# JulHoltzDevelopers/WavesAndEigenvalues.jl

Measured on AMD Instinct MI355X. Metric: eigenpairs/sec, higher is better.
Workload: dtype f64

## Files before the change

dev/probes/modes_ab.py:

```python
import os, sys
import numpy as np
ROOT = os.path.dirname(os.path.dirname(os.path.dirname(os.path.abspath(__file__))))
sys.path.insert(0, ROOT)
import wae_amd
from wae_amd.helmholtz.family import annulus_family
preset = sys.argv[1] if len(sys.argv) > 1 else "C3"
r = int(sys.argv[2]) if len(sys.argv) > 2 else 64
modes = [int(m) for m in sys.argv[3:]] or [0, 1, 2, 6]
L, pb = annulus_family(preset, tau=2e-4)
fam = L.device()
cz = L.coefficients(2 * np.pi * (500 + 20j))
names = {0: "A X", 1: "residual", 2: "Jacobi sweep", 6: "product + first sweep"}
out = {}
for m in modes:
    os.environ["WAE_BENCH_MODE"] = str(m)
    best = min(fam.bench_spmv(cz, r=r, reps=30) for _ in range(3))
    out[names.get(m, m)] = round(best * 1e3, 1)
print(os.environ.get("WAE_LIB_PATH", "default"), preset, r, out, flush=True)
```

wavesandeigenvalues.jl_amd/csrc/debug.hip:

```cpp
#include <algorithm>
#include <vector>

#include "solver.h"

namespace {
struct StreamGuard {
    hipStream_t s = nullptr;
    ~StreamGuard() { if (s) (void)hipStreamDestroy(s); }
};
int64_t span(int64_t nv, int64_t stride, int64_t blk) { return nv > 0 ? (nv - 1) * stride + blk : 0; }
void fill_xorshift(std::vector<cplx> &hx) {
    uint64_t s = 0x9E3779B97F4A7C15ull;
    for (auto &v : hx) { s ^= s << 13; s ^= s >> 7; s ^= s << 17; v.x = (double)(s & 0xFFFFF) / 524288.0 - 1.0; v.y = (double)((s >> 20) & 0xFFFFF) / 524288.0 - 1.0; }
}
template <class F> double mean_ms(hipStream_t st, int reps, F &&one) {
    for (int i = 0; i < 3; ++i) one();
    hipEvent_t e0, e1;
    HIP_CHECK(hipEventCreate(&e0));
    HIP_CHECK(hipEventCreate(&e1));
    HIP_CHECK(hipEventRecord(e0, st));
    for (int i = 0; i < reps; ++i) one();
    HIP_CHECK(hipEventRecord(e1, st));
    HIP_CHECK(hipEventSynchronize(e1));
    float ms = 0.f;
// ... 242 lines not shown
        HIP_CHECK(hipMemsetAsync(relres.p, 0, (size_t)nb * sizeof(double), st));
        HIP_CHECK(hipMemsetAsync(rescale.p, 0, (size_t)nb * sizeof(cplx), st));
        HIP_CHECK(hipMemsetAsync(cmask.p, 0, (size_t)nch, st));
        s_relres.alloc((size_t)nev * nb); s_int.alloc((size_t)nev * nint); s_cmask.alloc((size_t)nev * nch); s_rescale.alloc((size_t)nev * nb);
        s_sv.alloc((size_t)nev * 2 * nb); s_vsq.alloc((size_t)nev * 2 * nb);
        HIP_CHECK(hipMemsetAsync(s_sv.p, 0, (size_t)nev * 2 * nb * sizeof(double), st));
        HIP_CHECK(hipMemsetAsync(s_vsq.p, 0, (size_t)nev * 2 * nb * sizeof(cplx), st));
        GmresDev S;
        S.nb = nb; S.m = m; S.histcap = histcap;
        S.R = R.p; S.cs = cs.p; S.sn = sn.p; S.g = g.p; S.sv = sv.p; S.vsq = vsq.p;
        S.conv = ints.p; S.steps = S.conv + nb; S.iters = S.steps + nb; S.histlen = S.iters + nb; S.stalled = S.histlen + nb; S.status = S.stalled + nb;
        S.relres = relres.p; S.bnorm = bn.p; S.hist = hist.p; S.rescale = rescale.p; S.cmask = cmask.p;
        S.Hraw = Hraw.p; S.sub = sub.p;
        auto d2d = [&](void *dst, const void *src, size_t bytes) { HIP_CHECK(hipMemcpyAsync(dst, src, bytes, hipMemcpyDeviceToDevice, st)); };
        for (int e = 0, ii = 0; e < nev; ++e) {
            const int64_t kind = ev[4 * e], j = ev[4 * e + 1], off = ev[4 * e + 3];
            const int use_mask = ev[4 * e + 2] ? 1 : 0;
            const double tol = evd[2 * e], lim = evd[2 * e + 1];
            cplx *a = dpool.p + off;
            int row0 = -1, rows = 0;
            if (kind == WAE_GMRES_INIT) {
                launch_gmres_init(S, a, ddone.p + (size_t)ii * nb, use_mask, st);
                ++ii;
                row0 = 0; rows = 1;
            } else if (kind == WAE_GMRES_STEP) {
                d2d(vsq.p + (size_t)(j + 1) * nb, dinv.p + (size_t)e * 2 * nb, (size_t)nb * sizeof(cplx));
                launch_gmres_step(S, a, (int)j, tol, lim, use_mask, a + (j + 2) * N, n, st);
                row0 = (int)j + 1; rows = 1;
            } else if (kind == WAE_GMRES_PAIR) {
                cplx *c1 = a, *c2 = c1 + (j + 1) * N, *gram = c2 + (j + 1) * N, *norms = gram + 3 * N, *W1 = norms + 2 * N, *W2 = W1 + blk,
                     *alpha = W2 + blk, *c2m = alpha + N, *hd2 = c2m + (j + 1) * N;
                launch_gmres_pair_coef(S, (int)j, c1, c2, gram, alpha, c2m, hd2, st);
                d2d(vsq.p + (size_t)(j + 1) * nb, dinv.p + (size_t)e * 2 * nb, (size_t)2 * nb * sizeof(cplx));
                launch_gmres_step(S, c1, (int)j, tol, 1e300, use_mask, W1, n, st, norms);
                launch_gmres_step(S, hd2, (int)j + 1, tol, lim, use_mask, W2, n, st, norms + N);
                row0 = (int)j + 1; rows = 2;
            } else {
                launch_gmres_solve_y(S, (int)j, a, st);
            }
            d2d(s_relres.p + (size_t)e * nb, relres.p, (size_t)nb * sizeof(double));
            d2d(s_int.p + (size_t)e * nint, ints.p, (size_t)nint * sizeof(int));
            d2d(s_cmask.p + (size_t)e * nch, cmask.p, (size_t)nch);
            d2d(s_rescale.p + (size_t)e * nb, rescale.p, (size_t)nb * sizeof(cplx));
            if (rows) {
                d2d(s_sv.p + (size_t)e * 2 * nb, sv.p + (size_t)row0 * nb, (size_t)rows * nb * sizeof(double));
                d2d(s_vsq.p + (size_t)e * 2 * nb, vsq.p + (size_t)row0 * nb, (size_t)rows * nb * sizeof(cplx));
            }
        }
        auto back = [&](void *dst, const void *src, size_t bytes) { HIP_CHECK(hipMemcpyAsync(dst, src, bytes, hipMemcpyDeviceToHost, st)); };
        cplx *oc = (cplx *)cstate;
        back(pool, dpool.p, (size_t)plen * sizeof(cplx));
        back(oc, R.p, nR * sizeof(cplx)); back(oc + nR, sn.p, nrow * sizeof(cplx)); back(oc + nR + nrow, g.p, (nrow + nb) * sizeof(cplx));
        back(oc + nR + 2 * nrow + nb, vsq.p, (nrow + 2 * nb) * sizeof(cplx)); back(oc + nR + 3 * nrow + 3 * nb, Hraw.p, nR * sizeof(cplx));
        back(dstate, cs.p, nrow * sizeof(double)); back(dstate + nrow, sv.p, (nrow + 2 * nb) * sizeof(double));
        back(dstate + 2 * nrow + 2 * nb, sub.p, nrow * sizeof(double)); back(dstate + 3 * nrow + 2 * nb, hist.p, (size_t)histcap * nb * sizeof(double));
        back(snap_relres, s_relres.p, (size_t)nev * nb * sizeof(double)); back(snap_int, s_int.p, (size_t)nev * nint * sizeof(int));
        back(snap_cmask, s_cmask.p, (size_t)nev * nch); back(snap_rescale, s_rescale.p, (size_t)nev * nb * sizeof(cplx));
        back(snap_sv, s_sv.p, (size_t)nev * 2 * nb * sizeof(double)); back(snap_vsq, s_vsq.p, (size_t)nev * 2 * nb * sizeof(cplx));
        HIP_CHECK(hipStreamSynchronize(st));
        return WAE_OK;
    });
}

extern "C" {

int wae_bench_spmv(wae_family *h, const double *coeffs, int32_t r, int32_t reps, double *ms_out) {
    return guarded([&]() {
        WAE_REQUIRE(h && coeffs && r > 0 && reps > 0 && ms_out, "bad argument");
        HIP_CHECK(hipSetDevice(h->device));
        hipStream_t st = h->stream;
        const size_t cnt = (size_t)h->d * r;
        DevBuf<cplx> x, y, pcd;
        x.alloc(cnt); y.alloc(cnt);
        std::vector<cplx> hx(cnt);
        fill_xorshift(hx);
        HIP_CHECK(hipMemcpyAsync(x.p, hx.data(), cnt * sizeof(cplx), hipMemcpyHostToDevice, st));
        std::vector<zc> pc;
        plane_coeffs(h, coeffs, WAE_OP_N, pc);
        std::vector<cplx> tab((size_t)h->nplanes);
        slot_coeffs(h, h->slot_plane[0], pc, tab.data());
        pcd.upload(tab.data(), tab.size(), st);
        const OpDev A = h->ops[0].dev(WAE_OP_N);
        const int bmode = getenv("WAE_BENCH_MODE") ? atoi(getenv("WAE_BENCH_MODE")) : MODE_AX;
        DevBuf<cplx> bb;
        if (bmode != MODE_AX) { bb.alloc(cnt); HIP_CHECK(hipMemcpyAsync(bb.p, hx.data(), cnt * sizeof(cplx), hipMemcpyHostToDevice, st)); }
        auto one = [&]() { launch_spmv(A, pcd.p, 1 << 30, x.p, y.p, bmode != MODE_AX ? bb.p : nullptr, 0.8, r, bmode, st); };
        *ms_out = mean_ms(st, reps, one);
        return WAE_OK;
    });
}

int wae_debug_spmv(wae_family *h, int32_t which, int32_t level, int32_t mode, const double *coeffs, int32_t ncoef, const double *X,
                   const double *B, double *Y, double *B2, int32_t r, int32_t op, double jac_w, const uint8_t *cmask, int32_t flags,
                   int64_t *n_in_q, int64_t *n_out_q) {
    return guarded([&]() {
        WAE_REQUIRE(h && which >= 0 && which <= 2 && level >= 0 && op >= 0 && op <= 2, "bad argument");
        WAE_REQUIRE(level == 0 || h->solver_ready, "levels >= 1 need wae_solver_setup");
        WAE_REQUIRE(which == 0 ? (level == 0 || level < (int)h->ops.size() - 1) : level < (int)h->xfer.size(), "no such level");
        const int64_t n_in = which == 0 ? h->ops[level].n : (which == 1 ? h->xfer[level].nf : h->xfer[level].nc);
        const int64_t n_out = which == 0 ? h->ops[level].n : (which == 1 ? h->xfer[level].nc : h->xfer[level].nf);
        if (n_in_q) *n_in_q = n_in;
        if (n_out_q) *n_out_q = n_out;
        if (!X && !Y) return WAE_OK;
        WAE_REQUIRE(X && Y && r > 0 && r <= 256, "bad argument (1 <= r <= 256)");
        WAE_REQUIRE(which != 0 || (coeffs && (ncoef == 1 || ncoef == r)), "ncoef must be 1 or r");
        WAE_REQUIRE(mode >= MODE_AX && mode <= MODE_AX_J0 && (which == 0 || mode == (which == 1 ? MODE_AX : MODE_ADD)), "bad mode");
        WAE_REQUIRE(B || mode == MODE_AX || mode == MODE_AX_DS || mode == MODE_AX_J0, "this mode reads B");
        WAE_REQUIRE(mode != MODE_AX_J0 || B2, "mode 6 writes B2");
        HIP_CHECK(hipSetDevice(h->device));
        hipStream_t st = h->stream;
        const int *perm = level == 0 && which != 1 ? h->perm() : nullptr;
        const int *perm_in = level == 0 && which != 2 ? h->perm() : nullptr;
        DevBuf<cplx> xc, yc, xi, yi, bi, pcd;
        DevBuf<unsigned char> cm;
        const size_t cin = (size_t)n_in * r, cout = (size_t)n_out * r;
        xc.alloc(std::max(cin, cout)); yc.alloc(cout); xi.alloc(cin); yi.alloc(cout); bi.alloc(cout);
        HIP_CHECK(hipMemcpyAsync(xc.p, X, cin * sizeof(cplx), hipMemcpyHostToDevice, st));
        launch_colmajor_to_inter(xc.p, n_in, r, xi.p, r, st, perm_in);
        auto stage = [&](const double *src, cplx *dst) {
            HIP_CHECK(hipMemcpyAsync(yc.p, src, cout * sizeof(cplx), hipMemcpyHostToDevice, st));
            launch_colmajor_to_inter(yc.p, n_out, r, dst, r, st, perm);
        };
        stage(Y, yi.p);
        if (mode == MODE_AX_J0) stage(B2, bi.p);
        else if (B) stage(B, bi.p);
        if (cmask) cm.upload(cmask, (size_t)(r + 7) / 8, st);
        OpDev A;
        int cps = 1 << 30;
        if (which == 0) {
            std::vector<cplx> tab((size_t)ncoef * h->nplanes);
            std::vector<zc> pc;
            for (int s = 0; s < ncoef; ++s) {
                plane_coeffs(h, coeffs + (size_t)s * 2 * h->T, op, pc);
                slot_coeffs(h, h->slot_plane[level], pc, &tab[(size_t)s * h->nplanes]);
            }
            pcd.upload(tab.data(), tab.size(), st);
            A = h->ops[level].dev(op);
            cps = ncoef == 1 ? (1 << 30) : 1;
        } else {
            A = h->xfer[level].devR();
        }
        if (flags & 1) A.tiles = nullptr;
        const Transfer *xf = which == 0 ? nullptr : &h->xfer[level];
        const bool by_tile = xf && xf->ft.ready && !(flags & 1) && r >= 8;
        if (which == 2) {
            const cplx *src = (const void *)B == (const void *)Y ? yi.p : bi.p;
            if (by_tile) launch_prolong_tiles(xf->ft.dev, xi.p, src, yi.p, r, st, cmask ? cm.p : nullptr);
            else launch_prolong_add(xf->p_ptr.p, xf->p_col.p, xf->p_val.p, xf->nf, xi.p, src, yi.p, r, st, cmask ? cm.p : nullptr);
        } else
        launch_spmv(A, which == 0 ? pcd.p : h->one_dev.p, cps, xi.p, yi.p, (mode == MODE_AX || mode == MODE_AX_DS) ? nullptr : bi.p, jac_w, r, mode, st,
                    cmask ? cm.p : nullptr);
        launch_inter_to_colmajor(yi.p, r, n_out, r, yc.p, st, perm);
        HIP_CHECK(hipMemcpyAsync(Y, yc.p, cout * sizeof(cplx), hipMemcpyDeviceToHost, st));
        if (mode == MODE_AX_J0) {
            HIP_CHECK(hipStreamSynchronize(st));
            launch_inter_to_colmajor(bi.p, r, n_out, r, yc.p, st, perm);
            HIP_CHECK(hipMemcpyAsync(B2, yc.p, cout * sizeof(cplx), hipMemcpyDeviceToHost, st));
        }
        HIP_CHECK(hipStreamSynchronize(st));
        return WAE_OK;
    });
}

int wae_debug_prolong(wae_family *h, int32_t level, const double *X, const double *B, double *Y, double *norms, int32_t r, const uint8_t *cmask,
                      int32_t flags) {
    return guarded([&]() {
        WAE_REQUIRE(h && X && B && Y && norms, "bad argument");
        require_solver(h);
        WAE_REQUIRE(level >= 0 && level < (int)h->xfer.size(), "no such level");
        WAE_REQUIRE(r >= 1 && r <= 256, "bad argument (1 <= r <= 256)");
        WAE_REQUIRE(flags >= 0 && flags < 4, "unknown flag");
        const Transfer *xf = &h->xfer[level];
        const int64_t nc = xf->nc, nf = xf->nf;
        HIP_CHECK(hipSetDevice(h->device));
        hipStream_t st = h->stream;
        const int *perm = level == 0 ? h->perm() : nullptr;
        const size_t cin = (size_t)nc * r, cout = (size_t)nf * r;
        const bool by_tile = xf->ft.ready && !(flags & 1) && r >= 8;
        DevBuf<cplx> xc, yc, xi, yi, bi, part, nrm;
        DevBuf<unsigned char> cm;
        xc.alloc(cin); yc.alloc(cout); xi.alloc(cin); yi.alloc(cout); bi.alloc(cout); nrm.alloc((size_t)r);
        part.alloc((size_t)(by_tile ? xf->ft.dev.ntiles : PROLONG_NORM_BLOCKS) * r);
        HIP_CHECK(hipMemcpyAsync(xc.p, X, cin * sizeof(cplx), hipMemcpyHostToDevice, st));
        launch_colmajor_to_inter(xc.p, nc, r, xi.p, r, st, nullptr);
        HIP_CHECK(hipMemcpyAsync(yc.p, Y, cout * sizeof(cplx), hipMemcpyHostToDevice, st));
        launch_colmajor_to_inter(yc.p, nf, r, yi.p, r, st, perm);
        HIP_CHECK(hipStreamSynchronize(st));
        HIP_CHECK(hipMemcpyAsync(yc.p, B, cout * sizeof(cplx), hipMemcpyHostToDevice, st));
        launch_colmajor_to_inter(yc.p, nf, r, bi.p, r, st, perm);
        if (cmask) cm.upload(cmask, (size_t)(r + 7) / 8, st);
        cplx *const dst = (flags & 2) ? nullptr : yi.p;
        if (by_tile) launch_prolong_tiles(xf->ft.dev, xi.p, bi.p, dst, r, st, cmask ? cm.p : nullptr, part.p, nrm.p);
        else launch_prolong_add(xf->p_ptr.p, xf->p_col.p, xf->p_val.p, nf, xi.p, bi.p, dst, r, st, cmask ? cm.p : nullptr, part.p, nrm.p);
        launch_inter_to_colmajor(yi.p, r, nf, r, yc.p, st, perm);
        HIP_CHECK(hipMemcpyAsync(Y, yc.p, cout * sizeof(cplx), hipMemcpyDeviceToHost, st));
        std::vector<cplx> hn((size_t)r);
        HIP_CHECK(hipMemcpyAsync(hn.data(), nrm.p, (size_t)r * sizeof(cplx), hipMemcpyDeviceToHost, st));
        HIP_CHECK(hipStreamSynchronize(st));
        for (int b = 0; b < r; ++b) norms[b] = hn[(size_t)b].x;
        return WAE_OK;
    });
}

int wae_debug_vcycle(wae_family *h, int32_t level, const double *coeffs, int32_t ncoef, const double *B, double *Y, int32_t r, int32_t op,
                     int32_t flags, const uint8_t *cmask) {
    return guarded([&]() {
        WAE_REQUIRE(h && coeffs && B && Y, "bad argument");
        require_solver(h);
        const int L = (int)h->ops.size() - 1;
        WAE_REQUIRE(level >= 0 && level <= L, "no such level");
        WAE_REQUIRE(r >= 1 && r <= h->NB, "r must be in 1..NB (opts[6] of wae_solver_setup)");
        WAE_REQUIRE(ncoef == 1 || ncoef == r, "ncoef must be 1 or r");
        WAE_REQUIRE(op >= 0 && op <= 2, "bad op");
        WAE_REQUIRE(flags >= 0 && flags < 8, "unknown flag");
        WAE_REQUIRE(!(flags & 4) || level == 0, "flags bit 2 (Y = M^-1 A V) needs level 0");
        HIP_CHECK(hipSetDevice(h->device));
        hipStream_t st = h->stream;
        struct LightRestore { bool &on; bool was; ~LightRestore() { on = was; } } light_restore{h->vc_light, h->vc_light};
        h->vc_light = (flags & 1) != 0;
        const Batch bt = ncoef == 1 ? Batch::one_system(r, op) : Batch::per_column(r, op);
        std::vector<std::vector<zc>> pcs((size_t)bt.nsys);
        for (int s = 0; s < bt.nsys; ++s) plane_coeffs(h, coeffs + (size_t)s * 2 * h->T, op, pcs[(size_t)s]);
        upload_pc(h, pcs);
        dense_setup(h, bt);
        const int64_t n = h->ops[level].n;
        const size_t cnt = (size_t)n * r;
        const int *perm = level == 0 ? h->perm() : nullptr;
        DevBuf<cplx> col, vin, fout;
        DevBuf<unsigned char> cm;
        col.alloc(cnt);
        if (cmask) cm.upload(cmask, (size_t)(r + 7) / 8, st);
        const unsigned char *mk = (cmask && r >= 8) ? cm.p : nullptr;
        cplx *x = h->lx[level].p;
        HIP_CHECK(hipMemcpyAsync(col.p, Y, cnt * sizeof(cplx), hipMemcpyHostToDevice, st));
        launch_colmajor_to_inter(col.p, n, r, x, r, st, perm);
        launch_copy(x, h->lt[level].p, cnt, st);
        if (flags & 2) { fout.alloc(cnt); launch_copy(x, fout.p, cnt, st); }
        cplx *b = level == 0 ? h->W.p : h->lb[level].p;
        HIP_CHECK(hipMemcpyAsync(col.p, B, cnt * sizeof(cplx), hipMemcpyHostToDevice, st));
        bool have_x0 = false;
        if (flags & 4) {
            vin.alloc(cnt);
            launch_colmajor_to_inter(col.p, n, r, vin.p, r, st, perm);
            have_x0 = L > 0;
            launch_spmv(h->ops[0].dev(op), pc_level(h, 0), bt.cps, vin.p, b, have_x0 ? x : nullptr, have_x0 ? pre_weight(h) : 0.0, r,
                        have_x0 ? MODE_AX_J0 : MODE_AX, st, mk);
        } else {
            launch_colmajor_to_inter(col.p, n, r, b, r, st, perm);
        }
        const cplx *res = vcycle(h, bt, level, b, mk, have_x0, (flags & 2) ? fout.p : nullptr);
        launch_inter_to_colmajor(res, r, n, r, col.p, st, perm);
        HIP_CHECK(hipMemcpyAsync(Y, col.p, cnt * sizeof(cplx), hipMemcpyDeviceToHost, st));
        HIP_CHECK(hipStreamSynchronize(st));
        return WAE_OK;
    });
}

int wae_bench_spmv_level(wae_family *h, const double *coeffs, int32_t which, int32_t level, int32_t r, int32_t reps, double *ms_out,
                         int64_t *bytes_out) {
    return guarded([&]() {
        WAE_REQUIRE(h && coeffs && which >= 0 && which <= 2 && level >= 0 && r > 0 && r <= 256 && reps > 0 && ms_out, "bad argument");
        require_solver(h);
        WAE_REQUIRE(which == 0 ? (level == 0 || level < (int)h->ops.size() - 1) : level < (int)h->xfer.size(), "no such level");
        HIP_CHECK(hipSetDevice(h->device));
        hipStream_t st = h->stream;
        const int64_t n_in = which == 0 ? h->ops[level].n : (which == 1 ? h->xfer[level].nf : h->xfer[level].nc);
        const int64_t n_out = which == 0 ? h->ops[level].n : (which == 1 ? h->xfer[level].nc : h->xfer[level].nf);
        DevBuf<cplx> x, y, pcd;
        x.alloc((size_t)n_in * r); y.alloc((size_t)n_out * r);
        std::vector<cplx> hx((size_t)n_in * r);
        fill_xorshift(hx);
        HIP_CHECK(hipMemcpyAsync(x.p, hx.data(), hx.size() * sizeof(cplx), hipMemcpyHostToDevice, st));
        OpDev A;
        const cplx *pcp = h->one_dev.p;
        int64_t bytes = 2;
        if (which == 0) {
            std::vector<zc> pc;
            plane_coeffs(h, coeffs, WAE_OP_N, pc);
            std::vector<cplx> tab(h->nplanes);
            slot_coeffs(h, h->slot_plane[level], pc, tab.data());
            pcd.upload(tab.data(), tab.size(), st);
            pcp = pcd.p;
            A = h->ops[level].dev(WAE_OP_N);
            bytes = 0;
            for (size_t g = 0; g < h->ops[level].groups.size(); ++g) {
                const GroupHost &G = h->ops[level].groups[g];
                for (int q = 0; q < G.nplanes; ++q)
                    if (tab[G.plane0 + q].x != 0.0 || tab[G.plane0 + q].y != 0.0) bytes += G.nnz * 20 + (n_out + 1) * 4;
            }
        } else {
            A = h->xfer[level].devR();
            bytes = (int64_t)h->xfer[level].r_col.n * 12 + (n_out + 1) * 4;
        }
        bytes += (int64_t)r * (n_in + n_out) * 16;
        if (which == 2) bytes += (int64_t)r * n_out * 16;
        if (bytes_out) *bytes_out = bytes;
        const Transfer *xf = which == 0 ? nullptr : &h->xfer[level];
        const bool by_tile = xf && xf->ft.ready && r >= 8 && xfer_tiles_on();
        auto one = [&]() {
            if (which == 2) {
                if (by_tile) launch_prolong_tiles(xf->ft.dev, x.p, y.p, y.p, r, st);
                else launch_prolong_add(xf->p_ptr.p, xf->p_col.p, xf->p_val.p, xf->nf, x.p, y.p, y.p, r, st, nullptr);
            } else launch_spmv(A, pcp, 1 << 30, x.p, y.p, nullptr, 0.0, r, MODE_AX, st);
        };
        if (which == 2) HIP_CHECK(hipMemsetAsync(y.p, 0, (size_t)n_out * r * sizeof(cplx), st));
        *ms_out = mean_ms(st, reps, one);
        return WAE_OK;
    });
}

int wae_bench_triad(int32_t device, int64_t n, int32_t reps, double *gbs_out) {
    return guarded([&]() {
        WAE_REQUIRE(n > 0 && reps > 0 && gbs_out, "bad argument");
        HIP_CHECK(hipSetDevice(device));
        DevBuf<double> a, b, c;
        a.alloc(n); b.alloc(n); c.alloc(n);
        HIP_CHECK(hipMemset(b.p, 0, n * sizeof(double)));
        HIP_CHECK(hipMemset(c.p, 0, n * sizeof(double)));
        hipStream_t st;
        HIP_CHECK(hipStreamCreate(&st));
        hipEvent_t e0, e1;
        HIP_CHECK(hipEventCreate(&e0));
        HIP_CHECK(hipEventCreate(&e1));
        double best = 0.0;
        for (unsigned cap : {512u, 1024u, 4096u, 8192u, 65536u}) {
            for (int i = 0; i < 2; ++i) launch_triad(a.p, b.p, c.p, 1.5, n, st, cap);
            HIP_CHECK(hipEventRecord(e0, st));
            for (int i = 0; i < reps; ++i) launch_triad(a.p, b.p, c.p, 1.5, n, st, cap);
            HIP_CHECK(hipEventRecord(e1, st));
            HIP_CHECK(hipEventSynchronize(e1));
            float ms = 0.f;
            HIP_CHECK(hipEventElapsedTime(&ms, e0, e1));
            best = std::max(best, 3.0 * n * sizeof(double) * reps / (ms * 1e-3) / 1e9);
// ... 11 lines not shown
```

wavesandeigenvalues.jl_amd/csrc/gmres.hip:

```cpp
#include <cmath>

#include "solver.h"

void upload_pc(wae_family *h, const std::vector<std::vector<zc>> &pcs) {
    const int nsys = (int)pcs.size();
    const int nl = (int)h->ops.size();
    const size_t per_level = (size_t)nsys * h->nplanes;
    std::vector<cplx> tab(per_level * (nl + 2));
    for (int l = 0; l <= nl + 1; ++l) {
        if (l >= nl && h->n_penalty == 0) break;
        const std::vector<int> &sp = l < nl ? h->slot_plane[l] : (l == nl ? h->pen_slot : h->pen_row_slot);
        for (int s = 0; s < nsys; ++s) slot_coeffs(h, sp, pcs[s], &tab[l * per_level + (size_t)s * h->nplanes]);
    }
    h->pc_stride_level = per_level;
    h->pcdev.upload(tab.data(), tab.size(), h->stream);
    HIP_CHECK(hipStreamSynchronize(h->stream));
}
const cplx *pc_level(const wae_family *h, int l) { return h->pcdev.p + (size_t)l * h->pc_stride_level; }

void dense_setup(wae_family *h, const Batch &bt) {
    const int L = (int)h->ops.size() - 1;
    if (h->nc <= 0) return;
    HIP_CHECK(hipMemsetAsync(h->dstatus.p, 0, sizeof(int), h->stream));
    launch_dense_assemble(h->dense_planes.p, h->nplanes, (int)h->nc, pc_level(h, L), bt.nsys, bt.op, h->Ainv.p, h->stream);
    launch_dense_invert(h->Ainv.p, (int)h->nc, bt.nsys, h->dstatus.p, h->stream);
    int st = 0;
    HIP_CHECK(hipMemcpyAsync(&st, h->dstatus.p, sizeof(int), hipMemcpyDeviceToHost, h->stream));
    HIP_CHECK(hipStreamSynchronize(h->stream));
    if (st) throw WaeError(WAE_ERR_BREAKDOWN, "coarse operator is singular");
}

double pre_weight(const wae_family *h) { return h->vc_light ? h->jac_w_light : h->jac_w; }

cplx *vcycle(wae_family *h, const Batch &bt, int l, const cplx *b, const unsigned char *cm, bool have_x0, cplx *final_out, CycleNorms *cn) {
    const int L = (int)h->ops.size() - 1;
    hipStream_t st = h->stream;
    if (l == L) {
        launch_dense_apply(h->Ainv.p, (int)h->nc, bt.cps, b, h->lx[l].p, bt.nb, st, cm);
        return h->lx[l].p;
    }
    const OpDev A = h->ops[l].dev(bt.op);
    const cplx *pc = pc_level(h, l);
    cplx *x = h->lx[l].p, *t = h->lt[l].p;
    if (!have_x0) launch_jacobi0(A, pc, bt.cps, b, x, pre_weight(h), bt.nb, st, cm);
    for (int s = 1; s < h->nsweeps; ++s) {
        launch_spmv(A, pc, bt.cps, x, t, b, pre_weight(h), bt.nb, MODE_JAC, st, cm);
        std::swap(x, t);
    }
    launch_spmv(A, pc, bt.cps, x, t, b, 0.0, bt.nb, MODE_RES, st, cm);
    const bool by_tile = h->xfer[l].ft.ready && bt.nb >= 8 && xfer_tiles_on();
    launch_spmv(h->xfer[l].devR(), h->one_dev.p, 1 << 30, t, h->lb[l + 1].p, nullptr, 0.0, bt.nb, MODE_AX, st, cm);
    const cplx *xc = vcycle(h, bt, l + 1, h->lb[l + 1].p, cm);
    const int npost = h->vc_light ? 0 : h->nsweeps;
    const size_t npart = (size_t)(by_tile ? h->xfer[l].ft.dev.ntiles : PROLONG_NORM_BLOCKS) * bt.nb;
    const bool norms = cn && l == 0 && npost == 0 && npart <= h->partial.n && h->ops[l].n > 0 && !(cn->only && final_out);
    cplx *const px = (norms && cn->only) ? nullptr : (final_out && npost == 0) ? final_out : x;
    cplx *const part = norms ? h->partial.p : nullptr, *const nout = norms ? cn->out : nullptr;
    if (by_tile) launch_prolong_tiles(h->xfer[l].ft.dev, xc, x, px, bt.nb, st, cm, part, nout);
    else launch_prolong_add(h->xfer[l].p_ptr.p, h->xfer[l].p_col.p, h->xfer[l].p_val.p, h->xfer[l].nf, xc, x, px, bt.nb, st, cm, part, nout);
    if (norms) cn->done = true;
    if (px) x = px;
    for (int s = 0; s < npost; ++s) {
        cplx *dst = (final_out && s == npost - 1) ? final_out : t;
        launch_spmv(A, pc, bt.cps, x, dst, b, h->jac_w_post, bt.nb, MODE_JAC, st, cm);
        if (dst == t) std::swap(x, t); else x = dst;
    }
    if (final_out && x != final_out) { launch_copy(x, final_out, (size_t)h->ops[l].n * bt.nb, st); x = final_out; }
    return x;
}

struct ColState {
    std::vector<zc> H;
    std::vector<zc> Hraw;
    std::vector<zc> g;
    std::vector<double> cs;
    std::vector<zc> sn;
    std::vector<zc> cdef;
    int ld = 0;
    int steps = 0;
    bool conv = false;

    ColState(int m, bool keep_raw, double beta, bool done)
        : H((size_t)(m + 1) * m), Hraw(keep_raw ? (size_t)(m + 1) * m : 0), g(m + 1), cs(m), sn(m), cdef(m), ld(m + 1), conv(done) { g[0] = beta; }
    bool rotate_in(int jc, const zc *raw, zc cdef_j, bool &nan) {
        zc *Hc = &H[(size_t)jc * ld];
        for (int i = 0; i <= jc + 1; ++i) Hc[i] = raw[i];
        if (!Hraw.empty()) std::copy(raw, raw + jc + 2, &Hraw[(size_t)jc * ld]);
        cdef[jc] = cdef_j;
        for (int i = 0; i < jc; ++i) {
            const zc a = Hc[i], bb = Hc[i + 1];
            Hc[i] = cs[i] * a + sn[i] * bb;
            Hc[i + 1] = -std::conj(sn[i]) * a + cs[i] * bb;
        }
        const zc a = Hc[jc];
        const double bb = Hc[jc + 1].real();
        const double aa = std::abs(a);
        const double t = std::sqrt(aa * aa + bb * bb);
        if (!(t > 0.0) || std::isnan(t)) { conv = true; if (std::isnan(t)) nan = true; return false; }
        if (aa == 0.0) { cs[jc] = 0.0; sn[jc] = 1.0; }
        else { cs[jc] = aa / t; sn[jc] = (a / aa) * (bb / t); }
        Hc[jc] = cs[jc] * a + sn[jc] * bb;
        Hc[jc + 1] = 0;
        g[jc + 1] = -std::conj(sn[jc]) * g[jc];
        g[jc] = cs[jc] * g[jc];
        steps = jc + 1;
        return true;
    }
    std::vector<zc> back_substitute() const {
        std::vector<zc> y(steps);
        for (int i = steps - 1; i >= 0; --i) {
            zc s = g[i];
            for (int q = i + 1; q < steps; ++q) s -= H[(size_t)q * ld + i] * y[q];
            const zc dgi = H[(size_t)i * ld + i];
            y[i] = (dgi != zc(0)) ? s / dgi : zc(0);
        }
        return y;
    }
};

void penalty_polish(wae_family *h, const Batch &bt, const cplx *B, cplx *X) {
    if (h->n_penalty <= 0) return;
    static const std::vector<double> cheb = []() {
        const int n = 22;
        const double lo = 0.4, hi = 2.2, th = 0.5 * (hi + lo), de = 0.5 * (hi - lo);
        std::vector<double> w(n);
        for (int k = 0; k < n; ++k) w[k] = 1.0 / (th - de * std::cos((2 * k + 1) * M_PI / (2 * n)));
        std::vector<double> o;
        for (int a = 0, b = n - 1; a <= b; ++a, --b) { o.push_back(w[a]); if (a != b) o.push_back(w[b]); }
        return o;
    }();
    const int sweeps = (int)cheb.size();
    hipStream_t st = h->stream;
    const int nb = bt.nb;
    const int64_t nbk = h->n_penalty;
    const OpDev A = h->ops[0].dev(bt.op);
    const OpDev Ab = h->pen_op.dev(bt.op);
    const cplx *pcb = pc_level(h, (int)h->ops.size());
    if (bt.op == WAE_OP_N && h->pen_row_op.n == nbk) {
        launch_gather_rows(B, h->pen_rows.p, nbk, nb, h->pen_t.p, st);
        launch_spmv(h->pen_row_op.dev(WAE_OP_N), pc_level(h, (int)h->ops.size() + 1), bt.cps, X, h->pen_b.p, h->pen_t.p, 0.0, nb, MODE_RES, st);
    } else {
        launch_spmv(A, pc_level(h, 0), bt.cps, X, h->W.p, B, 0.0, nb, MODE_RES, st);
        launch_gather_rows(h->W.p, h->pen_rows.p, nbk, nb, h->pen_b.p, st);
    }
    launch_norms(h->pen_b.p, nbk, nb, h->partial.p, h->hdev.p, st);
    cplx *x = h->pen_x.p, *t = h->pen_t.p;
    launch_jacobi0(Ab, pcb, bt.cps, h->pen_b.p, x, cheb[0], nb, st);
    for (int s = 1; s < sweeps; ++s) {
        launch_spmv(Ab, pcb, bt.cps, x, t, h->pen_b.p, cheb[(size_t)s], nb, MODE_JAC, st);
        std::swap(x, t);
    }
    launch_spmv(Ab, pcb, bt.cps, x, t, h->pen_b.p, 0.0, nb, MODE_RES, st);
    launch_norms(t, nbk, nb, h->partial.p, h->hdev.p + nb, st);
    cplx *hp = h->h_pinned;
    HIP_CHECK(hipMemcpyAsync(hp, h->hdev.p, (size_t)2 * nb * sizeof(cplx), hipMemcpyDeviceToHost, st));
    HIP_CHECK(hipStreamSynchronize(st));
    for (int b = 0; b < nb; ++b)
        if (!(hp[nb + b].x <= 1e-3 * hp[b].x)) return;
    launch_scatter_add_rows(x, h->pen_rows.p, nbk, nb, X, st);
}

struct GmresEnv {
    bool lazy = env_int("WAE_LAZY", 1) != 0;
    double lazy_limit = getenv("WAE_LAZY_LIMIT") ? atof(getenv("WAE_LAZY_LIMIT")) : 1e100;
    bool device = env_int("WAE_GMRES_DEVICE", 1) != 0;
    int sync = std::max(1, env_int("WAE_GMRES_SYNC", 4));
    int pair_min = env_int("WAE_GMRES_PAIR", 2);
    int narrow_pair = env_int("WAE_NARROW_PAIR", -1);
    int debug = env_int("WAE_GMRES_DEBUG", 0);
    bool mask0 = env_int("WAE_GMRES_MASK0", 1) != 0;
};
static const GmresEnv &gmres_env() { static const GmresEnv e; return e; }

struct Gmres {
    wae_family *h;
    const Batch &bt;
    const cplx *B;
    cplx *X;
    const cplx *guess_dir;
    double tol;
    int maxit;
    bool have_x0;
    double *relres_out = nullptr;
    hipStream_t st = h->stream;
    int nb = bt.nb;
    int64_t n = h->d;
    size_t vec = (size_t)n * nb;
    OpDev A = h->ops[0].dev(bt.op);
    const cplx *pc = pc_level(h, 0);
    cplx *hp = h->h_pinned;
    bool reorth = nb <= 8;
    bool deflate = guess_dir != nullptr && h->ops.size() > 1;
    int off = deflate ? 1 : 0;
    int m = (int)std::min<size_t>(150, h->V.n / vec - 1) - off;
    bool lazy = gmres_env().lazy && !reorth && ((size_t)m + off + 2) * nb <= 4096 && ((size_t)m + off + 2) * nb <= h->vsq.n;
    bool pair_cfg = reorth && h->ops.size() > 1 &&
                    (gmres_env().narrow_pair > 0 || (gmres_env().narrow_pair < 0 && vec * sizeof(cplx) >= ((size_t)4 << 20)));
    size_t PK = (size_t)(m + off + 3) * nb;
    std::vector<double> bnorm = std::vector<double>(nb), relres = std::vector<double>(nb, 0.0);
    std::vector<int> iters = std::vector<int>(nb, 0);
    std::vector<unsigned char> done = std::vector<unsigned char>(nb, 0), stalled = std::vector<unsigned char>(nb, 0);
    int total_it = 0;
    bool nan_seen = false, x0_unchecked = have_x0;
    double t0 = now_s();
    std::vector<ColState> cs;
    std::vector<std::vector<double>> sv;
    std::vector<std::vector<double>> hist = std::vector<std::vector<double>>(nb);
    std::vector<double> unorm = std::vector<double>(nb, 0.0);
    std::vector<zc> beta0 = std::vector<zc>(nb, zc(0));
    const unsigned char *mk = nullptr;
    cplx *pr_dev = nullptr, *pr_host = nullptr;

    cplx *start() {
        if (!have_x0) launch_fill_zero(X, vec, st);
        CycleNorms cn{h->hdev.p, have_x0};
        cplx *const zb = vcycle(h, bt, 0, B, nullptr, false, nullptr, &cn);
        if (!cn.done) launch_norms(zb, n, nb, h->partial.p, h->hdev.p, st);
        HIP_CHECK(hipMemcpyAsync(hp, h->hdev.p, nb * sizeof(cplx), hipMemcpyDeviceToHost, st));
        HIP_CHECK(hipStreamSynchronize(st));
        for (int b = 0; b < nb; ++b) { bnorm[b] = hp[b].x; if (!(bnorm[b] > 0.0)) done[b] = 1; }
        return zb;
    }
    cplx *residual(CycleNorms *cn = nullptr) {
        launch_spmv(A, pc, bt.cps, X, h->W.p, B, 0.0, nb, MODE_RES, st);
        return vcycle(h, bt, 0, h->W.p, nullptr, false, nullptr, cn);
    }
    bool drop_bad_guess() {
        if (!x0_unchecked) return false;
        x0_unchecked = false;
        std::vector<cplx> keep(nb, cplx{1.0, 0.0});
        bool any_bad = false;
        for (int b = 0; b < nb; ++b)
            if (bnorm[b] > 0.0 && !(hp[b].x / bnorm[b] <= 1.0)) { keep[b] = cplx{0.0, 0.0}; any_bad = true; }
        if (!any_bad) return false;
        h->ydev.upload(keep.data(), nb, st);
        launch_mask_cols(X, h->ydev.p, n, nb, st);
        HIP_CHECK(hipStreamSynchronize(st));
        return true;
    }
    template <class F> bool cycle_start(F &&more) {
        bool all_done = true;
        for (int b = 0; b < nb; ++b) {
            if (bnorm[b] > 0.0) {
                relres[b] = hp[b].x / bnorm[b];
                if (std::isnan(relres[b])) nan_seen = true;
                done[b] = relres[b] <= tol || stalled[b];
                more(b);
            }
            if (!done[b]) all_done = false;
        }
        return all_done;
    }
    bool converged_by_estimate(int j) const {
        if (j > 12) return false;
        for (int b = 0; b < nb; ++b) if (stalled[b] || (bnorm[b] > 0.0 && !(relres[b] <= tol))) return false;
        return true;
    }
    template <class F> int finish(wae_solve_info *info, F &&debug_line) {
        if (have_x0 && !nan_seen) penalty_polish(h, bt, B, X);
        if (relres_out) for (int b = 0; b < nb; ++b) relres_out[b] = bnorm[b] > 0.0 ? relres[b] : 0.0;
        if (gmres_env().debug) {
            HIP_CHECK(hipStreamSynchronize(st));
            debug_line();
        }
        if (info) {
            int imax = 0, itot = 0, nun = 0;
            double rmax = 0.0;
            for (int b = 0; b < nb; ++b) {
                imax = std::max(imax, iters[b]);
                itot += iters[b];
                if (bnorm[b] > 0.0) {
                    if (!(relres[b] <= tol)) ++nun;
                    rmax = std::max(rmax, relres[b]);
                }
                if (stalled[b] && !(relres[b] <= tol)) info->levels |= 1 << 16;
            }
            info->iters_max = std::max(info->iters_max, imax);
            info->iters_total += itot;
            info->n_unconverged += nun;
            info->relres_max = std::max(info->relres_max, rmax);
            info->levels = (info->levels & (1 << 16)) | (int)h->ops.size();
        }
        if (nan_seen) throw WaeError(WAE_ERR_NAN, "NaN in GMRES");
        return total_it;
    }

    int run_device(wae_solve_info *info) {
        const GmresEnv &env = gmres_env();
        const double lim = env.lazy_limit;
        const bool use_mask = have_x0 || (env.mask0 && nb >= 8);
        const int nch = (nb + 7) / 8;
        const int histcap = maxit + m + 8;
        h->gs_R.reserve((size_t)m * (m + 1) * nb); h->gs_sn.reserve((size_t)m * nb); h->gs_g.reserve((size_t)(m + 1) * nb); h->gs_rescale.reserve((size_t)nb);
        h->gs_cs.reserve((size_t)m * nb); h->gs_sv.reserve((size_t)(m + 2) * nb); h->gs_relres.reserve((size_t)nb); h->gs_bnorm.reserve((size_t)nb);
        h->gs_hist.reserve((size_t)histcap * nb); h->gs_int.reserve((size_t)5 * nb + 4); h->gs_done.reserve((size_t)nb);
        h->cmask.reserve(nch); h->vsq.reserve((size_t)(m + 2) * nb);
        GmresDev S;
        S.nb = nb; S.m = m; S.histcap = histcap;
        S.R = h->gs_R.p; S.cs = h->gs_cs.p; S.sn = h->gs_sn.p; S.g = h->gs_g.p; S.sv = h->gs_sv.p; S.vsq = h->vsq.p;
        S.conv = h->gs_int.p; S.steps = S.conv + nb; S.iters = S.steps + nb; S.histlen = S.iters + nb; S.stalled = S.histlen + nb; S.status = S.stalled + nb;
        S.relres = h->gs_relres.p; S.bnorm = h->gs_bnorm.p; S.hist = h->gs_hist.p; S.rescale = h->gs_rescale.p; S.cmask = h->cmask.p;
        const int pair_min = env.pair_min;
        const bool pair_on = pair_min >= 0 && lim >= 1e50 && nb >= 8 && h->ops.size() > 1;
        h->gs_Hraw.reserve((size_t)m * (m + 1) * nb); h->gs_pair.reserve(((size_t)4 * (m + 3) + 8) * nb); h->gs_sub.reserve((size_t)m * nb);
        S.Hraw = h->gs_Hraw.p; S.sub = h->gs_sub.p;
        cplx *const pr_c1 = h->gs_pair.p, *const pr_c2 = pr_c1 + (size_t)(m + 3) * nb, *const pr_c2m = pr_c2 + (size_t)(m + 3) * nb,
                   *const pr_hd2 = pr_c2m + (size_t)(m + 3) * nb, *const pr_gram = pr_hd2 + (size_t)(m + 3) * nb, *const pr_alpha = pr_gram + (size_t)3 * nb,
                   *const pr_norm = pr_alpha + nb;
        HIP_CHECK(hipMemsetAsync(h->gs_int.p, 0, ((size_t)5 * nb + 4) * sizeof(int), st));
        cplx *const zb = start();
        std::vector<double> bn(bnorm);
        for (double &v : bn) if (!(v > 0.0)) v = 1.0;
        HIP_CHECK(hipMemcpyAsync(h->gs_bnorm.p, bn.data(), nb * sizeof(double), hipMemcpyHostToDevice, st));
        HIP_CHECK(hipStreamSynchronize(st));
        std::vector<int> hostint((size_t)5 * nb + 4);
        bool first = !have_x0;
        while (true) {
            CycleNorms cn{h->hdev.p, false};
            cplx *const z0 = first ? zb : residual(&cn);
            first = false;
            if (!cn.done) launch_norms(z0, n, nb, h->partial.p, h->hdev.p, st);
            HIP_CHECK(hipMemcpyAsync(hp, h->hdev.p, (size_t)nb * sizeof(cplx), hipMemcpyDeviceToHost, st));
            HIP_CHECK(hipStreamSynchronize(st));
            if (drop_bad_guess()) continue;
            if (cycle_start([](int) {}) || total_it >= maxit || nan_seen) break;
            launch_scale_inv(z0, h->hdev.p, h->V.p, n, nb, st);
            HIP_CHECK(hipMemcpyAsync(h->gs_done.p, done.data(), nb, hipMemcpyHostToDevice, st));
            launch_gmres_init(S, h->hdev.p, h->gs_done.p, use_mask ? 1 : 0, st);
            HIP_CHECK(hipStreamSynchronize(st));
            const unsigned char *mk = (use_mask && nb >= 8) ? h->cmask.p : nullptr;
            int j = 0;
            int status[4] = {0, 0, 0, 0};
            for (int b = 0; b < nb; ++b) status[0] += done[b] ? 0 : 1;
            int since_sync = 0;
            for (; j < m && total_it < maxit;) {
                const cplx *vj = h->V.p + (size_t)j * vec;
                const int nvj = j + 1;
                const bool fuse0 = h->ops.size() > 1;
                if (pair_on && j >= pair_min && j + 2 <= m && total_it + 2 <= maxit && status[0] > nb / 4) {
                    cplx *w1 = h->V.p + (size_t)nvj * vec, *w2 = w1 + vec;
                    launch_spmv(A, pc, bt.cps, vj, h->W.p, h->lx[0].p, pre_weight(h), nb, MODE_AX_J0, st, mk);
                    vcycle(h, bt, 0, h->W.p, mk, true, w1);
                    launch_spmv(A, pc, bt.cps, w1, h->W.p, h->lx[0].p, pre_weight(h), nb, MODE_AX_J0, st, mk);
                    vcycle(h, bt, 0, h->W.p, mk, true, w2);
                    launch_dots2_scaled(h->V.p, vec, nvj, w1, w2, n, nb, h->partial.p, pr_c1, pr_c2, pr_gram, h->vsq.p, st, mk);
                    launch_gmres_pair_coef(S, j, pr_c1, pr_c2, pr_gram, pr_alpha, pr_c2m, pr_hd2, st);
                    launch_axpy2_norm(h->V.p, vec, nvj, pr_c1, pr_c2m, pr_alpha, w1, w2, n, nb, h->partial.p, pr_norm, h->vsq.p + (size_t)nvj * nb, st, mk);
                    launch_gmres_step(S, pr_c1, j, tol, 1e300, use_mask ? 1 : 0, w1, n, st, pr_norm);
                    launch_gmres_step(S, pr_hd2, j + 1, tol, lim, use_mask ? 1 : 0, w2, n, st, pr_norm + nb);
                    j += 2;
                    total_it += 2;
                    since_sync += 2;
                } else {
                    launch_spmv(A, pc, bt.cps, vj, h->W.p, fuse0 ? h->lx[0].p : nullptr, fuse0 ? pre_weight(h) : 0.0, nb, fuse0 ? MODE_AX_J0 : MODE_AX, st, mk);
                    cplx *w = vcycle(h, bt, 0, h->W.p, mk, fuse0);
                    launch_dots_scaled(h->V.p, vec, nvj, w, n, nb, h->partial.p, h->hdev.p, h->vsq.p, st, mk);
                    launch_axpy_neg_norm(h->V.p, vec, nvj, h->hdev.p, h->V.p + (size_t)nvj * vec, n, nb, h->partial.p, h->hdev.p + (size_t)nvj * nb, st, mk,
                                         w, h->vsq.p + (size_t)nvj * nb);
                    launch_gmres_step(S, h->hdev.p, j, tol, lim, use_mask ? 1 : 0, h->V.p + (size_t)nvj * vec, n, st);
                    ++j;
                    ++total_it;
                    ++since_sync;
                }
                if (since_sync >= ((have_x0 && j <= 4) ? 1 : env.sync) || j == m || total_it >= maxit || status[0] <= nb / 4) {
                    since_sync = 0;
                    HIP_CHECK(hipMemcpyAsync(status, S.status, 3 * sizeof(int), hipMemcpyDeviceToHost, st));
                    HIP_CHECK(hipStreamSynchronize(st));
                    if (status[1]) nan_seen = true;
                    if (status[0] == 0 || nan_seen) break;
                }
            }
            if (j > 0) {
                launch_gmres_solve_y(S, j, h->ydev.p, st);
                launch_lincomb_add(h->V.p, vec, j, h->ydev.p, X, n, nb, st);
            }
            HIP_CHECK(hipMemcpyAsync(hostint.data(), h->gs_int.p, ((size_t)5 * nb + 4) * sizeof(int), hipMemcpyDeviceToHost, st));
            HIP_CHECK(hipMemcpyAsync(hp, h->gs_relres.p, nb * sizeof(double), hipMemcpyDeviceToHost, st));
            HIP_CHECK(hipStreamSynchronize(st));
            const double *rr = (const double *)hp;
            for (int b = 0; b < nb; ++b) {
                iters[b] = hostint[(size_t)2 * nb + b];
                stalled[b] = (unsigned char)hostint[(size_t)4 * nb + b];
                if (hostint[(size_t)nb + b] > 0 && bnorm[b] > 0.0) relres[b] = rr[b];
            }
            if (hostint[(size_t)5 * nb + 1]) nan_seen = true;
            if (nan_seen || converged_by_estimate(j)) break;
        }
        return finish(info, [&]() {
            int itot = 0;
            for (int b = 0; b < nb; ++b) itot += iters[b];
            fprintf(stderr, "[gmres] nb=%d x0=%d lockstep_its=%d column_its=%d %.1f ms (device recurrence)\n", nb, (int)have_x0, total_it, itot,
                    (now_s() - t0) * 1e3);
            if (env.debug > 2) {
                for (int b0 = 0; b0 < nb; b0 += bt.cps) {
                    fprintf(stderr, "[gmres]   steps");
                    for (int b = b0; b < std::min(nb, b0 + bt.cps); ++b) fprintf(stderr, " %d", iters[b]);
                    fprintf(stderr, "\n");
                }
            }
        });
    }

    void absorb(int b, int jc, const zc *raw, zc cdef_j) {
        ColState &c = cs[b];
        if (c.conv || !c.rotate_in(jc, raw, cdef_j, nan_seen)) return;
        iters[b]++;
        relres[b] = std::abs(c.g[jc + 1]) / bnorm[b];
        hist[b].push_back(relres[b]);
        const size_t hs = hist[b].size();
        if (relres[b] <= 0.7 * tol) c.conv = true;
        else if (hs > 60 && relres[b] > 0.9 * hist[b][hs - 31]) { c.conv = true; stalled[b] = 1; }
    }

    void pair_step(int j) {
        const cplx *vj = h->V.p + (size_t)(off + j) * vec;
        const int nv = off + j + 1;
        cplx *w1 = h->V.p + (size_t)nv * vec, *w2 = w1 + vec;
        cplx *c1a = pr_dev, *c2a = c1a + PK, *c1b = c2a + PK, *c2b = c1b + PK, *c2m = c2b + PK, *zero_al = c2m + PK,
             *gram = zero_al + nb, *alpha = gram + 3 * (size_t)nb, *nrm = alpha + nb, *inv = nrm + 2 * (size_t)nb,
             *tdef = inv + 2 * (size_t)nb;
        launch_spmv(A, pc, bt.cps, vj, h->W.p, h->lx[0].p, pre_weight(h), nb, MODE_AX_J0, st, mk);
        vcycle(h, bt, 0, h->W.p, mk, true, w1);
        if (deflate) {
            launch_dots(h->V.p, vec, 1, w1, n, nb, h->partial.p, tdef, st, mk);
            launch_axpy_neg(h->V.p, vec, 1, tdef, w1, n, nb, st, mk);
        }
        launch_spmv(A, pc, bt.cps, w1, h->W.p, h->lx[0].p, pre_weight(h), nb, MODE_AX_J0, st, mk);
        vcycle(h, bt, 0, h->W.p, mk, true, w2);
        launch_dots2_scaled(h->V.p, vec, nv, w1, w2, n, nb, h->partial.p, c1a, c2a, gram, h->vsq.p, st, mk);
        launch_fill_zero(zero_al, nb, st);
        launch_axpy2_norm(h->V.p, vec, nv, c1a, c2a, zero_al, w1, w2, n, nb, h->partial.p, nrm, inv, st, mk);
        launch_dots2_scaled(h->V.p, vec, nv, w1, w2, n, nb, h->partial.p, c1b, c2b, gram, h->vsq.p, st, mk);
        HIP_CHECK(hipMemcpyAsync(pr_host, pr_dev, (4 * PK) * sizeof(cplx), hipMemcpyDeviceToHost, st));
        HIP_CHECK(hipMemcpyAsync(pr_host + 5 * PK + nb, gram, (size_t)3 * nb * sizeof(cplx), hipMemcpyDeviceToHost, st));
        cplx *htdef = pr_host + 5 * PK + 7 * (size_t)nb;
        if (deflate) HIP_CHECK(hipMemcpyAsync(htdef, tdef, (size_t)nb * sizeof(cplx), hipMemcpyDeviceToHost, st));
        HIP_CHECK(hipStreamSynchronize(st));
        const cplx *hc1a = pr_host, *hc2a = hc1a + PK, *hc1b = hc2a + PK, *hc2b = hc1b + PK, *hgram = pr_host + 5 * PK + nb;
        cplx *hc2m = pr_host + 4 * PK, *halpha = pr_host + 5 * PK + 4 * (size_t)nb;
        auto Z = [](const cplx &v) { return zc(v.x, v.y); };
        std::vector<zc> rawcol((size_t)m + 3);
        std::vector<zc> beta(nb, zc(0));
        for (int b = 0; b < nb; ++b) {
            double g11 = hgram[b].x;
            zc g12 = Z(hgram[(size_t)nb + b]);
            for (int i = 0; i < nv; ++i) {
                const zc p1 = Z(hc1b[(size_t)i * nb + b]), p2 = Z(hc2b[(size_t)i * nb + b]);
                g11 -= std::norm(p1);
                g12 -= std::conj(p1) * p2;
            }
            beta[b] = g11 > 0.0 ? g12 / g11 : zc(0);
            if (!std::isfinite(beta[b].real()) || !std::isfinite(beta[b].imag())) beta[b] = zc(0);
            halpha[b] = cplx{beta[b].real(), beta[b].imag()};
            for (int i = 0; i < nv; ++i) {
                const zc q = Z(hc2b[(size_t)i * nb + b]) - beta[b] * Z(hc1b[(size_t)i * nb + b]);
                hc2m[(size_t)i * nb + b] = cplx{q.real(), q.imag()};
            }
        }
        HIP_CHECK(hipMemcpyAsync(c2m, hc2m, (size_t)nv * nb * sizeof(cplx), hipMemcpyHostToDevice, st));
        HIP_CHECK(hipMemcpyAsync(alpha, halpha, (size_t)nb * sizeof(cplx), hipMemcpyHostToDevice, st));
        launch_axpy2_norm(h->V.p, vec, nv, c1b, c2m, alpha, w1, w2, n, nb, h->partial.p, nrm, inv, st, mk);
        launch_scale_inv(w1, nrm, w1, n, nb, st, mk);
        launch_scale_inv(w2, nrm + nb, w2, n, nb, st, mk);
        cplx *hnrm = pr_host + 5 * PK + 5 * (size_t)nb;
        HIP_CHECK(hipMemcpyAsync(hnrm, nrm, (size_t)2 * nb * sizeof(cplx), hipMemcpyDeviceToHost, st));
        HIP_CHECK(hipStreamSynchronize(st));
        total_it += 2;
        for (int b = 0; b < nb; ++b) {
            ColState &c = cs[b];
            if (c.conv) continue;
            const double a1 = hnrm[b].x, a2 = hnrm[(size_t)nb + b].x;
            const int nk = j + 1;
            std::vector<zc> cc1(nk), cc2(nk);
            for (int i = 0; i < nk; ++i) {
                cc1[i] = Z(hc1a[(size_t)(off + i) * nb + b]) + Z(hc1b[(size_t)(off + i) * nb + b]);
                cc2[i] = Z(hc2a[(size_t)(off + i) * nb + b]) + Z(hc2b[(size_t)(off + i) * nb + b]);
            }
            const zc e1 = deflate ? Z(hc1a[b]) + Z(hc1b[b]) : zc(0), e2 = deflate ? Z(hc2a[b]) + Z(hc2b[b]) : zc(0);
            const zc cdef_j = deflate ? Z(htdef[b]) + e1 : zc(0);
            for (int i = 0; i < nk; ++i) rawcol[i] = cc1[i];
            rawcol[nk] = a1;
            absorb(b, j, rawcol.data(), cdef_j);
            if (c.conv) continue;
            if (!(a1 > 0.0)) { c.conv = true; continue; }
            for (int r = 0; r <= j; ++r) {
                zc d = 0;
                for (int i = std::max(0, r - 1); i < j; ++i) d += c.Hraw[(size_t)i * c.ld + r] * cc1[i];
                rawcol[r] = (cc2[r] - d - cc1[j] * cc1[r]) / a1;
            }
            rawcol[j + 1] = beta[b] - cc1[j];
            rawcol[j + 2] = a2 / a1;
            zc cdef_n = 0;
            if (deflate) {
                cdef_n = e2 - cc1[j] * cdef_j;
                for (int i = 0; i < j; ++i) cdef_n -= cc1[i] * c.cdef[i];
                cdef_n /= a1;
            }
            absorb(b, j + 1, rawcol.data(), cdef_n);
        }
    }

    void single_step(int j) {
        const cplx *vj = h->V.p + (size_t)(off + j) * vec;
        const int nvj = off + j + 1;
        const bool fuse0 = h->ops.size() > 1;
        launch_spmv(A, pc, bt.cps, vj, h->W.p, fuse0 ? h->lx[0].p : nullptr, fuse0 ? pre_weight(h) : 0.0, nb, fuse0 ? MODE_AX_J0 : MODE_AX, st, mk);
        cplx *w = vcycle(h, bt, 0, h->W.p, mk, fuse0);
        if (lazy) {
            launch_dots_scaled(h->V.p, vec, nvj, w, n, nb, h->partial.p, h->hdev.p, h->vsq.p, st, mk);
            launch_axpy_neg_norm(h->V.p, vec, nvj, h->hdev.p, h->V.p + (size_t)nvj * vec, n, nb, h->partial.p, h->hdev.p + (size_t)nvj * nb, st, mk,
                                 w, h->vsq.p + (size_t)nvj * nb);
        } else {
            launch_dots(h->V.p, vec, nvj, w, n, nb, h->partial.p, h->hdev.p, st, mk);
            if (reorth) {
                launch_axpy_neg(h->V.p, vec, nvj, h->hdev.p, w, n, nb, st, mk);
                cplx *h2 = h->hdev.p + (size_t)(off + m + 2) * nb;
                launch_dots(h->V.p, vec, nvj, w, n, nb, h->partial.p, h2, st, mk);
                launch_axpy_neg_norm(h->V.p, vec, nvj, h2, w, n, nb, h->partial.p, h->hdev.p + (size_t)nvj * nb, st, mk);
                launch_add(h2, h->hdev.p, (size_t)nvj * nb, st);
            } else {
                launch_axpy_neg_norm(h->V.p, vec, nvj, h->hdev.p, w, n, nb, h->partial.p, h->hdev.p + (size_t)nvj * nb, st, mk);
            }
            launch_scale_inv(w, h->hdev.p + (size_t)nvj * nb, h->V.p + (size_t)nvj * vec, n, nb, st, mk);
        }
        HIP_CHECK(hipMemcpyAsync(hp, h->hdev.p, (size_t)(nvj + 1) * nb * sizeof(cplx), hipMemcpyDeviceToHost, st));
        HIP_CHECK(hipStreamSynchronize(st));
        if (lazy) {
            for (int b = 0; b < nb; ++b) {
                const double sj = sv[nvj - 1][b];
                for (int i = 0; i < nvj; ++i) {
                    const double f = sv[i][b] > 0.0 ? sj / sv[i][b] : 0.0;
                    hp[(size_t)i * nb + b].x *= f;
                    hp[(size_t)i * nb + b].y *= f;
                }
                const double r = hp[(size_t)nvj * nb + b].x;
                sv[nvj][b] = r > 0.0 ? 1.0 / r : 0.0;
                hp[(size_t)nvj * nb + b].x = sj * r;
            }
            const double lim = gmres_env().lazy_limit;
            bool rescale = false;
            for (int b = 0; b < nb; ++b) rescale = rescale || sv[nvj][b] > lim || (sv[nvj][b] > 0.0 && sv[nvj][b] < 1.0 / lim);
            if (rescale) {
                launch_scale_inv(h->V.p + (size_t)nvj * vec, h->hdev.p + (size_t)nvj * nb, h->V.p + (size_t)nvj * vec, n, nb, st, mk);
                std::vector<cplx> ones(nb, cplx{1.0, 0.0});
                for (int b = 0; b < nb; ++b) if (sv[nvj][b] > 0.0) sv[nvj][b] = 1.0; else ones[b] = cplx{0.0, 0.0};
                HIP_CHECK(hipMemcpyAsync(h->vsq.p + (size_t)nvj * nb, ones.data(), (size_t)nb * sizeof(cplx), hipMemcpyHostToDevice, st));
                HIP_CHECK(hipStreamSynchronize(st));
            }
        }
        ++total_it;
        std::vector<zc> rawcol((size_t)m + 3);
        for (int b = 0; b < nb; ++b) {
            if (cs[b].conv) continue;
            for (int i = 0; i <= j + 1; ++i) rawcol[i] = zc(hp[(size_t)(off + i) * nb + b].x, hp[(size_t)(off + i) * nb + b].y);
            absorb(b, j, rawcol.data(), deflate ? zc(hp[b].x, hp[b].y) : zc(0));
        }
    }

    void add_alpha_g(const std::vector<zc> &num) {
        std::vector<cplx> al(nb, cplx{0.0, 0.0});
        for (int b = 0; b < nb; ++b) {
            if (!(unorm[b] > 0.0)) continue;
            const zc a = num[b] / unorm[b];
            if (std::isfinite(a.real()) && std::isfinite(a.imag())) al[b] = cplx{a.real(), a.imag()};
        }
        h->ydev.upload(al.data(), nb, st);
        launch_lincomb(guess_dir, 0, 1, h->ydev.p, h->U.p, n, nb, st);
        launch_add(h->U.p, X, vec, st);
        HIP_CHECK(hipStreamSynchronize(st));
    }

    int run_host(wae_solve_info *info) {
        sv.assign(lazy ? (size_t)m + off + 2 : 0, std::vector<double>(nb, 1.0));
        const int pair_min = 4;
        if (pair_cfg) {
            const size_t need = 6 * PK + 16 * (size_t)nb;
            h->gs_pair.reserve(need);
            if (h->h_pin_pair_n < need) {
                if (h->h_pin_pair) { (void)hipHostFree(h->h_pin_pair); h->h_pin_pair = nullptr; h->h_pin_pair_n = 0; }
                HIP_CHECK(hipHostMalloc((void **)&h->h_pin_pair, need * sizeof(cplx)));
                h->h_pin_pair_n = need;
            }
            pr_dev = h->gs_pair.p; pr_host = h->h_pin_pair;
            h->vsq.reserve(PK);
            std::vector<cplx> ones(PK, cplx{1.0, 0.0});
            h->vsq.upload(ones.data(), ones.size(), st);
            HIP_CHECK(hipStreamSynchronize(st));
        }
        cplx *const zb0 = start();
        std::vector<double> drift_ref(nb, 0.0);
        bool drift_mode = false;
        bool first = !have_x0;
        const int nch = (nb + 7) / 8;
        const bool use_mask = have_x0;
        std::vector<unsigned char> cm(nch, 1), cm_prev(nch, 2);
        h->cmask.reserve(nch);
        auto set_mask = [&](auto &&active) {
            for (int k = 0; k < nch; ++k) cm[k] = 0;
            for (int b = 0; b < nb; ++b) if (active(b)) cm[b >> 3] = 1;
            if (cm != cm_prev) {
                HIP_CHECK(hipMemcpyAsync(h->cmask.p, cm.data(), nch, hipMemcpyHostToDevice, st));
                HIP_CHECK(hipStreamSynchronize(st));
                cm_prev = cm;
            }
        };
        if (deflate) {
            launch_spmv(A, pc, bt.cps, guess_dir, h->W.p, nullptr, 0.0, nb, MODE_AX, st);
            launch_copy(vcycle(h, bt, 0, h->W.p), h->V.p, vec, st);
            launch_norms(h->V.p, n, nb, h->partial.p, h->hdev.p, st);
            launch_norms(guess_dir, n, nb, h->partial.p, h->hdev.p + nb, st);
            HIP_CHECK(hipMemcpyAsync(hp, h->hdev.p, (size_t)2 * nb * sizeof(cplx), hipMemcpyDeviceToHost, st));
            HIP_CHECK(hipStreamSynchronize(st));
            std::vector<cplx> un(nb);
            for (int b = 0; b < nb; ++b) {
                unorm[b] = (hp[b].x > 1e-12 * hp[nb + b].x && hp[nb + b].x > 0.0) ? hp[b].x : 0.0;
                un[b] = cplx{unorm[b], 0.0};
            }
            h->ydev.upload(un.data(), nb, st);
            launch_scale_inv(h->V.p, h->ydev.p, h->V.p, n, nb, st);
            HIP_CHECK(hipStreamSynchronize(st));
        }
        if (guess_dir && !deflate) {
            launch_spmv(A, pc, bt.cps, guess_dir, h->W.p, nullptr, 0.0, nb, MODE_AX, st);
            launch_copy(vcycle(h, bt, 0, h->W.p), h->U.p, vec, st);
            const cplx *zb = vcycle(h, bt, 0, B);
            launch_dots(h->U.p, 0, 1, zb, n, nb, h->partial.p, h->hdev.p, st);
            launch_dots(h->U.p, 0, 1, h->U.p, n, nb, h->partial.p, h->hdev.p + nb, st);
            HIP_CHECK(hipMemcpyAsync(hp, h->hdev.p, (size_t)2 * nb * sizeof(cplx), hipMemcpyDeviceToHost, st));
            HIP_CHECK(hipStreamSynchronize(st));
            std::vector<cplx> al(nb);
            for (int b = 0; b < nb; ++b) {
                const double den = hp[nb + b].x;
                al[b] = den > 0.0 ? cplx{hp[b].x / den, hp[b].y / den} : cplx{0.0, 0.0};
            }
            h->ydev.upload(al.data(), nb, st);
            launch_lincomb(guess_dir, 0, 1, h->ydev.p, X, n, nb, st);
            HIP_CHECK(hipStreamSynchronize(st));
            first = false;
        }
        while (true) {
            cplx *const z0 = !first ? residual() : guess_dir ? vcycle(h, bt, 0, B) : zb0;
            first = false;
            if (deflate) {
                launch_dots(h->V.p, 0, 1, z0, n, nb, h->partial.p, h->hdev.p + nb, st);
                launch_axpy_neg(h->V.p, 0, 1, h->hdev.p + nb, z0, n, nb, st);
            }
            launch_norms(z0, n, nb, h->partial.p, h->hdev.p, st);
            HIP_CHECK(hipMemcpyAsync(hp, h->hdev.p, (size_t)2 * nb * sizeof(cplx), hipMemcpyDeviceToHost, st));
            HIP_CHECK(hipStreamSynchronize(st));
            if (deflate) for (int b = 0; b < nb; ++b) beta0[b] = zc(hp[nb + b].x, hp[nb + b].y);
            if (drop_bad_guess()) continue;
            const bool all_done = cycle_start([&](int b) {
                if (!done[b]) {
                    const double est = hist[b].empty() ? -1.0 : hist[b].back();
                    if (drift_mode && drift_ref[b] > 0.0 && relres[b] > 0.5 * drift_ref[b]) { stalled[b] = 1; done[b] = 1; }
                    else if (est >= 0.0 && est <= tol && relres[b] > 50.0 * est) drift_mode = true;
                }
                drift_ref[b] = relres[b];
            });
            if (gmres_env().debug > 1) {
                double rmax = 0.0, emax = 0.0;
                for (int b = 0; b < nb; ++b) { rmax = std::max(rmax, relres[b]); if (!hist[b].empty()) emax = std::max(emax, hist[b].back()); }
                fprintf(stderr, "[gmres]   cycle start at %d steps: true relres max %.2e (last estimate %.2e)\n", total_it, rmax, emax);
            }
            if (all_done || total_it >= maxit || nan_seen) {
                if (deflate && !nan_seen) add_alpha_g(beta0);
                break;
            }
            launch_scale_inv(z0, h->hdev.p, h->V.p + (size_t)off * vec, n, nb, st);
            if (lazy) {
                for (int i = 0; i <= off; ++i) std::fill(sv[i].begin(), sv[i].end(), 1.0);
                std::vector<cplx> ones((size_t)(off + 1) * nb, cplx{1.0, 0.0});
                h->vsq.upload(ones.data(), ones.size(), st);
                HIP_CHECK(hipStreamSynchronize(st));
            }
            if (use_mask && nb >= 8) {
                set_mask([&](int b) { return !done[b]; });
                mk = h->cmask.p;
            }
            cs.clear();
            for (int b = 0; b < nb; ++b) cs.emplace_back(m, pair_cfg, hp[b].x, done[b]);
            int j = 0;
            const int m_cycle = drift_mode ? std::min(m, 5) : m;
            while (j < m_cycle && total_it < maxit) {
                if (pair_cfg && j >= pair_min && j + 2 <= m_cycle && total_it + 2 <= maxit) {
                    pair_step(j);
                    j += 2;
                } else {
                    single_step(j);
                    ++j;
                }
                bool all_conv = true;
                for (int b = 0; b < nb; ++b) all_conv = all_conv && cs[b].conv;
                if (all_conv || nan_seen) break;
                if (mk) set_mask([&](int b) { return !cs[b].conv; });
            }
            mk = nullptr;
            const int ju = std::min(j, m);
            std::vector<cplx> y((size_t)std::max(ju, 1) * nb, cplx{0.0, 0.0});
            for (int b = 0; b < nb; ++b) {
                const std::vector<zc> yy = cs[b].back_substitute();
                for (int i = 0; i < cs[b].steps; ++i) {
                    const double f = lazy ? sv[off + i][b] : 1.0;
                    y[(size_t)i * nb + b] = cplx{f * yy[i].real(), f * yy[i].imag()};
                }
            }
            if (ju > 0) {
// ... 99 lines not shown
```

wavesandeigenvalues.jl_amd/csrc/kernel_helpers.h:

```cpp
#pragma once
#include <algorithm>
#include <mutex>
#include "wae_internal.h"

__device__ __forceinline__ cplx cmul(cplx a, cplx b) { return cplx{a.x * b.x - a.y * b.y, a.x * b.y + a.y * b.x}; }
__device__ __forceinline__ cplx cconj(cplx a) { return cplx{a.x, -a.y}; }
__device__ __forceinline__ void cfma(cplx &acc, cplx a, cplx b) {
    acc.x = fma(a.x, b.x, acc.x); acc.x = fma(-a.y, b.y, acc.x);
    acc.y = fma(a.x, b.y, acc.y); acc.y = fma(a.y, b.x, acc.y);
}
typedef double dbl2v __attribute__((ext_vector_type(2)));
__device__ __forceinline__ cplx stream_load(const cplx *p) {
#ifndef WAE_NO_NT_GS
    const dbl2v v = __builtin_nontemporal_load((const dbl2v *)p);
    return cplx{v.x, v.y};
#else
    return *p;
#endif
}
__device__ __forceinline__ cplx cdiv(cplx a, cplx b) {
    double s = 1.0 / (b.x * b.x + b.y * b.y);
    return cplx{(a.x * b.x + a.y * b.y) * s, (a.y * b.x - a.x * b.y) * s};
}
__device__ __forceinline__ int next_chunk(const unsigned char *cmask, int c, int nch) { while (c < nch && cmask && !cmask[c]) ++c; return c; }

static inline unsigned grid_for(size_t total, unsigned cap = 4096) {
    size_t g = (total + 255) / 256;
    if (g < 1) g = 1;
    return (unsigned)(g > cap ? cap : g);
}
struct RowGrid { int R; int64_t steps; unsigned grid; };
static inline RowGrid row_grid(int64_t n, int nb, int nt, int rpt, int64_t cap) {
    const int R = nt / nb;
    const int64_t per = (int64_t)R * rpt, steps = (n + per - 1) / per;
    return RowGrid{R, steps, (unsigned)std::min(steps, cap)};
}
struct OncePerDevice { std::mutex mu; bool done[64] = {false}; };
template <class F> static inline int once_per_device(OncePerDevice &s, F &&f) {
    int dev = 0;
    HIP_CHECK(hipGetDevice(&dev));
    std::lock_guard<std::mutex> lock(s.mu);
    if (!s.done[dev & 63]) { f(dev); s.done[dev & 63] = true; }
    return dev;
}
```

wavesandeigenvalues.jl_amd/csrc/kernels.hip:

```cpp
#include <type_traits>
#include "block_reduce.h"
#include "kernel_helpers.h"

#include <cstdlib>

__device__ __forceinline__ void long_row_piece(const int *__restrict__ ptr, const int *__restrict__ col, const int *__restrict__ slot,
                                               const cplx *__restrict__ val, int npl, int conj, const cplx *__restrict__ pc, int cps,
                                               const cplx *__restrict__ X, int nb, const unsigned char *__restrict__ cmask, cplx *__restrict__ part) {
    __shared__ cplx red[256];
    const int li = blockIdx.x / WAE_LONG_SPLIT, k = blockIdx.x - li * WAE_LONG_SPLIT, ch = blockIdx.y;
    if (cmask && !cmask[ch]) return;
    const int tid = threadIdx.x, c = tid & 7, seg = tid >> 3;
    const int b = ch * 8 + c;
    const int bb = b < nb ? b : nb - 1;
    const cplx *mypc = pc + (size_t)(bb / cps) * npl;
    const double sg = conj ? -1.0 : 1.0;
    const int beg = ptr[li], end = ptr[li + 1];
    const int piece = ((end - beg + WAE_LONG_SPLIT - 1) / WAE_LONG_SPLIT + 31) & ~31;
    const int p0 = beg + k * piece, p1 = min(end, p0 + piece);
    cplx acc = {0.0, 0.0};
    int p = p0 + seg;
    for (; p + 96 < p1; p += 128) {
        int cc[4], sl[4];
        cplx a[4], x[4];
#pragma unroll
        for (int u = 0; u < 4; ++u) { cc[u] = col[p + 32 * u]; sl[u] = slot[p + 32 * u]; a[u] = val[p + 32 * u]; }
#pragma unroll
        for (int u = 0; u < 4; ++u) x[u] = X[(size_t)cc[u] * nb + bb];
#pragma unroll
        for (int u = 0; u < 4; ++u) { a[u].y *= sg; cfma(acc, cmul(mypc[sl[u]], a[u]), x[u]); }
    }
    for (; p < p1; p += 32) {
        cplx a = val[p];
        a.y *= sg;
        cfma(acc, cmul(mypc[slot[p]], a), X[(size_t)col[p] * nb + bb]);
    }
    red[tid] = acc;
    __syncthreads();
    for (int off = 128; off >= 8; off >>= 1) {
        if (tid < off) { red[tid].x += red[tid + off].x; red[tid].y += red[tid + off].y; }
        __syncthreads();
    }
    if (tid < 8 && b < nb) part[((size_t)li * WAE_LONG_SPLIT + k) * nb + b] = red[tid];
}
__global__ __launch_bounds__(256) void spmv_long_kernel(OpDev op, const cplx *__restrict__ pc, int cps, const cplx *__restrict__ X, int nb,
                                                        const unsigned char *__restrict__ cmask) {
    long_row_piece(op.long_ptr, op.long_col, op.long_slot, op.long_val, op.nplanes_total, op.long_conj, pc, cps, X, nb, cmask, op.long_part);
}
__global__ __launch_bounds__(256) void long_reduce_kernel(const cplx *__restrict__ part, int nrows, int nb, const int *__restrict__ map,
                                                          cplx *__restrict__ acc, const unsigned char *__restrict__ cmask) {
    const int e = blockIdx.x * 256 + threadIdx.x;
    if (e >= nrows * nb) return;
    const int i = e / nb, b = e - i * nb;
    if (cmask && !cmask[b >> 3]) return;
    cplx s = {0.0, 0.0};
    for (int k = 0; k < WAE_LONG_SPLIT; ++k) { const cplx t = part[((size_t)i * WAE_LONG_SPLIT + k) * nb + b]; s.x += t.x; s.y += t.y; }
    acc[(size_t)(map ? map[i] : i) * nb + b] = s;
}
static void launch_long_rows(const OpDev &op, const cplx *pc, int cps, const cplx *X, int nb, const unsigned char *cmask, hipStream_t st) {
    hipLaunchKernelGGL(spmv_long_kernel, dim3((unsigned)op.nlong * WAE_LONG_SPLIT, (unsigned)((nb + 7) / 8)), dim3(256), 0, st, op, pc, cps, X, nb, cmask);
    HIP_CHECK(hipGetLastError());
    hipLaunchKernelGGL(long_reduce_kernel, dim3((unsigned)((op.nlong * nb + 255) / 256)), dim3(256), 0, st, op.long_part, op.nlong, nb,
                       (const int *)nullptr, op.long_acc, cmask);
    HIP_CHECK(hipGetLastError());
}
__device__ __forceinline__ int long_row_index(const OpDev &op, int64_t row) {
    int lo = 0, hi = op.nlong - 1;
    while (lo <= hi) {
        const int mid = (lo + hi) >> 1;
        const int v = op.long_rows[mid];
        if (v == row) return mid;
        if (v < row) lo = mid + 1; else hi = mid - 1;
    }
    return -1;
}

template <int C, int S>
__global__ __launch_bounds__(256) void spmv_kernel(OpDev op, const cplx *__restrict__ pc, int cps,
                                                   const cplx *__restrict__ X, cplx *Y,
                                                   const cplx *B, double jac_w, int nb, int mode,
                                                   const unsigned char *__restrict__ cmask) {
    if (C == 8 && cmask && !cmask[blockIdx.y]) return;
    constexpr int TEAM = C * S;
    constexpr int TPB = 256 / TEAM;
    extern __shared__ cplx spc[];
    const int tid = threadIdx.x;
    const int npl = op.nplanes_total;
    for (int i = tid; i < C * npl; i += 256) {
        int cc = i / npl, q = i - cc * npl;
        int bb = blockIdx.y * C + cc;
        spc[i] = (bb < nb) ? pc[(size_t)(bb / cps) * npl + q] : cplx{0.0, 0.0};
    }
    __syncthreads();
    const int team = tid / TEAM;
    const int lt = tid - team * TEAM;
    const int c = lt % C;
    const int s = lt / C;
    const unsigned per_xcd = gridDim.x >> 3;
    const int64_t rb = (int64_t)(blockIdx.x & 7u) * per_xcd + (blockIdx.x >> 3);
    const int64_t row = rb * TPB + team;
    if (row >= op.n) return;
    const int b = blockIdx.y * C + c;
    const bool active = b < nb;
    const int bb = active ? b : nb - 1;
    const cplx *mypc = spc + c * npl;
    cplx acc = {0.0, 0.0};
#pragma unroll 1
    for (int g = 0; g < op.ngroups; ++g) {
        const GroupDev G = op.g[g];
        const int p0 = G.rowptr[row], p1 = G.rowptr[row + 1];
        const int np = G.nplanes;
        const cplx *gpc = mypc + G.plane0;
        if (G.is_real) {
            const double *__restrict__ v = (const double *)G.vals;
            if (np == 2) {
                const double2 *__restrict__ v2 = (const double2 *)G.vals;
                const cplx c0 = gpc[0], c1 = gpc[1];
                constexpr int U = 4;
                for (int p = p0 + s; p < p1; p += U * S) {
                    int j[U];
                    double2 a[U];
                    cplx x[U];
#pragma unroll
                    for (int u = 0; u < U; ++u) {
                        const int pp = p + u * S;
                        const int pc_ = pp < p1 ? pp : p1 - 1;
                        j[u] = G.col[pc_];
                        a[u] = v2[pc_];
                        if (pp >= p1) a[u] = double2{0.0, 0.0};
                    }
#pragma unroll
                    for (int u = 0; u < U; ++u) x[u] = X[(size_t)j[u] * nb + bb];
#pragma unroll
                    for (int u = 0; u < U; ++u) {
                        cplx m = {fma(c0.x, a[u].x, c1.x * a[u].y), fma(c0.y, a[u].x, c1.y * a[u].y)};
                        cfma(acc, m, x[u]);
                    }
                }
            } else {
                for (int p = p0 + s; p < p1; p += S) {
                    const int j = G.col[p];
                    cplx m = {0.0, 0.0};
                    for (int q = 0; q < np; ++q) {
                        const double a = v[(size_t)p * np + q];
                        m.x = fma(gpc[q].x, a, m.x);
                        m.y = fma(gpc[q].y, a, m.y);
                    }
                    const cplx x = X[(size_t)j * nb + bb];
                    cfma(acc, m, x);
                }
            }
        } else {
            const cplx *__restrict__ v = (const cplx *)G.vals;
            const double sg = G.conj_vals ? -1.0 : 1.0;
            for (int p = p0 + s; p < p1; p += S) {
                const int j = G.col[p];
                cplx m = {0.0, 0.0};
                for (int q = 0; q < np; ++q) {
                    cplx a = v[(size_t)p * np + q];
                    a.y *= sg;
                    cfma(m, gpc[q], a);
                }
                const cplx x = X[(size_t)j * nb + bb];
                cfma(acc, m, x);
            }
        }
    }
#pragma unroll
    for (int off = C; off < TEAM; off <<= 1) {
        acc.x += __shfl_xor(acc.x, off);
        acc.y += __shfl_xor(acc.y, off);
    }
    if (s != 0 || !active) return;
    if (op.nlong) {
        const int li = long_row_index(op, row);
        if (li >= 0) { const cplx t = op.long_acc[(size_t)li * nb + b]; acc.x += t.x; acc.y += t.y; }
    }
    const size_t e = (size_t)row * nb + b;
    cplx out;
    if (mode == MODE_AX) {
        out = acc;
    } else if (mode == MODE_RES) {
        const cplx bv = B[e];
        out = cplx{bv.x - acc.x, bv.y - acc.y};
    } else if (mode == MODE_ADD) {
        const cplx bv = B[e];
        out = cplx{bv.x + acc.x, bv.y + acc.y};
    } else {
        cplx dg = {0.0, 0.0};
        const double dsg = op.conj_diag ? -1.0 : 1.0;
        for (int q = 0; q < npl; ++q) { cplx dq = op.diag[(size_t)row * npl + q]; dq.y *= dsg; cfma(dg, mypc[q], dq); }
        if (mode == MODE_AX_DS) {
            out = cdiv(acc, dg);
        } else if (mode == MODE_RES_DS) {
            const cplx bv = B[e];
            out = cdiv(cplx{bv.x - acc.x, bv.y - acc.y}, dg);
        } else {
            const cplx bv = B[e], xv = X[e];
            cplx r = cdiv(cplx{bv.x - acc.x, bv.y - acc.y}, dg);
            out = cplx{xv.x + jac_w * r.x, xv.y + jac_w * r.y};
        }
    }
    Y[e] = out;
}

constexpr int LDS_WORDS = 2048;
constexpr int LDS_NNZ = 1024;

template <int NCH>
__global__ __launch_bounds__(256, 4) void spmv_lds_kernel(OpDev op, const cplx *__restrict__ pc, int cps,
                                                       const cplx *__restrict__ X, cplx *Y, const cplx *B, double jac_w,
                                                       int nb, int mode, const unsigned char *__restrict__ cmask) {
    constexpr int C = 8;
    constexpr int TPB = 256 / C;
    constexpr int CW = C * NCH;
    if (cmask) {
        bool any = false;
#pragma unroll
        for (int k = 0; k < NCH; ++k) {
            const int ch = blockIdx.y * NCH + k;
            if (ch * C < nb && cmask[ch]) any = true;
        }
        if (!any) return;
    }
    extern __shared__ cplx spc[];
    __shared__ __attribute__((aligned(16))) double lds_w[LDS_WORDS];
    __shared__ int lds_c[LDS_NNZ];
    const int tid = threadIdx.x;
    const int npl = op.nplanes_total;
    const int col0 = blockIdx.y * CW;
    for (int i = tid; i < CW * npl; i += 256) {
        int cc = i / npl, q = i - cc * npl;
        int bb = col0 + cc;
        spc[i] = (bb < nb) ? pc[(size_t)(bb / cps) * npl + q] : cplx{0.0, 0.0};
    }
    const int team = tid / C;
    const int c = tid - team * C;
    const unsigned per_xcd = gridDim.x >> 3;
    const int64_t rb = (int64_t)(blockIdx.x & 7u) * per_xcd + (blockIdx.x >> 3);
    const int64_t row0 = rb * TPB;
    const int64_t row = row0 + team;
    const bool valid = row < op.n;
    int bcol[NCH];
    bool act[NCH];
#pragma unroll
    for (int k = 0; k < NCH; ++k) {
        const int b = col0 + k * C + c;
        act[k] = b < nb && (!cmask || cmask[blockIdx.y * NCH + k]);
        bcol[k] = b < nb ? b : nb - 1;
    }
    cplx acc[NCH];
#pragma unroll
    for (int k = 0; k < NCH; ++k) acc[k] = cplx{0.0, 0.0};
    const int64_t rlast = (row0 + TPB < op.n) ? row0 + TPB : op.n;
    __syncthreads();
    if (row0 < op.n) {
#pragma unroll 1
        for (int g = 0; g < op.ngroups; ++g) {
            const GroupDev G = op.g[g];
            const int np = G.nplanes;
            const int wpn = G.is_real ? np : 2 * np;
            int chunk = LDS_WORDS / wpn;
            if (chunk > LDS_NNZ) chunk = LDS_NNZ;
            const int blo = G.rowptr[row0], bhi = G.rowptr[rlast];
            const int p0 = valid ? G.rowptr[row] : 0, p1 = valid ? G.rowptr[row + 1] : 0;
            const double *__restrict__ gw = (const double *)G.vals;
            const double sg = G.conj_vals ? -1.0 : 1.0;
            for (int lo = blo; lo < bhi; lo += chunk) {
                const int hi = (lo + chunk < bhi) ? lo + chunk : bhi;
                const int cnt = hi - lo;
                __syncthreads();
                for (int i = tid; i < cnt; i += 256) lds_c[i] = G.col[lo + i];
                const int nw = cnt * wpn;
                const double *src = gw + (size_t)lo * wpn;
                for (int i = tid; i < nw; i += 256) lds_w[i] = src[i];
                __syncthreads();
                const int a0 = p0 > lo ? p0 : lo, a1 = p1 < hi ? p1 : hi;
                if (G.is_real && np == 2) {
                    const double2 *lv = (const double2 *)lds_w;
                    constexpr int U = (NCH >= 4) ? 2 : 4;
                    for (int p = a0; p < a1; p += U) {
                        int j[U];
                        double2 a[U];
                        cplx x[U][NCH];
#pragma unroll
                        for (int u = 0; u < U; ++u) {
                            const int pp = (p + u < a1) ? p + u : a1 - 1;
                            j[u] = lds_c[pp - lo];
                            a[u] = lv[pp - lo];
                            if (p + u >= a1) a[u] = double2{0.0, 0.0};
                        }
#pragma unroll
                        for (int u = 0; u < U; ++u)
#pragma unroll
                            for (int k = 0; k < NCH; ++k) x[u][k] = act[k] ? X[(size_t)j[u] * nb + bcol[k]] : cplx{0.0, 0.0};
#pragma unroll
                        for (int u = 0; u < U; ++u)
#pragma unroll
                            for (int k = 0; k < NCH; ++k) {
                                const cplx *gpc = spc + (k * C + c) * npl + G.plane0;
                                const cplx c0 = gpc[0], c1 = gpc[1];
                                cplx m = {fma(c0.x, a[u].x, c1.x * a[u].y), fma(c0.y, a[u].x, c1.y * a[u].y)};
                                cfma(acc[k], m, x[u][k]);
                            }
                    }
                } else {
                    for (int p = a0; p < a1; ++p) {
                        const int j = lds_c[p - lo];
#pragma unroll
                        for (int k = 0; k < NCH; ++k) {
                            const cplx *gpc = spc + (k * C + c) * npl + G.plane0;
                            cplx m = {0.0, 0.0};
                            if (G.is_real) {
                                for (int q = 0; q < np; ++q) {
                                    const double a = lds_w[(p - lo) * np + q];
                                    m.x = fma(gpc[q].x, a, m.x);
                                    m.y = fma(gpc[q].y, a, m.y);
                                }
                            } else {
                                const cplx *lv = (const cplx *)lds_w;
                                for (int q = 0; q < np; ++q) {
                                    cplx a = lv[(p - lo) * np + q];
                                    a.y *= sg;
                                    cfma(m, gpc[q], a);
                                }
                            }
                            if (act[k]) cfma(acc[k], m, X[(size_t)j * nb + bcol[k]]);
                        }
                    }
                }
            }
        }
    }
    if (!valid) return;
    const int li_long = op.nlong ? long_row_index(op, row) : -1;
#pragma unroll
    for (int k = 0; k < NCH; ++k) {
        if (!act[k]) continue;
        const int b = col0 + k * C + c;
        if (li_long >= 0) { const cplx t = op.long_acc[(size_t)li_long * nb + b]; acc[k].x += t.x; acc[k].y += t.y; }
        const cplx *mypc = spc + (k * C + c) * npl;
        const size_t e = (size_t)row * nb + b;
        cplx out;
        if (mode == MODE_AX) {
            out = acc[k];
        } else if (mode == MODE_RES) {
            const cplx bv = B[e];
            out = cplx{bv.x - acc[k].x, bv.y - acc[k].y};
        } else if (mode == MODE_ADD) {
            const cplx bv = B[e];
            out = cplx{bv.x + acc[k].x, bv.y + acc[k].y};
        } else {
            cplx dg = {0.0, 0.0};
            const double dsg = op.conj_diag ? -1.0 : 1.0;
            for (int q = 0; q < npl; ++q) { cplx dq = op.diag[(size_t)row * npl + q]; dq.y *= dsg; cfma(dg, mypc[q], dq); }
            if (mode == MODE_AX_J0) {
                out = acc[k];
                const cplx r = cdiv(acc[k], dg);
                const_cast<cplx *>(B)[e] = cplx{jac_w * r.x, jac_w * r.y};
            } else if (mode == MODE_AX_DS) {
                out = cdiv(acc[k], dg);
            } else if (mode == MODE_RES_DS) {
                const cplx bv = B[e];
                out = cdiv(cplx{bv.x - acc[k].x, bv.y - acc[k].y}, dg);
            } else {
                const cplx bv = B[e], xv = X[e];
                cplx r = cdiv(cplx{bv.x - acc[k].x, bv.y - acc[k].y}, dg);
                out = cplx{xv.x + jac_w * r.x, xv.y + jac_w * r.y};
            }
        }
        Y[e] = out;
    }
}

__global__ __launch_bounds__(256) void spmv_side_kernel(TileDev td, int npl, int conj, const cplx *__restrict__ pc, int cps,
                                                        const cplx *__restrict__ X, int nb, const unsigned char *__restrict__ cmask) {
    const int ch = blockIdx.y;
    if (cmask && !cmask[ch]) return;
    const int i = blockIdx.x * 32 + (threadIdx.x >> 3), b = ch * 8 + (threadIdx.x & 7);
    if (i >= td.nside || b >= nb) return;
    const cplx *mypc = pc + (size_t)(b / cps) * npl;
    const double sg = conj ? -1.0 : 1.0;
    cplx acc = {0.0, 0.0};
    const int beg = td.side_ptr[i], end = td.side_ptr[i + 1];
    for (int p0 = beg; p0 < end; p0 += 8) {
        int c[8], sl[8];
        cplx a[8], x[8];
#pragma unroll
        for (int u = 0; u < 8; ++u) {
            const int p = p0 + u < end ? p0 + u : end - 1;
            c[u] = td.side_col[p]; sl[u] = td.side_slot[p]; a[u] = td.side_val[p];
        }
#pragma unroll
        for (int u = 0; u < 8; ++u) x[u] = X[(size_t)c[u] * nb + b];
#pragma unroll
        for (int u = 0; u < 8; ++u)
            if (p0 + u < end) { a[u].y *= sg; cfma(acc, cmul(mypc[sl[u]], a[u]), x[u]); }
    }
    td.side_acc[(size_t)i * nb + b] = acc;
}

__global__ __launch_bounds__(256) void spmv_side_long_kernel(TileDev td, int npl, int conj, const cplx *__restrict__ pc, int cps,
                                                             const cplx *__restrict__ X, int nb, const unsigned char *__restrict__ cmask) {
    long_row_piece(td.ls_ptr, td.ls_col, td.ls_slot, td.ls_val, npl, conj, pc, cps, X, nb, cmask, td.ls_part);
}

#ifdef WAE_TILE_STAMPS
__device__ unsigned long long wae_tile_stamps[8 * 64 + 8];
#ifndef TILE_STAMP_WG
#define TILE_STAMP_WG 101
#endif
__device__ unsigned long long wae_tile_wglog[1024 * 4];
#ifndef TILE_STAMP_FIRST
#define TILE_STAMP_FIRST 21
#endif
#define TILE_STAMP(k) do { if (blockIdx.x == TILE_STAMP_WG && tid == 0 && nstamp >= TILE_STAMP_FIRST && nstamp < TILE_STAMP_FIRST + 8) { \
                               wae_tile_stamps[(nstamp - TILE_STAMP_FIRST) * 8 + (k)] = __builtin_amdgcn_s_memtime(); \
                               if ((k) == 0) wae_tile_stamps[(nstamp - TILE_STAMP_FIRST) * 8 + 7] = __builtin_amdgcn_s_memrealtime(); } } while (0)
#else
#define TILE_STAMP(k) do { } while (0)
#endif
template <int CTRL> __device__ __forceinline__ double lane_quad(double v) {
    const int lo = __builtin_amdgcn_mov_dpp(__double2loint(v), CTRL, 0xF, 0xF, true);
    const int hi = __builtin_amdgcn_mov_dpp(__double2hiint(v), CTRL, 0xF, 0xF, true);
    return __hiloint2double(hi, lo);
}
template <int CTRL, int BANKS> __device__ __forceinline__ double lane_dpp_masked(double old, double src) {
    const int lo = __builtin_amdgcn_update_dpp(__double2loint(old), __double2loint(src), CTRL, 0xF, BANKS, false);
    const int hi = __builtin_amdgcn_update_dpp(__double2hiint(old), __double2hiint(src), CTRL, 0xF, BANKS, false);
    return __hiloint2double(hi, lo);
}
template <bool UNI, int LPR, int NBUF, int NWV = 8, int KRT = (LPR == 2 ? 8 : 12)>
__global__ __launch_bounds__(64 * NWV, NWV == 8 ? 1 : 4) void spmv_tile_kernel(OpDev op, TileDev td, const cplx *__restrict__ pc, int cps,
                                                          const cplx *__restrict__ X, cplx *Y, const cplx *B, double jac_w,
                                                          int nb, int mode, const unsigned char *__restrict__ cmask, int spc_all, int csplit) {
    extern __shared__ __attribute__((aligned(16))) unsigned char tile_smem[];
    const int tid = threadIdx.x;
#ifdef WAE_TILE_STAMPS
    if (blockIdx.x == TILE_STAMP_WG && tid == 0) wae_tile_stamps[64] = __builtin_amdgcn_s_memtime();
    if (tid == 0 && blockIdx.x < 1024) {
        wae_tile_wglog[blockIdx.x * 4] = __builtin_amdgcn_s_memrealtime();
        wae_tile_wglog[blockIdx.x * 4 + 3] = (unsigned long long)__builtin_amdgcn_s_getreg(63492) | ((unsigned long long)__builtin_amdgcn_s_getreg(63508) << 32);
    }
#endif
    const int nch_all = (nb + 7) >> 3;
    const int npl = op.nplanes_total;
    const int wslots = (td.wmax + 7) & ~7;
    cplx *const smem = (cplx *)tile_smem;
    cplx *spc0 = smem + (size_t)wslots * 8 * NBUF;
    const int lane = tid & 63, wv = __builtin_amdgcn_readfirstlane(tid >> 6);
    constexpr int RPW = 64 / LPR;
    constexpr int NOUT = 8 / LPR;
    const int sub = lane & (LPR - 1);
    const int rot = LPR == 2 ? (lane >> 1) & 7 : (((lane >> 2) & 1) + 2 * sub) & 7;
    const int rot_out = LPR == 2 ? (rot + 4 * sub) & 7 : rot;
    const int tpx = (td.ntiles + 7) >> 3;
    const int xcd = (int)(blockIdx.x & 7u), gpx = (int)(gridDim.x >> 3);
    auto next_active = [&](int c, int end) { while (c < end && cmask && !cmask[c]) ++c; return c; };
    auto share_tiles = [&](int x) { const int left = td.ntiles - x * tpx; return left < tpx ? (left > 0 ? left : 0) : tpx; };
    auto share_split = [&](int x) { const int n = share_tiles(x); return csplit > 1 ? (n < gpx ? n : gpx) : 0; };
    auto share_size = [&](int x) { return share_tiles(x) + share_split(x) * (csplit - 1); };
    auto decode = [&](int item, int &tile_, int &ch_, int &end_) {
        const int x = item >> 24, p = item & 0xFFFFFF;
        const int nfull = share_tiles(x) - share_split(x);
        int part = 0, parts = 1;
        if (p < nfull) tile_ = x * tpx + p;
        else { const int q = p - nfull; tile_ = x * tpx + nfull + q / csplit; part = q - (q / csplit) * csplit; parts = csplit; }
        end_ = (part + 1) * nch_all / parts;
        ch_ = next_active(part * nch_all / parts, end_);
        return ch_ < end_;
    };
    auto draw = [&](int pend) {
        int t_, c_, e_;
        if (pend >= 0 && pend < share_size(xcd) && decode(xcd << 24 | pend, t_, c_, e_)) return xcd << 24 | pend;
        for (int a = 0; a < 8; ++a) {
            const int x2 = (xcd + a) & 7, lim = share_size(x2);
            while (gpx < lim) {
                const int p = gpx + (int)atomicAdd(td.counters + x2, 1u);
                if (p >= lim) break;
                if (decode(x2 << 24 | p, t_, c_, e_)) return x2 << 24 | p;
            }
        }
        return -1;
    };
    int *const vt_slot = (int *)(spc0 + (size_t)(spc_all ? nch_all * 8 : 8) * npl);
    auto leave = [&]() {
        if (tid == 0 && atomicAdd(td.counters + 8, 1u) == gridDim.x - 1)
            for (int i = 0; i < 9; ++i) atomicExch(td.counters + i, 0u);
    };
    int tile, ch, ch_end;
    {
        const int p0 = (int)(blockIdx.x >> 3);
        bool ok = p0 < share_size(xcd) && decode(xcd << 24 | p0, tile, ch, ch_end);
        if (!ok) {
            if (tid == 0) *vt_slot = draw(-1);
            __syncthreads();
            const int vt = *vt_slot;
            __syncthreads();
            ok = vt >= 0 && decode(vt, tile, ch, ch_end);
        }
        if (!ok) { leave(); return; }
    }
    constexpr int KR = KRT;
    constexpr int WSTEP = 8 * NWV;
    constexpr int NTHR = 64 * NWV;
    constexpr int NW = NBUF > 2 ? 7 : 640 / WSTEP;
    constexpr bool QUAD = NWV == 16;
    static_assert(!QUAD || (LPR == 4 && UNI && NBUF == 2 && KRT == 8), "QUAD: LPR = 4, one system per chunk, two buffers, 8 entries per lane");
    const int qh = lane & 1, qc = (lane >> 1) & 1, qrot = (lane >> 2) & 3;
    constexpr bool COAL = UNI && LPR == 2 && NBUF == 2 && !QUAD;
    const bool he = ((sub ^ rot) & 1) != 0;
    auto ocol = [&](int j) { return QUAD ? 4 * qc + ((2 * qh + j + qrot) & 3) : COAL ? (2 * j + (he ? 1 : 0) + rot) & 7 : (rot_out + j) & 7; };
    auto tcol = [&](int k) { return (2 * ((lane >> 1) & 3) + ((lane ^ k) & 1) + ((4 * (lane >> 3) + k) & 7)) & 7; };
    auto transpose4 = [&](cplx (&R)[4]) {
        const bool odd = ((lane >> 1) & 1) != 0;
#pragma unroll
        for (int m0 = 0; m0 < 4; m0 += 2) {
            const double sx = odd ? R[m0].x : R[m0 + 1].x, sy = odd ? R[m0].y : R[m0 + 1].y;
// ... 99 lines not shown
    load_list(gr, w0, W);
    load_matrix();
    int buf = 0;
    bool wn0 = false, wn1 = false, wn2 = false;
    if (spc_all)
        for (int i = tid; i < nch_all * 8 * npl; i += NTHR) {
            const int cc = i / npl, q = i - cc * npl;
            spc0[i] = pc[(size_t)((cc < nb ? cc : nb - 1) / cps) * npl + q];
        }
    int nx = 0;
    unsigned pend = 0;
    bool pub_fresh = false;
    int tile_n = 0, ch_n = 0, ch_end_n = 0;
    bool has_next = false;
    {
        if (tid == 0) *vt_slot = draw(-1);
        __syncthreads();
        const int vt = *vt_slot;
        has_next = vt >= 0 && decode(vt, tile_n, ch_n, ch_end_n);
    }
    int s00_n = 0, n0_n = 0, w0_n = 0, W_n = 0, r0_n = 0, nrows_n = 0;
    bool sc_ready = false;
    bool pre_ready = false;
    bool pre_asked = false;
    int pre_raw[6];
#pragma unroll
    for (int u = 0; u < 6; ++u) pre_raw[u] = 0;
#ifdef WAE_TILE_STAMPS
    if (blockIdx.x == TILE_STAMP_WG && tid == 0) wae_tile_stamps[65] = __builtin_amdgcn_s_memtime();
    int nstamp = 0;
#endif
    while (true) {
        const int c1o = next_active(ch + 1, ch_end);
        const bool same = c1o < ch_end;
        const bool v1 = same || has_next;
        const bool n1 = !same;
        const int c1 = same ? c1o : ch_n;
        int c2 = 0;
        bool v2 = false, n2 = false;
        if (NBUF > 2) {
            if (same) {
                const int c2o = next_active(c1o + 1, ch_end);
                if (c2o < ch_end) { v2 = true; c2 = c2o; }
                else if (has_next) { v2 = true; n2 = true; c2 = ch_n; }
            } else if (has_next) {
                const int c2o = next_active(ch_n + 1, ch_end_n);
                if (c2o < ch_end_n) { v2 = true; n2 = true; c2 = c2o; }
            }
        }
        const int col0 = ch * 8;
        TILE_STAMP(0);
        cplx *spc = spc0 + (spc_all ? (size_t)col0 * npl : 0);
        if (!wn0) {
            if (pre_ready) { load_list(gr, w0, W); pre_ready = false; }
            __syncthreads();
            issue_window(ch, buf, gr, w0, W);
            TILE_DMA_WAIT();
            wn0 = true;
        }
        __syncthreads();
        if (!spc_all) {
            for (int i = tid; i < 8 * npl; i += NTHR) {
                const int cc = i / npl, q = i - cc * npl;
                int bb = col0 + cc;
                if (bb >= nb) bb = nb - 1;
                spc[i] = pc[(size_t)(bb / cps) * npl + q];
            }
            __syncthreads();
        }
        cplx *win = smem + (size_t)buf * wslots * 8;
        TILE_STAMP(1);
        pub_fresh = false;
        if (nx == 0) {
            if (has_next) {
                if (tid == 0 && gpx < share_size(xcd)) pend = atomicAdd(td.counters + xcd, 1u);
                request_scalars(tile_n, pre_raw);
                pre_asked = true;
            }
            nx = 1;
        }
        const int lrow = wv * RPW + lane / LPR;
        const bool live = lrow < nrows;
        const int64_t row = r0 + (live ? lrow : 0);
        const bool need_b = mode == MODE_RES || mode == MODE_ADD || mode == MODE_RES_DS || mode == MODE_JAC;
        const bool need_d = !(mode == MODE_AX || mode == MODE_RES || mode == MODE_ADD);
        const double dsg = op.conj_diag ? -1.0 : 1.0;
        cplx bv[NOUT], xv[NOUT];
        cplx dgu = {1.0, 0.0};
        auto trow = [&](int k) { return wv * RPW + 4 * (lane >> 3) + k; };
        auto b_loads = [&]() {
#pragma unroll
            for (int k = 0; k < 4; ++k) {
                const int lr = trow(k) < nrows ? trow(k) : (nrows > 0 ? nrows - 1 : 0);
                const int c = tcol(k);
                const int b = col0 + c < nb ? col0 + c : nb - 1;
                bv[k] = need_b ? B[(size_t)(r0 + lr) * nb + b] : cplx{0.0, 0.0};
            }
        };
        auto epilogue_loads = [&]() {
#pragma unroll
            for (int j = 0; j < NOUT; ++j) {
                const int c = ocol(j);
                const int b = col0 + c < nb ? col0 + c : nb - 1;
                const size_t e = (size_t)row * nb + b;
                if constexpr (!COAL) bv[j] = need_b ? B[e] : cplx{0.0, 0.0};
                xv[j] = (mode == MODE_JAC && dslot == 0xFFFFu) ? X[e] : cplx{0.0, 0.0};
            }
            if (UNI && need_d) {
                dgu = cplx{0.0, 0.0};
                for (int q = 0; q < npl; ++q) { cplx dq = op.diag[(size_t)row * npl + q]; dq.y *= dsg; cfma(dgu, spc[q], dq); }
            }
        };
        constexpr bool SPLIT = !UNI;
        constexpr bool FOLD = NBUF > 2 && !SPLIT;
        cplx acc[8], acc2[8];
#pragma unroll
        for (int s = 0; s < 8; ++s) { acc[s] = cplx{0.0, 0.0}; acc2[s] = cplx{0.0, 0.0}; }
        if constexpr (COAL) b_loads();
        if (NBUF > 2) {
            epilogue_loads();
            const double sb = mode == MODE_ADD ? 1.0 : -1.0;
#pragma unroll
            for (int j = 0; j < NOUT; ++j) {
                if (!FOLD) continue;
                if (LPR == 2) {
                    acc[j] = cplx{sub == 0 ? sb * bv[j].x : 0.0, sub == 0 ? sb * bv[j].y : 0.0};
                    acc[j + 4] = cplx{sub == 1 ? sb * bv[j].x : 0.0, sub == 1 ? sb * bv[j].y : 0.0};
                } else {
                    acc[j] = cplx{sb * bv[j].x, sb * bv[j].y};
                }
            }
        }
        if (NBUF > 2 && !wn1 && v1 && (n1 ? pre_ready : !pre_ready)) {
            issue_window(c1, (buf + 1) % NBUF, gr, n1 ? w0_n : w0, n1 ? W_n : W);
            wn1 = true;
        }
        const bool vt_ = NBUF > 2 ? v2 : v1, nt_ = NBUF > 2 ? n2 : n1;
        const bool already = NBUF > 2 ? wn2 : wn1;
        const bool more = vt_ && !already && (nt_ ? pre_ready : !pre_ready);
        const int ct = NBUF > 2 ? c2 : c1;
        const cplx *Xn = window_src(more ? ct : ch);
        const int Wd = nt_ ? W_n : W;
        const int bt = (buf + NBUF - 1) % NBUF;
        TILE_STAMP(2);
        constexpr bool HALVES = SPLIT && LPR == 2;
        cplx res[NOUT];
#pragma unroll
        for (int j = 0; j < NOUT; ++j) res[j] = cplx{0.0, 0.0};
        if (HALVES && n0 > 0) {
            const unsigned short *__restrict__ si = T0.sidx;
            const double2 *__restrict__ v2 = (const double2 *)T0.svals;
            auto half_pass = [&](auto HC) {
                constexpr int H = decltype(HC)::value;
                cplx p[4], q[4];
#pragma unroll
                for (int s = 0; s < 4; ++s) { p[s] = cplx{0.0, 0.0}; q[s] = cplx{0.0, 0.0}; }
                auto fetch4 = [&](cplx (&x)[4], unsigned ix) {
                    const cplx *wr = win + ix * 8;
#pragma unroll
                    for (int s = 0; s < 4; ++s) x[s] = wr[(4 * H + s + rot) & 7];
                };
                auto apply4 = [&](const cplx (&x)[4], double2 a) {
#pragma unroll
                    for (int s = 0; s < 4; ++s) {
                        p[s].x = fma(a.x, x[s].x, p[s].x); p[s].y = fma(a.x, x[s].y, p[s].y);
                        q[s].x = fma(a.y, x[s].x, q[s].x); q[s].y = fma(a.y, x[s].y, q[s].y);
                    }
                };
                unsigned ixs = 0;
                double2 avs = {0.0, 0.0};
                if (n0 > KR) { const int e = s00 + lane + 64 * KR; ixs = si[e]; avs = v2[e]; }
                cplx xa[4], xb[4];
                fetch4(xa, ixr[0]);
#pragma unroll
                for (int u = 0; u < KR; ++u) {
                    if (u + 1 < KR) { if (u & 1) fetch4(xa, ixr[u + 1]); else fetch4(xb, ixr[u + 1]); }
                    __builtin_amdgcn_sched_barrier(0);
                    if (u & 1) apply4(xb, avr[u]); else apply4(xa, avr[u]);
                    asm volatile("" : "+v"(p[0].x), "+v"(p[0].y), "+v"(p[1].x), "+v"(p[1].y), "+v"(p[2].x), "+v"(p[2].y), "+v"(p[3].x), "+v"(p[3].y),
                                      "+v"(q[0].x), "+v"(q[0].y), "+v"(q[1].x), "+v"(q[1].y), "+v"(q[2].x), "+v"(q[2].y), "+v"(q[3].x), "+v"(q[3].y)
                                 : : "memory");
                    __builtin_amdgcn_sched_barrier(0);
                    if (H == 0 && more && 2 * u < NW) {
                        issue_piece(Xn, bt, gr, Wd, 2 * u);
                        if (2 * u + 1 < NW) issue_piece(Xn, bt, gr, Wd, 2 * u + 1);
                    }
                }
                if (H == 0 && more) issue_rest(Xn, bt, nt_ ? w0_n : w0, Wd);
#pragma unroll 1
                for (int k = KR; k < n0; ++k) {
                    const unsigned ixc = ixs;
                    const double2 avc = avs;
                    if (k + 1 < n0) { const int e = s00 + lane + 64 * (k + 1); ixs = si[e]; avs = v2[e]; }
                    cplx x[4];
                    fetch4(x, ixc);
                    apply4(x, avc);
                }
#pragma unroll
                for (int j = 0; j < 4; ++j) {
                    const cplx P = {p[j].x + lane_quad<0xB1>(p[j].x), p[j].y + lane_quad<0xB1>(p[j].y)};
                    const cplx Q = {q[j].x + lane_quad<0xB1>(q[j].x), q[j].y + lane_quad<0xB1>(q[j].y)};
                    const int cs = (4 * H + j + rot) & 7;
                    const cplx d0 = spc[cs * npl + G0.plane0], d1 = spc[cs * npl + G0.plane0 + 1];
                    cplx t = {0.0, 0.0};
                    cfma(t, d0, P);
                    cfma(t, d1, Q);
                    if (sub == H) res[j] = t;
                }
            };
            half_pass(std::integral_constant<int, 0>{});
            half_pass(std::integral_constant<int, 1>{});
        } else if (HALVES) {
// ... 36 lines not shown
                } else {
                    if (u > 0) fetch(xa, ixr[u]);
                    apply(xa, avr[u]);
                }
                if constexpr (QUAD)
                    asm volatile("" : "+v"(acc[0].x), "+v"(acc[0].y), "+v"(acc[1].x), "+v"(acc[1].y), "+v"(acc[2].x), "+v"(acc[2].y),
                                      "+v"(acc[3].x), "+v"(acc[3].y) : : "memory");
                else
                asm volatile("" : "+v"(acc[0].x), "+v"(acc[0].y), "+v"(acc[1].x), "+v"(acc[1].y), "+v"(acc[2].x), "+v"(acc[2].y),
                                  "+v"(acc[3].x), "+v"(acc[3].y), "+v"(acc[4].x), "+v"(acc[4].y), "+v"(acc[5].x), "+v"(acc[5].y),
                                  "+v"(acc[6].x), "+v"(acc[6].y), "+v"(acc[7].x), "+v"(acc[7].y) : : "memory");
                if (SPLIT)
                    asm volatile("" : "+v"(acc2[0].x), "+v"(acc2[0].y), "+v"(acc2[1].x), "+v"(acc2[1].y), "+v"(acc2[2].x), "+v"(acc2[2].y),
                                      "+v"(acc2[3].x), "+v"(acc2[3].y), "+v"(acc2[4].x), "+v"(acc2[4].y), "+v"(acc2[5].x), "+v"(acc2[5].y),
                                      "+v"(acc2[6].x), "+v"(acc2[6].y), "+v"(acc2[7].x), "+v"(acc2[7].y) : : "memory");
                __builtin_amdgcn_sched_barrier(0);
                if (more && 2 * u < NW) {
                    issue_piece(Xn, bt, gr, Wd, 2 * u);
                    if (2 * u + 1 < NW) issue_piece(Xn, bt, gr, Wd, 2 * u + 1);
                }
            }
            if (more) issue_rest(Xn, bt, nt_ ? w0_n : w0, Wd);
#pragma unroll 1
            for (int k = KR; k < n0; ++k) {
                const unsigned ixc = ixs;
                const double2 avc = avs;
                if (k + 1 < n0) { const int e = s00 + mlane + 64 * (k + 1); ixs = si[e]; avs = v2[e]; }
                cplx x[8];
                fetch(x, ixc);
                apply(x, avc);
            }
        } else if (more) {
            issue_window(ct, bt, gr, nt_ ? w0_n : w0, Wd);
        }
        if (more) { if (NBUF > 2) wn2 = true; else wn1 = true; }
        TILE_STAMP(3);
        auto meet = [&](const cplx (&a)[8], cplx (&r)[NOUT]) {
            if constexpr (QUAD) {
#pragma unroll
                for (int j = 0; j < NOUT; ++j) {
                    const cplx lo = {a[j].x + lane_quad<0xB1>(a[j].x), a[j].y + lane_quad<0xB1>(a[j].y)};
                    const cplx hi = {a[j + 2].x + lane_quad<0xB1>(a[j + 2].x), a[j + 2].y + lane_quad<0xB1>(a[j + 2].y)};
                    r[j] = qh ? hi : lo;
                }
            } else
            if (LPR == 2) {
#pragma unroll
                for (int j = 0; j < NOUT; ++j) {
                    const cplx lo = {a[j].x + lane_quad<0xB1>(a[j].x), a[j].y + lane_quad<0xB1>(a[j].y)};
                    const cplx hi = {a[j + 4].x + lane_quad<0xB1>(a[j + 4].x), a[j + 4].y + lane_quad<0xB1>(a[j + 4].y)};
                    r[j] = sub ? hi : lo;
                }
            } else {
#pragma unroll
                for (int j = 0; j < NOUT; ++j)
                    r[j] = cplx{a[j].x + lane_quad<0x93>(a[j + 2].x) + lane_quad<0x4E>(a[j + 4].x) + lane_quad<0x39>(a[j + 6].x),
                                a[j].y + lane_quad<0x93>(a[j + 2].y) + lane_quad<0x4E>(a[j + 4].y) + lane_quad<0x39>(a[j + 6].y)};
            }
        };
        if constexpr (COAL) {
#pragma unroll
            for (int m = 0; m < 4; ++m) {
                const double sx = he ? acc[2 * m].x : acc[2 * m + 1].x, sy = he ? acc[2 * m].y : acc[2 * m + 1].y;
                const double mx = he ? acc[2 * m + 1].x : acc[2 * m].x, my = he ? acc[2 * m + 1].y : acc[2 * m].y;
                res[m] = cplx{mx + lane_quad<0xB1>(sx), my + lane_quad<0xB1>(sy)};
            }
        } else if (!HALVES) meet(acc, res);
        if (SPLIT && !HALVES) {
            cplx res2[NOUT];
            meet(acc2, res2);
#pragma unroll
            for (int j = 0; j < NOUT; ++j) {
                const int cs = (rot_out + j) & 7;
                const cplx d0 = td.unit ? cplx{1.0, 0.0} : spc[cs * npl + G0.plane0], d1 = td.unit ? cplx{0.0, 0.0} : spc[cs * npl + G0.plane0 + 1];
                cplx t = {0.0, 0.0};
                cfma(t, d0, res[j]);
                cfma(t, d1, res2[j]);
                res[j] = t;
            }
        }
        TILE_STAMP(4);
        if (NBUF == 2) epilogue_loads();
        if constexpr (COAL) { if (need_b) transpose4(bv); }
        if (mode == MODE_JAC && dslot != 0xFFFFu) {
#pragma unroll
            for (int j = 0; j < NOUT; ++j) xv[j] = win[dslot * 8 + ocol(j)];
        }
        if (side >= 0) {
#pragma unroll
            for (int j = 0; j < NOUT; ++j) {
                const int c = ocol(j);
                const int b = col0 + c < nb ? col0 + c : nb - 1;
                const cplx sv = td.side_acc[(size_t)side * nb + b];
                res[j].x += sv.x; res[j].y += sv.y;
            }
        }
        cplx out[NOUT], b2[NOUT];
#pragma unroll
        for (int j = 0; j < NOUT; ++j) {
            const int c = ocol(j);
            const cplx av = res[j];
            b2[j] = cplx{0.0, 0.0};
            const cplx bz = FOLD ? cplx{0.0, 0.0} : bv[j];
            if (mode == MODE_AX) {
                out[j] = av;
            } else if (mode == MODE_RES) {
                out[j] = cplx{bz.x - av.x, bz.y - av.y};
            } else if (mode == MODE_ADD) {
                out[j] = cplx{bz.x + av.x, bz.y + av.y};
            } else {
                cplx dg = dgu;
                if (!UNI) {
                    const cplx *mypc = spc + c * npl;
                    dg = cplx{0.0, 0.0};
                    for (int q = 0; q < npl; ++q) { cplx dq = op.diag[(size_t)row * npl + q]; dq.y *= dsg; cfma(dg, mypc[q], dq); }
                }
                if (mode == MODE_AX_J0) {
                    out[j] = av;
                    const cplx r = cdiv(av, dg);
                    b2[j] = cplx{jac_w * r.x, jac_w * r.y};
                } else if (mode == MODE_AX_DS) {
                    out[j] = cdiv(av, dg);
                } else if (mode == MODE_RES_DS) {
                    out[j] = cdiv(cplx{bz.x - av.x, bz.y - av.y}, dg);
                } else {
                    const cplx r = cdiv(cplx{bz.x - av.x, bz.y - av.y}, dg);
                    out[j] = cplx{xv[j].x + jac_w * r.x, xv[j].y + jac_w * r.y};
                }
            }
        }
        TILE_STAMP(5);
        if (NBUF > 2 && more) dma_wait_but(pieces_of(Wd)); else TILE_DMA_WAIT();
        if (nx == 1) {
            if (tid == 0 && has_next) *vt_slot = draw(gpx < share_size(xcd) ? gpx + (int)pend : -1);
            nx = 2;
            pub_fresh = true;
        }
        if (pre_asked) {
            take_scalars(pre_raw, s00_n, n0_n, w0_n, W_n, r0_n, nrows_n);
            pre_asked = false;
            sc_ready = true;
        }
        if (sc_ready && !pre_ready && has_next && same) {
            int left = 0;
            for (int c = next_active(c1o + 1, ch_end); c < ch_end && left < NBUF; c = next_active(c + 1, ch_end)) ++left;
            if (left < NBUF - 1) { load_list(gr, w0_n, W_n); pre_ready = true; }
        }
        if constexpr (COAL) {
            transpose4(out);
            if (mode == MODE_AX_J0) transpose4(b2);
#pragma unroll
            for (int k = 0; k < 4; ++k) {
                const int b = col0 + tcol(k);
                if (trow(k) >= nrows || b >= nb) continue;
                const size_t e = (size_t)(r0 + trow(k)) * nb + b;
                typedef double dv2_t __attribute__((ext_vector_type(2)));
                __builtin_nontemporal_store(dv2_t{out[k].x, out[k].y}, (dv2_t *)(Y + e));
                if (mode == MODE_AX_J0) __builtin_nontemporal_store(dv2_t{b2[k].x, b2[k].y}, (dv2_t *)(const_cast<cplx *>(B) + e));
            }
        } else
        if (live) {
#pragma unroll
            for (int j = 0; j < NOUT; ++j) {
                const int b = col0 + ocol(j);
                if (b >= nb) continue;
                const size_t e = (size_t)row * nb + b;
                Y[e] = out[j];
                if (mode == MODE_AX_J0) const_cast<cplx *>(B)[e] = b2[j];
            }
        }
        TILE_STAMP(6);
#ifdef WAE_TILE_STAMPS
        ++nstamp;
#endif
        buf = (buf + 1) % NBUF;
        wn0 = wn1; wn1 = wn2; wn2 = false;
        if (same) {
            ch = c1o;
        } else {
            if (!has_next) break;
            if (!pre_ready) {
                if (!sc_ready) load_scalars(tile_n, s00_n, n0_n, w0_n, W_n, r0_n, nrows_n);
                load_list(gr, w0_n, W_n);
            }
            tile = tile_n; ch = ch_n; ch_end = ch_end_n;
            s00 = s00_n; n0 = n0_n; w0 = w0_n; W = W_n; r0 = r0_n; nrows = nrows_n;
            load_matrix();
            pre_ready = false;
            sc_ready = false;
            if (pub_fresh) __syncthreads();
            {
                const int vt = *vt_slot;
                has_next = vt >= 0 && decode(vt, tile_n, ch_n, ch_end_n);
            }
            nx = 0;
        }
    }
    leave();
#ifdef WAE_TILE_STAMPS
    if (blockIdx.x == TILE_STAMP_WG && tid == 0) { TILE_DMA_WAIT(); wae_tile_stamps[66] = __builtin_amdgcn_s_memtime(); }
    if (tid == 0 && blockIdx.x < 1024) { wae_tile_wglog[blockIdx.x * 4 + 1] = __builtin_amdgcn_s_memrealtime(); wae_tile_wglog[blockIdx.x * 4 + 2] = nstamp; }
#endif
}

#ifdef WAE_TILE_STAMPS
extern "C" int wae_debug_tile_wglog(unsigned long long *out) {
    return (int)hipMemcpyFromSymbol(out, HIP_SYMBOL(wae_tile_wglog), sizeof(unsigned long long) * 1024 * 4);
}
extern "C" int wae_debug_tile_stamps(unsigned long long *out) {
    return (int)hipMemcpyFromSymbol(out, HIP_SYMBOL(wae_tile_stamps), sizeof(unsigned long long) * (8 * 64 + 8));
}
#endif
static void launch_spmv_tile(const OpDev &op, const TileDev &td, const cplx *pc, int cps, const cplx *X, cplx *Y, const cplx *B, double jac_w,
                             int nb, int mode, hipStream_t st, const unsigned char *cmask) {
    const int nbuf = td.nbuf == 3 && td.lpr == 2 ? 3 : 2;
    const size_t wslots = (size_t)((td.wmax + 7) & ~7);
    const int nch8 = ((nb + 7) / 8) * 8;
    size_t shm = nbuf * wslots * 8 * sizeof(cplx) + (size_t)nch8 * op.nplanes_total * sizeof(cplx) + 16;
    const int spc_all = shm <= 160 * 1024;
    if (!spc_all) shm = nbuf * wslots * 8 * sizeof(cplx) + (size_t)8 * op.nplanes_total * sizeof(cplx) + 16;
    if (shm > 160 * 1024) throw WaeError(WAE_ERR_INVALID, "tile windows do not fit LDS (WAE_TILE_WCAP too large)");
    static OncePerDevice lds_opt_in;
    static int ncu_dev[64] = {0};
    const int dev_now = once_per_device(lds_opt_in, [](int dev) {
        const void *fns[] = {(const void *)spmv_tile_kernel<true, 2, 2>, (const void *)spmv_tile_kernel<false, 2, 2>,
                             (const void *)spmv_tile_kernel<true, 2, 3>, (const void *)spmv_tile_kernel<false, 2, 3>,
                             (const void *)spmv_tile_kernel<true, 4, 2>, (const void *)spmv_tile_kernel<false, 4, 2>,
                             (const void *)spmv_tile_kernel<true, 4, 2, 16, 8>};
        for (const void *fn : fns) HIP_CHECK(hipFuncSetAttribute(fn, hipFuncAttributeMaxDynamicSharedMemorySize, 160 * 1024));
        int ncu = 0;
        HIP_CHECK(hipDeviceGetAttribute(&ncu, hipDeviceAttributeMultiprocessorCount, dev));
        if (getenv("WAE_TILE_GRID")) ncu = atoi(getenv("WAE_TILE_GRID"));
        ncu_dev[dev & 63] = ncu < 8 ? 8 : ncu & ~7;
    });
    const int ncu = ncu_dev[dev_now & 63];
    const int nchunks = (nb + 7) / 8;
    int csplit = td.ntiles < ncu ? (int)((ncu + td.ntiles - 1) / td.ntiles)
                                 : std::min(getenv("WAE_TILE_TAIL") ? atoi(getenv("WAE_TILE_TAIL")) : 4, std::max(1, nchunks / 2));
    if (csplit > nchunks) csplit = nchunks;
    if (csplit < 1) csplit = 1;
    const unsigned tpx = (unsigned)((td.ntiles + 7) / 8);
    const unsigned units = std::min<unsigned>(tpx, (unsigned)(ncu / 8)) * (unsigned)csplit + (tpx > (unsigned)(ncu / 8) ? tpx - (unsigned)(ncu / 8) : 0u);
    const dim3 grid(8u * std::min(units, (unsigned)(ncu / 8)));
    if (td.nside) {
        if (nb > 256) throw WaeError(WAE_ERR_INVALID, "launch_spmv: batch wider than 256 columns");
        hipLaunchKernelGGL(spmv_side_kernel, dim3((unsigned)((td.nside + 31) / 32), (unsigned)nchunks), dim3(256), 0, st, td, op.nplanes_total,
                           op.conj_diag, pc, cps, X, nb, cmask);
        HIP_CHECK(hipGetLastError());
        if (td.nlong_side) {
            hipLaunchKernelGGL(spmv_side_long_kernel, dim3((unsigned)td.nlong_side * WAE_LONG_SPLIT, (unsigned)nchunks), dim3(256), 0, st, td,
                               op.nplanes_total, op.conj_diag, pc, cps, X, nb, cmask);
            HIP_CHECK(hipGetLastError());
            hipLaunchKernelGGL(long_reduce_kernel, dim3((unsigned)((td.nlong_side * nb + 255) / 256)), dim3(256), 0, st, td.ls_part, td.nlong_side, nb,
                               td.ls_side, td.side_acc, cmask);
            HIP_CHECK(hipGetLastError());
        }
    }
#define WAE_TILE_LAUNCH(U, L, N) hipLaunchKernelGGL((spmv_tile_kernel<U, L, N>), grid, dim3(512), shm, st, op, td, pc, cps, X, Y, B, jac_w, nb, mode, cmask, spc_all, csplit)
    static const int waves16 = getenv("WAE_TILE_WAVES") ? atoi(getenv("WAE_TILE_WAVES")) == 16 : 0;
    if (waves16 && td.lpr == 2 && nbuf == 2 && cps % 8 == 0 && !td.unit)
        hipLaunchKernelGGL((spmv_tile_kernel<true, 4, 2, 16, 8>), grid, dim3(1024), shm, st, op, td, pc, cps, X, Y, B, jac_w, nb, mode, cmask, spc_all, csplit);
    else
    if (td.lpr == 4) { if (cps % 8 == 0) WAE_TILE_LAUNCH(true, 4, 2); else WAE_TILE_LAUNCH(false, 4, 2); }
    else if (nbuf == 3) { if (cps % 8 == 0) WAE_TILE_LAUNCH(true, 2, 3); else WAE_TILE_LAUNCH(false, 2, 3); }
    else { if (cps % 8 == 0) WAE_TILE_LAUNCH(true, 2, 2); else WAE_TILE_LAUNCH(false, 2, 2); }
#undef WAE_TILE_LAUNCH
    HIP_CHECK(hipGetLastError());
}

typedef void (*spmv_fn)(OpDev, const cplx *, int, const cplx *, cplx *, const cplx *, double, int, int, const unsigned char *);
template <int C, int S> static spmv_fn spmv_ptr() { return spmv_kernel<C, S>; }

static spmv_fn pick_spmv(int C, int S) {
#define PICK(c, s_) if (C == c && S == s_) return spmv_ptr<c, s_>();
    PICK(1, 1) PICK(1, 2) PICK(1, 4) PICK(1, 8) PICK(1, 16) PICK(1, 32)
    PICK(2, 1) PICK(2, 2) PICK(2, 4) PICK(2, 8) PICK(2, 16)
    PICK(4, 1) PICK(4, 2) PICK(4, 4) PICK(4, 8) PICK(4, 16)
    PICK(8, 1) PICK(8, 2) PICK(8, 4) PICK(8, 8)
    PICK(16, 1) PICK(16, 2) PICK(16, 4)
#undef PICK
    return nullptr;
}

static int env_int(const char *name, int dflt) {
    const char *e = getenv(name);
    return e ? atoi(e) : dflt;
}

void launch_spmv(const OpDev &op, const cplx *pc, int cps, const cplx *X, cplx *Y, const cplx *B, double jac_w,
                 int nb, int mode, hipStream_t st, const unsigned char *cmask) {
    const int envC = env_int("WAE_SPMV_C", 0), envS = env_int("WAE_SPMV_S", 0);
    int C = nb >= 8 ? 8 : (nb >= 4 ? 4 : (nb >= 2 ? 2 : 1));
    int S = 64 / C >= 8 ? 8 : 64 / C;
    if (C == 8) S = 1;
    if (C == 8 && op.n < env_int("WAE_SPMV_SMALL8", 4096)) S = 8;
    else if (C == 8 && op.n < env_int("WAE_SPMV_SMALL4", 65536)) S = 4;
    else if (C < 8 && op.n >= env_int("WAE_SPMV_SMALL4", 65536)) S = 8 / C;
    if (envC > 0 && envC <= nb) C = envC;
    if (envS > 0) S = envS;
    if (op.n <= 0) return;
    if (op.tiles && nb >= 8 && envC == 0 && envS == 0 && env_int("WAE_SPMV_TILE", 1)) {
        launch_spmv_tile(op, *op.tiles, pc, cps, X, Y, B, jac_w, nb, mode, st, cmask);
        return;
    }
    if (op.nlong) {
        if (nb > 256) throw WaeError(WAE_ERR_INVALID, "launch_spmv: batch wider than 256 columns");
        launch_long_rows(op, pc, cps, X, nb, nb >= 8 ? cmask : (const unsigned char *)nullptr, st);
    }
    if (mode == MODE_AX_J0 && !(C == 8 && S == 1 && env_int("WAE_SPMV_LDS", 1))) {
        launch_spmv(op, pc, cps, X, Y, nullptr, 0.0, nb, MODE_AX, st, cmask);
        launch_jacobi0(op, pc, cps, Y, const_cast<cplx *>(B), jac_w, nb, st, cmask);
        return;
    }
    if (C == 8 && S == 1 && env_int("WAE_SPMV_LDS", 1)) {
        const int nch_env = env_int("WAE_SPMV_NCH", 0);
        int nchunks = (nb + 7) / 8;
        int NCH = nch_env > 0 ? nch_env : (nchunks >= 4 ? 4 : (nchunks >= 2 ? 2 : 1));
        const unsigned nrb = (unsigned)((op.n + 31) / 32);
        dim3 grid((nrb + 7u) / 8u * 8u, (unsigned)((nb + 8 * NCH - 1) / (8 * NCH)));
        size_t shm = (size_t)8 * NCH * op.nplanes_total * sizeof(cplx);
        if (NCH == 8) hipLaunchKernelGGL(spmv_lds_kernel<8>, grid, dim3(256), shm, st, op, pc, cps, X, Y, B, jac_w, nb, mode, cmask);
        else if (NCH == 4) hipLaunchKernelGGL(spmv_lds_kernel<4>, grid, dim3(256), shm, st, op, pc, cps, X, Y, B, jac_w, nb, mode, cmask);
        else if (NCH == 2) hipLaunchKernelGGL(spmv_lds_kernel<2>, grid, dim3(256), shm, st, op, pc, cps, X, Y, B, jac_w, nb, mode, cmask);
        else hipLaunchKernelGGL(spmv_lds_kernel<1>, grid, dim3(256), shm, st, op, pc, cps, X, Y, B, jac_w, nb, mode, cmask);
        HIP_CHECK(hipGetLastError());
        return;
    }
    spmv_fn fn = pick_spmv(C, S);
    if (!fn) throw WaeError(WAE_ERR_INVALID, "launch_spmv: unsupported (C,S)");
    const int tpb = 256 / (C * S);
    const unsigned nrb = (unsigned)((op.n + tpb - 1) / tpb);
    dim3 grid((nrb + 7u) / 8u * 8u, (unsigned)((nb + C - 1) / C));
    size_t shm = (size_t)C * op.nplanes_total * sizeof(cplx);
    hipLaunchKernelGGL(fn, grid, dim3(256), shm, st, op, pc, cps, X, Y, B, jac_w, nb, mode, C == 8 ? cmask : (const unsigned char *)nullptr);
    HIP_CHECK(hipGetLastError());
}

__global__ __launch_bounds__(256) void jacobi0_kernel(OpDev op, const cplx *__restrict__ pc, int cps,
                                                      const cplx *__restrict__ B, cplx *__restrict__ X, double w, int nb,
                                                      const unsigned char *__restrict__ cmask) {
    const size_t total = (size_t)op.n * nb;
    const int npl = op.nplanes_total;
    for (size_t e = (size_t)blockIdx.x * 256 + threadIdx.x; e < total; e += (size_t)gridDim.x * 256) {
        const size_t row = e / nb;
        const int b = (int)(e - row * nb);
        if (cmask && !cmask[b >> 3]) continue;
        const cplx *mypc = pc + (size_t)(b / cps) * npl;
        cplx dg = {0.0, 0.0};
        const double dsg = op.conj_diag ? -1.0 : 1.0;
        for (int q = 0; q < npl; ++q) { cplx dq = op.diag[row * npl + q]; dq.y *= dsg; cfma(dg, mypc[q], dq); }
        cplx r = cdiv(B[e], dg);
        X[e] = cplx{w * r.x, w * r.y};
    }
}

__device__ __forceinline__ cplx prolong_row(const int *__restrict__ ptr, const int *__restrict__ col, const double *__restrict__ val,
                                            const cplx *__restrict__ Xc, cplx acc, size_t row, int b, int nb) {
    const int p0 = ptr[row], p1 = ptr[row + 1];
    int p = p0;
    for (; p + 4 <= p1; p += 4) {
        cplx v[4];
        double a[4];
#pragma unroll
        for (int u = 0; u < 4; ++u) { a[u] = val[p + u]; v[u] = Xc[(size_t)col[p + u] * nb + b]; }
#pragma unroll
        for (int u = 0; u < 4; ++u) { acc.x += a[u] * v[u].x; acc.y += a[u] * v[u].y; }
    }
    for (; p < p1; ++p) {
        const double a = val[p];
        const cplx v = Xc[(size_t)col[p] * nb + b];
        acc.x += a * v.x; acc.y += a * v.y;
    }
    return acc;
}
__global__ __launch_bounds__(256) void prolong_add_kernel(const int *__restrict__ ptr, const int *__restrict__ col, const double *__restrict__ val,
                                                          const cplx *__restrict__ Xc, const cplx *X, cplx *Y, size_t total, int nb,
                                                          const unsigned char *__restrict__ cmask) {
    for (size_t e = (size_t)blockIdx.x * 256 + threadIdx.x; e < total; e += (size_t)gridDim.x * 256) {
        const size_t row = e / nb;
        const int b = (int)(e - row * nb);
        if (cmask && !cmask[b >> 3]) continue;
        Y[e] = prolong_row(ptr, col, val, Xc, X[e], row, b, nb);
    }
}
__global__ __launch_bounds__(256) void prolong_add_norm_kernel(const int *__restrict__ ptr, const int *__restrict__ col, const double *__restrict__ val,
                                                               const cplx *__restrict__ Xc, const cplx *X, cplx *Y, int64_t n, int nb,
                                                               const unsigned char *__restrict__ cmask, cplx *__restrict__ partial) {
    __shared__ double sm[256];
    const int tid = threadIdx.x;
    const int R = 256 / nb;
    const int b = tid % nb, rl = tid / nb;
    const bool live = rl < R && !(cmask && !cmask[b >> 3]);
    double nrm2 = 0.0;
    if (live)
        for (int64_t row = (int64_t)blockIdx.x * R + rl; row < n; row += (int64_t)gridDim.x * R) {
            const size_t e = (size_t)row * nb + b;
            const cplx acc = prolong_row(ptr, col, val, Xc, X[e], (size_t)row, b, nb);
            if (Y) Y[e] = acc;
            nrm2 += acc.x * acc.x + acc.y * acc.y;
        }
    nrm2 = nb <= 64 && (nb & (nb - 1)) == 0 ? block_colsum<true, 256>(nrm2, nb, sm) : block_colsum<false, 256>(nrm2, nb, sm);
    if (tid < nb) partial[(size_t)blockIdx.x * nb + tid] = cplx{nrm2, 0.0};
}
template <bool NORM>
__global__ __launch_bounds__(256) void prolong_tiles_kernel(XferTilesDev T, const cplx *__restrict__ Xc, const cplx *X, cplx *Y, int nb,
                                                            const unsigned char *__restrict__ cmask, cplx *__restrict__ partial) {
    extern __shared__ __attribute__((aligned(16))) unsigned char xt_smem[];
    __shared__ double nsm[NORM ? 32 : 1];
    const int t = blockIdx.x, tid = threadIdx.x;
    if (NORM)
        for (int bb = tid; bb < nb; bb += 256)
            if (cmask && !cmask[bb >> 3]) partial[(size_t)t * nb + bb] = cplx{0.0, 0.0};
    const int col = tid & 7, rl = tid >> 3;
    const int nch = (nb + 7) >> 3;
    const int s0 = T.tptr[t], ns = T.tptr[t + 1] - s0;
    const int r0 = T.row_ptr[t], nr = T.row_ptr[t + 1] - r0;
    const int e0 = T.pptr[r0], ne = T.pptr[r0 + nr] - e0;
    cplx *const sl = (cplx *)xt_smem;
    double *const ev = (double *)(sl + (size_t)T.maxslots * 8);
    int *const ep = (int *)(ev + T.maxent);
    unsigned short *const el = (unsigned short *)(ep + 260);
    for (int i = tid; i < ne; i += 256) { ev[i] = T.pval[e0 + i]; el[i] = T.ploc[e0 + i]; }
// ... 352 lines not shown
```

wavesandeigenvalues.jl_amd/csrc/solver.h:

```cpp
#pragma once
#include "family.h"

void upload_pc(wae_family *h, const std::vector<std::vector<zc>> &pcs);
const cplx *pc_level(const wae_family *h, int l);
void dense_setup(wae_family *h, const Batch &bt);
double pre_weight(const wae_family *h);
struct CycleNorms { cplx *out; bool only; bool done = false; };
cplx *vcycle(wae_family *h, const Batch &bt, int l, const cplx *b, const unsigned char *cm = nullptr, bool have_x0 = false,
             cplx *final_out = nullptr, CycleNorms *cn = nullptr);
void penalty_polish(wae_family *h, const Batch &bt, const cplx *B, cplx *X);
int gmres(wae_family *h, const Batch &bt, const cplx *B, cplx *X, double tol, int maxit, wae_solve_info *info, const cplx *guess_dir = nullptr,
          bool have_x0 = false, double *relres_out = nullptr);
int solve_chunk(wae_family *h, const Batch &bt, const std::vector<std::vector<zc>> &pcs, const cplx *B, cplx *X, double tol, int maxit,
                wae_solve_info *info, const cplx *guess_dir = nullptr, bool have_x0 = false);
struct CallInfo {
    wae_solve_info li{};
    double t0 = now_s();
    int finish(wae_solve_info *out);
};

cplx *slot_col(wae_family *h, int32_t slot, int32_t col);
const cplx *slot_cols_ptr(wae_family *h, int32_t slot, const int32_t *cols, int n, DevBuf<cplx> &stage, hipStream_t st);
```

wavesandeigenvalues.jl_amd/csrc/wae_internal.h:

```cpp
#pragma once
#include <hip/hip_runtime.h>
#include <algorithm>
#include <cmath>
#include <complex>
#include <cstdint>
#include <cstdio>
#include <cstring>
#include <stdexcept>
#include <string>
#include <vector>

#include "../../include/waehip.h"

typedef std::complex<double> zc;
typedef double2 cplx;

struct WaeError : std::runtime_error {
    int code;
    WaeError(int c, const std::string &m) : std::runtime_error(m), code(c) {}
};
void wae_set_error(const std::string &m);
int wae_internal_device(const wae_family *h);
hipStream_t wae_internal_stream(const wae_family *h);

// ... 155 lines not shown
    std::vector<GroupHost> groups;
    DevBuf<cplx> diag;
    TileStore tiles;
    LongRows long_n, long_t;
    OpDev dev(int op) const;
    std::vector<CsrZ> planes;
};

struct XferTilesDev {
    int ntiles = 0, maxslots = 0, maxent = 0;
    int64_t nslots = 0, nf = 0, nc = 0;
    const int *row_ptr = nullptr;
    const int *tptr = nullptr;
    const int *clist = nullptr;
    const int *pptr = nullptr;
    const unsigned short *ploc = nullptr;
    const double *pval = nullptr;
};
struct XferTiles {
    DevBuf<int> row_ptr, tptr, clist, pptr;
    DevBuf<unsigned short> ploc;
    DevBuf<double> pval;
    XferTilesDev dev;
    bool ready = false;
};
void launch_prolong_tiles(const XferTilesDev &T, const cplx *Xc, const cplx *X, cplx *Y, int nb, hipStream_t s, const unsigned char *cmask = nullptr,
                          cplx *partial = nullptr, cplx *norms = nullptr);

struct Transfer {
    int64_t nf = 0, nc = 0;
    DevBuf<int> p_ptr, p_col, r_ptr, r_col;
    DevBuf<double> p_val, r_val;
    XferTiles ft;
    TileStore r_tiles;
    OpDev devP() const;
    OpDev devR() const;
};

struct P1Handle {
    int64_t np = 0, nnz = 0;
    std::vector<int> rowptr, col;
    std::vector<double> m, k;
};
template <class T> struct Dev {
    T *p = nullptr;
    explicit Dev(size_t n) { HIP_CHECK(hipMalloc((void **)&p, std::max<size_t>(n, 1) * sizeof(T))); }
    Dev(const Dev &) = delete;
    Dev &operator=(const Dev &) = delete;
    ~Dev() { if (p) (void)hipFree(p); }
};
P1Handle *triplets_to_csr(int64_t npoints, size_t ne, Dev<unsigned long long> &k0, Dev<double> &mv, Dev<double> *kv);
struct TripletCsr {
    int64_t np = 0;
    int nnz = 0;
    DevBuf<int> rowptr, col;
    DevBuf<double> m, k;
};
void triplets_to_csr_dev(int64_t npoints, size_t ne, Dev<unsigned long long> &k0, Dev<double> &mv, Dev<double> *kv, TripletCsr &out);

struct DevPlane {
    int64_t n = 0, nnz = 0;
    bool real = true;
    DevBuf<int> ptr, col;
    DevBuf<double> re, im;
};
struct DevProlongator {
    int64_t n = 0, m = 0, nnz = 0;
    DevBuf<int> ptr, col;
    DevBuf<double> val;
};
constexpr int64_t WAE_GALERKIN_MAX_TRIPLETS = 2147483647;
void upload_plane(const CsrZ &A, DevPlane &D);
void upload_prolongator(const CsrD &P, DevProlongator &D);
int64_t galerkin_device(const DevPlane &A, const DevProlongator &P, DevPlane &C, CsrZ &host);
void pairs_to_dense(int64_t n, size_t ne, Dev<unsigned long long> &k0, Dev<double> &v, double *out);
void p2_check_tets(int64_t npoints, int64_t ntets, const int32_t *tets);
int64_t p2_edge_list(int64_t npoints, int64_t nt, const int *dtets, Dev<unsigned long long> &ek);
inline void check_c_point(int64_t npoints, const double *c_point) {
    if (!c_point) throw WaeError(WAE_ERR_INVALID, "c_point is required: one speed of sound per mesh point");
    for (int64_t i = 0; i < npoints; ++i)
        if (!std::isfinite(c_point[i])) throw WaeError(WAE_ERR_INVALID, "c_point holds a value that is not finite");
}

enum { MODE_AX = 0, MODE_RES = 1, MODE_JAC = 2, MODE_ADD = 3, MODE_AX_DS = 4, MODE_RES_DS = 5, MODE_AX_J0 = 6 };
void launch_spmv(const OpDev &op, const cplx *pc, int cps, const cplx *X, cplx *Y, const cplx *B, double jac_w,
                 int nb, int mode, hipStream_t s, const unsigned char *cmask = nullptr);
void launch_jacobi0(const OpDev &op, const cplx *pc, int cps, const cplx *B, cplx *X, double jac_w, int nb, hipStream_t s,
                    const unsigned char *cmask = nullptr);
void launch_spmv_multi(const OpDev &op, const cplx *pc, const int *plane_col, const cplx *X, cplx *Y, int nb, hipStream_t s);

void launch_dense_assemble(const cplx *planes, int nplanes, int n, const cplx *pc, int nsys, int op,
                           cplx *Ainv, hipStream_t s);
void launch_dense_invert(cplx *Ainv, int n, int nsys, int *status, hipStream_t s);
void launch_dense_apply(const cplx *Ainv, int n, int cps, const cplx *X, cplx *Y, int nb, hipStream_t s, const unsigned char *cmask = nullptr);

void launch_fill_zero(cplx *X, size_t count, hipStream_t s);
void launch_copy(const cplx *X, cplx *Y, size_t count, hipStream_t s);
void launch_dots(const cplx *V, size_t stride, int nv, const cplx *W, int64_t n, int nb, cplx *partial, cplx *out, hipStream_t s,
                 const unsigned char *cmask = nullptr);
void launch_axpy_neg_multi(const cplx *V, size_t stride, int nv, const cplx *h, cplx *W, size_t wstride, int cnt, int64_t n, int nb, hipStream_t s);
void launch_axpy_neg(const cplx *V, size_t stride, int nv, const cplx *h, cplx *W, int64_t n, int nb, hipStream_t s,
                     const unsigned char *cmask = nullptr);
void launch_axpy_neg_norm(const cplx *V, size_t stride, int nv, const cplx *h, cplx *W, int64_t n, int nb, cplx *partial, cplx *norms,
                          hipStream_t s, const unsigned char *cmask = nullptr, const cplx *base = nullptr, cplx *inv_out = nullptr);
void launch_dots_scaled(const cplx *V, size_t stride, int nv, const cplx *W, int64_t n, int nb, cplx *partial, cplx *out, const cplx *scale,
                        hipStream_t s, const unsigned char *cmask = nullptr);
void launch_lincomb(const cplx *V, size_t stride, int nv, const cplx *y, cplx *Y, int64_t n, int nb, hipStream_t s);
void launch_lincomb_add(const cplx *V, size_t stride, int nv, const cplx *y, cplx *X, int64_t n, int nb, hipStream_t s);
void launch_norms(const cplx *X, int64_t n, int nb, cplx *partial, cplx *out, hipStream_t s, const unsigned char *cmask = nullptr);
void launch_scale_inv(const cplx *X, const cplx *alpha, cplx *Y, int64_t n, int nb, hipStream_t s, const unsigned char *cmask = nullptr);
void launch_axpby1(cplx a, const cplx *x, cplx b, const cplx *y, cplx *out, size_t n, hipStream_t s, int conj_x = 0);
void launch_add(const cplx *X, cplx *Y, size_t count, hipStream_t s);
void launch_colmajor_to_inter(const cplx *Xc, int64_t d, int r, cplx *Xi, int nb, hipStream_t s, const int *perm = nullptr);
void launch_inter_to_colmajor(const cplx *Xi, int nb, int64_t d, int r, cplx *Xc, hipStream_t s, const int *perm = nullptr);
void launch_replicate(const cplx *Vc, int64_t d, int l, cplx *Xi, int nb, hipStream_t s, const int *perm = nullptr);
constexpr int PROLONG_NORM_BLOCKS = 1024;
void launch_prolong_add(const int *ptr, const int *col, const double *val, int64_t n, const cplx *Xc, const cplx *X, cplx *Y, int nb, hipStream_t s,
                        const unsigned char *cmask = nullptr, cplx *partial = nullptr, cplx *norms = nullptr);
void launch_reduce_partials(const cplx *partial, int nblk, int count, cplx *out, int do_sqrt, hipStream_t s, const cplx *scale = nullptr,
                            cplx *inv_out = nullptr);
void launch_dots_multi(const cplx *V, size_t sv, int nv, const cplx *W, size_t sw, int nw, int64_t n, int nb, cplx *partial, cplx *out,
                       hipStream_t s);
void launch_gather_rows(const cplx *X, const int *rows, int64_t nrows, int nb, cplx *out, hipStream_t s);
void launch_scatter_add_rows(const cplx *D, const int *rows, int64_t nrows, int nb, cplx *X, hipStream_t s);
void launch_extract_cols(const cplx *X, int nb, int off, int l, cplx *out, int64_t n, hipStream_t s);
void launch_lincomb_rep(const cplx *Q, size_t stride, int nv, const cplx *y, cplx *X, int64_t n, int nb, int l, hipStream_t s);
void launch_mask_cols(cplx *X, const cplx *keep, int64_t n, int nb, hipStream_t s);
void launch_beyn_accum(const cplx *Xi, int nb, int64_t d, int l, int nsys, const cplx *w, const cplx *z, int npow, cplx *A, hipStream_t s,
                       int lA = 0, int c0 = 0, const int *perm = nullptr);
void launch_pt_gemm_batch(const cplx *V, size_t stride, int k, const cplx *G, cplx *U, int64_t d, int T, int nb, hipStream_t s);
void launch_pt_spmv_batch(const OpDev &op, const cplx *pc, const int *plane_col, const cplx *U, int nin, cplx *Y, int nb, int accumulate,
                          hipStream_t s);
void launch_pt_axpby_cols(const cplx *coef, const cplx *x, const cplx *y, cplx *out, int64_t d, int nb, hipStream_t s);
void launch_pt_project(cplx *vk, const cplx *v0, const cplx *dots, int nd, int64_t d, int nb, hipStream_t s);
struct GmresDev {
    int nb, m, histcap;
    cplx *R;
    double *cs;
    cplx *sn;
    cplx *g;
    double *sv;
    cplx *vsq;
    int *conv, *steps, *iters, *histlen, *stalled;
    double *relres, *bnorm;
    double *hist;
    cplx *rescale;
    int *status;
    unsigned char *cmask;
    cplx *Hraw;
    double *sub;
};
void launch_gmres_init(const GmresDev &S, const cplx *beta, const unsigned char *done, int use_mask, hipStream_t s);
void launch_gmres_step(const GmresDev &S, const cplx *hd, int j, double tol, double lim, int use_mask, cplx *Vnew, int64_t n, hipStream_t s,
                       const cplx *rn = nullptr);
void launch_dots2_scaled(const cplx *V, size_t stride, int nv, const cplx *W1, const cplx *W2, int64_t n, int nb, cplx *partial, cplx *out1,
                         cplx *out2, cplx *gram_out, const cplx *scale, hipStream_t s, const unsigned char *cmask = nullptr);
void launch_axpy2_norm(const cplx *V, size_t stride, int nv, const cplx *c1, const cplx *c2m, const cplx *alpha, cplx *W1, cplx *W2, int64_t n, int nb,
                       cplx *partial, cplx *norms, cplx *inv_out, hipStream_t s, const unsigned char *cmask = nullptr);
void launch_gmres_pair_coef(const GmresDev &S, int j, const cplx *c1, const cplx *c2, const cplx *gram, cplx *alpha, cplx *c2m, cplx *hd2, hipStream_t s);
void launch_gmres_solve_y(const GmresDev &S, int ju, cplx *out, hipStream_t s);
void launch_forced_rhs(const int *rows, const cplx *M, int64_t nr, int nsrc, const cplx *G, cplx *B, int nb, hipStream_t s);
void launch_forced_observe(const int64_t *ptr, const int *idx, const cplx *val, int nobs, const cplx *X, int nb, cplx *H, int64_t j0, hipStream_t s);
void launch_triad(double *a, const double *b, const double *c, double s, int64_t n, hipStream_t st, unsigned grid_cap = 8192);
```

wavesandeigenvalues.jl_amd/nlevp/linopfam.py:

```python
from __future__ import annotations

import copy
import ctypes as C
from math import factorial

import numpy as np
import scipy.sparse as sp

from .. import _lib
from .._lib import OP_C, OP_N, SolveInfo, check, zptr

NaN = complex(float("nan"), float("nan"))


class Term:

    def __init__(self, coeff, func, params, symbol="", operator=""):
        if isinstance(symbol, str) and operator == "" and symbol != "":
            operator, symbol = symbol, ""
        self.coeff = coeff
        self.func = tuple(func)
        self.params = tuple(tuple(p) for p in params)
        self.symbol = symbol
        self.operator = operator
# ... 338 lines not shown
        dc, dcp = self._icols(dst_cols)
        sc, scp = self._icols(src_cols)
        n = len(dc)
        assert len(sc) == n
        a = np.ascontiguousarray(np.broadcast_to(np.asarray(alpha, dtype=np.complex128), (n,)))
        b = np.ascontiguousarray(np.broadcast_to(np.asarray(beta, dtype=np.complex128), (n,)))
        check(_lib.lib().wae_slot_axpby(self.handle, n, int(dst_slot), dcp, int(src_slot), scp, zptr(a), zptr(b), 1 if conj_src else 0))

    def slot_forms(self, coeffs, a_slot, a_cols, b_slot, b_cols, op=OP_N):
        ac, acp = self._icols(a_cols)
        bc, bcp = self._icols(b_cols)
        n = len(ac)
        assert len(bc) == n
        c = np.ascontiguousarray(np.broadcast_to(np.asarray(coeffs, dtype=np.complex128).reshape(-1, self.T), (n, self.T)))
        out = np.zeros(n, dtype=np.complex128)
        check(_lib.lib().wae_slot_forms(self.handle, n, zptr(c), int(op), int(a_slot), acp, int(b_slot), bcp, zptr(out)))
        return out

    def arnoldi_slots(self, coeffsA, coeffsM, m, v0_slot, v0_cols, op=OP_N, tol=1e-12, maxit=300, ritz_tol=0.0, quiet=False):
        cA = np.ascontiguousarray(coeffsA, dtype=np.complex128).reshape(-1, self.T)
        nsys = cA.shape[0]
        cM = np.ascontiguousarray(np.broadcast_to(np.asarray(coeffsM, dtype=np.complex128).reshape(-1, self.T), (nsys, self.T)))
        vc, vcp = self._icols(v0_cols)
        assert len(vc) == nsys
        H = np.zeros((nsys, m, m + 1), dtype=np.complex128)
        info = SolveInfo()
        code = check(_lib.lib().wae_arnoldi_shiftinvert_slots(self.handle, nsys, zptr(cA), zptr(cM), m, int(v0_slot), vcp, op, tol, maxit,
                                                              float(ritz_tol), zptr(H), C.byref(info)))
        self._report(code, info, "arnoldi_slots", quiet=quiet)
        return H.transpose(0, 2, 1)

    def ritz_to_slot(self, Y, dst_slot, dst_cols, normalise=True):
        Yc = np.ascontiguousarray(Y, dtype=np.complex128)
        nsys, ny = Yc.shape
        dc, dcp = self._icols(dst_cols)
        assert len(dc) == nsys
        check(_lib.lib().wae_arnoldi_ritz_to_slot(self.handle, nsys, ny, zptr(Yc), int(dst_slot), dcp, 1 if normalise else 0))

    def perturb_slots(self, coeff_table, N, v_slot, v_col, vadj_slot, vadj_col, norm_mode=1, coeffsY=None, tol=1e-12, maxit=400, quiet=False,
                      vectors=False):
        ct = np.ascontiguousarray(coeff_table, dtype=np.complex128).reshape((N + 1) * (N + 1), self.T)
        lam = np.zeros(N + 1, dtype=np.complex128)
        V = np.zeros((self.d, N + 1), dtype=np.complex128, order="F") if vectors else None
        cy = None if coeffsY is None else np.ascontiguousarray(coeffsY, dtype=np.complex128)
        info = SolveInfo()
        code = check(_lib.lib().wae_perturb_slots(self.handle, zptr(ct), N, int(v_slot), int(v_col), int(vadj_slot), int(vadj_col), norm_mode,
                                                  None if cy is None else zptr(cy), tol, maxit, zptr(lam), None if V is None else zptr(V),
                                                  C.byref(info)))
        self._report(code, info, f"perturb_slots (order {N})", quiet=quiet)
        return lam, V

    def perturb_batch(self, coeff_tables, N, V0=None, V0adj=None, slots=None, norm_mode=1, coeffsY=None, tol=1e-12, maxit=400, quiet=False,
                      vectors=True):
        ct = np.ascontiguousarray(coeff_tables, dtype=np.complex128).reshape(-1, (N + 1) * (N + 1) * self.T)
        nsys = ct.shape[0]
        lam = np.zeros((nsys, N + 1), dtype=np.complex128)
        want_v = vectors and not (norm_mode & 16)
        V = np.zeros((nsys, N + 1, self.d), dtype=np.complex128) if want_v else None
        status = np.zeros(max(nsys, 1), dtype=np.int32)
        sp_ = status.ctypes.data_as(C.POINTER(C.c_int32))
        cy = None if coeffsY is None else np.ascontiguousarray(coeffsY, dtype=np.complex128)
        cyp = None if cy is None else zptr(cy)
        vp = None if V is None else zptr(V)
        info = SolveInfo()
        if slots is None:
            v0 = np.asfortranarray(np.asarray(V0, dtype=np.complex128).reshape(self.d, -1))
            va = np.asfortranarray(np.asarray(V0adj, dtype=np.complex128).reshape(self.d, -1))
            if v0.shape[1] != nsys or va.shape[1] != nsys:
                raise ValueError("perturb_batch: one right and one left vector per coefficient table")
            code = check(_lib.lib().wae_perturb_batch(self.handle, nsys, zptr(ct), N, zptr(v0), zptr(va), norm_mode, cyp, tol, maxit, zptr(lam), vp,
                                                      sp_, C.byref(info)))
        else:
            v_slot, v_cols, w_slot, w_cols = slots
            vc, vcp = self._icols(v_cols)
            wc, wcp = self._icols(w_cols)
            if len(vc) != nsys or len(wc) != nsys:
                raise ValueError("perturb_batch: one right and one left slot column per coefficient table")
            code = check(_lib.lib().wae_perturb_batch_slots(self.handle, nsys, zptr(ct), N, int(v_slot), vcp, int(w_slot), wcp, norm_mode, cyp, tol,
                                                            maxit, zptr(lam), vp, sp_, C.byref(info)))
        self.last_status = status[:nsys].copy()
        self._report(code, info, f"perturb_batch ({nsys} systems, order {N})", quiet=quiet)
        return lam, (None if V is None else V.transpose(0, 2, 1)), self.last_status

    def debug_spmv(self, coeffs, X, mode=0, B=None, Y0=None, op=OP_N, jac_w=0.8, cmask=None, level=0, which=0, no_tiles=False):
        lib = _lib.lib()
        nin, nout = C.c_int64(0), C.c_int64(0)
        check(lib.wae_debug_spmv(self.handle, which, level, 0, None, 0, None, None, None, None, 0, op, 0.0, None, 0, C.byref(nin), C.byref(nout)))
        c = np.ascontiguousarray(coeffs, dtype=np.complex128).reshape(-1, self.T)
        Xf = np.asfortranarray(np.asarray(X, dtype=np.complex128).reshape(nin.value, -1))
        r = Xf.shape[1]
        Y = np.zeros((nout.value, r), dtype=np.complex128, order="F") if Y0 is None else np.asfortranarray(np.array(Y0, dtype=np.complex128))
        Bf = None if B is None else np.asfortranarray(np.asarray(B, dtype=np.complex128).reshape(nout.value, r))
        B2 = np.zeros((nout.value, r), dtype=np.complex128, order="F") if mode == 6 else None
        if mode == 6 and Y0 is not None:
            B2[...] = Y0
        cm = None if cmask is None else (C.c_uint8 * ((r + 7) // 8))(*[1 if x else 0 for x in cmask])
        check(lib.wae_debug_spmv(self.handle, which, level, mode, zptr(c), c.shape[0], zptr(Xf), None if Bf is None else zptr(Bf), zptr(Y),
                                 None if B2 is None else zptr(B2), r, op, float(jac_w), cm, 1 if no_tiles else 0, C.byref(nin), C.byref(nout)))
        return (Y, B2) if mode == 6 else Y

    def debug_prolong(self, X, B, Y0=None, level=0, cmask=None, no_tiles=False, norms_only=False):
        nin, nout = C.c_int64(0), C.c_int64(0)
        check(_lib.lib().wae_debug_spmv(self.handle, 2, level, 0, None, 0, None, None, None, None, 0, 0, 0.0, None, 0, C.byref(nin), C.byref(nout)))
        nf = nout.value
        Bf = np.asfortranarray(np.asarray(B, dtype=np.complex128).reshape(nf, -1))
        r = Bf.shape[1]
        Xf = np.asfortranarray(np.asarray(X, dtype=np.complex128).reshape(nin.value, r))
        Y = np.zeros((nf, r), dtype=np.complex128, order="F") if Y0 is None else np.asfortranarray(np.array(Y0, dtype=np.complex128).reshape(nf, r))
        norms = np.zeros(r)
        cm = None if cmask is None else (C.c_uint8 * ((r + 7) // 8))(*[1 if x else 0 for x in cmask])
        check(_lib.lib().wae_debug_prolong(self.handle, level, zptr(Xf), zptr(Bf), zptr(Y), norms.ctypes.data_as(C.POINTER(C.c_double)), r, cm,
                                           (1 if no_tiles else 0) | (2 if norms_only else 0)))
        return Y, norms

    def level_sizes(self):
        out = []
        lib = _lib.lib()
        for which in (0, 1):
            lv = 0
            while True:
                nin, nout = C.c_int64(0), C.c_int64(0)
                if lib.wae_debug_spmv(self.handle, which, lv, 0, None, 0, None, None, None, None, 0, 0, 0.0, None, 0, C.byref(nin), C.byref(nout)) != 0:
                    break
                out.append((which, lv, nin.value, nout.value))
                lv += 1
        return out

    def debug_vcycle(self, coeffs, B, level=0, Y0=None, op=OP_N, light=False, final_out=False, fused=False, cmask=None):
        c = np.ascontiguousarray(coeffs, dtype=np.complex128).reshape(-1, self.T)
        B = np.asarray(B, dtype=np.complex128)
        Bf = np.asfortranarray(B if B.ndim == 2 else B.reshape(-1, 1))
        n, r = Bf.shape
        if level == 0 and n != self.d:
            raise ValueError(f"debug_vcycle: B has {n} rows, the family {self.d}")
        Y = np.zeros((n, r), dtype=np.complex128, order="F") if Y0 is None else np.asfortranarray(np.array(Y0, dtype=np.complex128).reshape(n, r))
        cm = None if cmask is None else (C.c_uint8 * ((r + 7) // 8))(*[1 if x else 0 for x in cmask])
        flags = (1 if light else 0) | (2 if final_out else 0) | (4 if fused else 0)
        check(_lib.lib().wae_debug_vcycle(self.handle, level, zptr(c), c.shape[0], zptr(Bf), zptr(Y), r, op, flags, cm))
        return Y

    def bench_spmv_level(self, coeffs, which=0, level=1, r=64, reps=20):
        c = np.ascontiguousarray(coeffs, dtype=np.complex128)
        ms, nbytes = C.c_double(0), C.c_int64(0)
        check(_lib.lib().wae_bench_spmv_level(self.handle, zptr(c), which, level, r, reps, C.byref(ms), C.byref(nbytes)))
        return ms.value, nbytes.value

    def bench_spmv(self, coeffs, r=1, reps=20):
        c = np.ascontiguousarray(coeffs, dtype=np.complex128)
        ms = C.c_double(0)
        check(_lib.lib().wae_bench_spmv(self.handle, zptr(c), r, reps, C.byref(ms)))
        return ms.value


class Operator:

    def __init__(self, fam, coeffs, op=OP_N, owner=None):
        self.fam = fam
        self.coeffs = np.asarray(coeffs, dtype=np.complex128)
        self.op = op
        self.owner = owner
        self.shape = (fam.d, fam.d)

    @property
    def H(self):
        return Operator(self.fam, self.coeffs, OP_N if self.op == OP_C else OP_C, self.owner)

    def __matmul__(self, x):
        return self.fam.spmv(self.coeffs, x, self.op)

    dot = __matmul__

    def solve(self, b, tol=None, maxit=None, guess=None, quiet=False):
        own = self.owner
        if own is not None:
            own.ensure_solver()
        tol = tol if tol is not None else (own.solver_tol if own is not None else 1e-12)
        maxit = maxit if maxit is not None else (own.solver_maxit if own is not None else 300)
        return self.fam.solve(self.coeffs, b, self.op, tol, maxit, guess=guess, quiet=quiet)

    def __neg__(self):
        return Operator(self.fam, -self.coeffs, self.op, self.owner)
# ... 198 lines not shown
```

Before: 4.385.

## Imply the fine-level right-hand side from the first Jacobi sweep in V-cycles

Adds spmv modes that rebuild the fine-level right-hand side from the first Jacobi iterate (b = D·x1/w) rather than reading the stored b. With one sweep and a tiled SpMV, the residual V-cycle fuses the residual with the first sweep. The later residual and post-smoothing steps then recover b implicitly from x1, saving a full-vector read per kernel and a separate residual pass. It also factors the product/residual cycle launches into helpers. The risk is extra division work and rounding error from reconstructing b, plus aliasing subtleties when the post-sweep writes in place.

```diff
diff --git a/dev/probes/modes_ab.py b/dev/probes/modes_ab.py
--- a/dev/probes/modes_ab.py
+++ b/dev/probes/modes_ab.py
@@ -10,7 +10,8 @@
 L, pb = annulus_family(preset, tau=2e-4)
 fam = L.device()
 cz = L.coefficients(2 * np.pi * (500 + 20j))
-names = {0: "A X", 1: "residual", 2: "Jacobi sweep", 6: "product + first sweep"}
+names = {0: "A X", 1: "residual", 2: "Jacobi sweep", 6: "product + first sweep", 7: "first sweep alone", 8: "residual, implied b",
+         9: "Jacobi sweep, implied b", 10: "residual + first sweep"}
 out = {}
 for m in modes:
     os.environ["WAE_BENCH_MODE"] = str(m)
diff --git a/wavesandeigenvalues.jl_amd/csrc/debug.hip b/wavesandeigenvalues.jl_amd/csrc/debug.hip
--- a/wavesandeigenvalues.jl_amd/csrc/debug.hip
+++ b/wavesandeigenvalues.jl_amd/csrc/debug.hip
@@ -348,9 +348,11 @@
         pcd.upload(tab.data(), tab.size(), st);
         const OpDev A = h->ops[0].dev(WAE_OP_N);
         const int bmode = getenv("WAE_BENCH_MODE") ? atoi(getenv("WAE_BENCH_MODE")) : MODE_AX;
+        WAE_REQUIRE(bmode >= MODE_AX && bmode <= MODE_RES_J0, "WAE_BENCH_MODE: no such form");
+        const bool wants_b = !(bmode == MODE_AX || bmode == MODE_J0 || bmode == MODE_RES_X1);
         DevBuf<cplx> bb;
-        if (bmode != MODE_AX) { bb.alloc(cnt); HIP_CHECK(hipMemcpyAsync(bb.p, hx.data(), cnt * sizeof(cplx), hipMemcpyHostToDevice, st)); }
-        auto one = [&]() { launch_spmv(A, pcd.p, 1 << 30, x.p, y.p, bmode != MODE_AX ? bb.p : nullptr, 0.8, r, bmode, st); };
+        if (wants_b) { bb.alloc(cnt); HIP_CHECK(hipMemcpyAsync(bb.p, hx.data(), cnt * sizeof(cplx), hipMemcpyHostToDevice, st)); }
+        auto one = [&]() { launch_spmv(A, pcd.p, 1 << 30, x.p, y.p, wants_b ? bb.p : nullptr, 0.8, r, bmode, st, nullptr, 0.8); };
         *ms_out = mean_ms(st, reps, one);
         return WAE_OK;
     });
@@ -370,8 +372,9 @@
         if (!X && !Y) return WAE_OK;
         WAE_REQUIRE(X && Y && r > 0 && r <= 256, "bad argument (1 <= r <= 256)");
         WAE_REQUIRE(which != 0 || (coeffs && (ncoef == 1 || ncoef == r)), "ncoef must be 1 or r");
-        WAE_REQUIRE(mode >= MODE_AX && mode <= MODE_AX_J0 && (which == 0 || mode == (which == 1 ? MODE_AX : MODE_ADD)), "bad mode");
-        WAE_REQUIRE(B || mode == MODE_AX || mode == MODE_AX_DS || mode == MODE_AX_J0, "this mode reads B");
+        WAE_REQUIRE(mode >= MODE_AX && mode <= MODE_RES_J0 && (which == 0 || mode == (which == 1 ? MODE_AX : MODE_ADD)), "bad mode");
+        const bool no_b = mode == MODE_AX || mode == MODE_AX_DS || mode == MODE_AX_J0 || mode == MODE_J0 || mode == MODE_RES_X1;
+        WAE_REQUIRE(B || no_b, "this mode reads B");
         WAE_REQUIRE(mode != MODE_AX_J0 || B2, "mode 6 writes B2");
         HIP_CHECK(hipSetDevice(h->device));
         hipStream_t st = h->stream;
@@ -389,7 +392,9 @@
         };
         stage(Y, yi.p);
         if (mode == MODE_AX_J0) stage(B2, bi.p);
-        else if (B) stage(B, bi.p);
+        else if (B && !no_b) stage(B, bi.p);
+        const bool inplace9 = mode == MODE_JAC_X1 && (const void *)B == (const void *)Y;
+        const double jac_w2 = (mode == MODE_JAC_X1 && B2) ? B2[0] : jac_w;
         if (cmask) cm.upload(cmask, (size_t)(r + 7) / 8, st);
         OpDev A;
         int cps = 1 << 30;
@@ -414,8 +419,8 @@
             if (by_tile) launch_prolong_tiles(xf->ft.dev, xi.p, src, yi.p, r, st, cmask ? cm.p : nullptr);
             else launch_prolong_add(xf->p_ptr.p, xf->p_col.p, xf->p_val.p, xf->nf, xi.p, src, yi.p, r, st, cmask ? cm.p : nullptr);
         } else
-        launch_spmv(A, which == 0 ? pcd.p : h->one_dev.p, cps, xi.p, yi.p, (mode == MODE_AX || mode == MODE_AX_DS) ? nullptr : bi.p, jac_w, r, mode, st,
-                    cmask ? cm.p : nullptr);
+        launch_spmv(A, which == 0 ? pcd.p : h->one_dev.p, cps, xi.p, yi.p, (no_b && mode != MODE_AX_J0) ? nullptr : inplace9 ? yi.p : bi.p, jac_w, r,
+                    mode, st, cmask ? cm.p : nullptr, jac_w2);
         launch_inter_to_colmajor(yi.p, r, n_out, r, yc.p, st, perm);
         HIP_CHECK(hipMemcpyAsync(Y, yc.p, cout * sizeof(cplx), hipMemcpyDeviceToHost, st));
         if (mode == MODE_AX_J0) {
@@ -504,17 +509,15 @@
         if (flags & 2) { fout.alloc(cnt); launch_copy(x, fout.p, cnt, st); }
         cplx *b = level == 0 ? h->W.p : h->lb[level].p;
         HIP_CHECK(hipMemcpyAsync(col.p, B, cnt * sizeof(cplx), hipMemcpyHostToDevice, st));
-        bool have_x0 = false;
+        const cplx *res;
         if (flags & 4) {
             vin.alloc(cnt);
             launch_colmajor_to_inter(col.p, n, r, vin.p, r, st, perm);
-            have_x0 = L > 0;
-            launch_spmv(h->ops[0].dev(op), pc_level(h, 0), bt.cps, vin.p, b, have_x0 ? x : nullptr, have_x0 ? pre_weight(h) : 0.0, r,
-                        have_x0 ? MODE_AX_J0 : MODE_AX, st, mk);
+            res = cycle_of_product(h, bt, vin.p, mk, (flags & 2) ? fout.p : nullptr);
         } else {
             launch_colmajor_to_inter(col.p, n, r, b, r, st, perm);
-        }
-        const cplx *res = vcycle(h, bt, level, b, mk, have_x0, (flags & 2) ? fout.p : nullptr);
+            res = vcycle(h, bt, level, b, mk, false, (flags & 2) ? fout.p : nullptr);
+        }
         launch_inter_to_colmajor(res, r, n, r, col.p, st, perm);
         HIP_CHECK(hipMemcpyAsync(Y, col.p, cnt * sizeof(cplx), hipMemcpyDeviceToHost, st));
         HIP_CHECK(hipStreamSynchronize(st));
diff --git a/wavesandeigenvalues.jl_amd/csrc/gmres.hip b/wavesandeigenvalues.jl_amd/csrc/gmres.hip
--- a/wavesandeigenvalues.jl_amd/csrc/gmres.hip
+++ b/wavesandeigenvalues.jl_amd/csrc/gmres.hip
@@ -32,6 +32,29 @@
 
 double pre_weight(const wae_family *h) { return h->vc_light ? h->jac_w_light : h->jac_w; }
 
+bool implied_rhs_cycle(const wae_family *h, const Batch &bt, int l) {
+    return l == 0 && h->ops.size() > 1 && h->nsweeps == 1 && pre_weight(h) > 0.0 && launch_spmv_tiled(h->ops[0].dev(bt.op), bt.nb);
+}
+
+cplx *cycle_of_product(wae_family *h, const Batch &bt, const cplx *v, const unsigned char *cm, cplx *final_out) {
+    const OpDev A = h->ops[0].dev(bt.op);
+    const cplx *pc = pc_level(h, 0);
+    const bool fuse0 = h->ops.size() > 1;
+    launch_spmv(A, pc, bt.cps, v, h->W.p, fuse0 ? h->lx[0].p : nullptr, fuse0 ? pre_weight(h) : 0.0, bt.nb, fuse0 ? MODE_AX_J0 : MODE_AX, h->stream, cm);
+    return vcycle(h, bt, 0, h->W.p, cm, fuse0, final_out);
+}
+
+cplx *cycle_of_residual(wae_family *h, const Batch &bt, const cplx *B, const cplx *X, CycleNorms *cn) {
+    const OpDev A = h->ops[0].dev(bt.op);
+    const cplx *pc = pc_level(h, 0);
+    if (implied_rhs_cycle(h, bt, 0)) {
+        launch_spmv(A, pc, bt.cps, X, h->lx[0].p, B, pre_weight(h), bt.nb, MODE_RES_J0, h->stream);
+        return vcycle(h, bt, 0, nullptr, nullptr, true, nullptr, cn);
+    }
+    launch_spmv(A, pc, bt.cps, X, h->W.p, B, 0.0, bt.nb, MODE_RES, h->stream);
+    return vcycle(h, bt, 0, h->W.p, nullptr, false, nullptr, cn);
+}
+
 cplx *vcycle(wae_family *h, const Batch &bt, int l, const cplx *b, const unsigned char *cm, bool have_x0, cplx *final_out, CycleNorms *cn) {
     const int L = (int)h->ops.size() - 1;
     hipStream_t st = h->stream;
@@ -42,24 +65,33 @@
     const OpDev A = h->ops[l].dev(bt.op);
     const cplx *pc = pc_level(h, l);
     cplx *x = h->lx[l].p, *t = h->lt[l].p;
+    const bool implied = !b;
+    if (implied && !(implied_rhs_cycle(h, bt, l) && have_x0)) throw WaeError(WAE_ERR_INVALID, "vcycle: no right-hand side and no first sweep that implies it");
     if (!have_x0) launch_jacobi0(A, pc, bt.cps, b, x, pre_weight(h), bt.nb, st, cm);
     for (int s = 1; s < h->nsweeps; ++s) {
         launch_spmv(A, pc, bt.cps, x, t, b, pre_weight(h), bt.nb, MODE_JAC, st, cm);
         std::swap(x, t);
     }
-    launch_spmv(A, pc, bt.cps, x, t, b, 0.0, bt.nb, MODE_RES, st, cm);
+    if (implied) launch_spmv(A, pc, bt.cps, x, t, nullptr, pre_weight(h), bt.nb, MODE_RES_X1, st, cm);
+    else launch_spmv(A, pc, bt.cps, x, t, b, 0.0, bt.nb, MODE_RES, st, cm);
     const bool by_tile = h->xfer[l].ft.ready && bt.nb >= 8 && xfer_tiles_on();
     launch_spmv(h->xfer[l].devR(), h->one_dev.p, 1 << 30, t, h->lb[l + 1].p, nullptr, 0.0, bt.nb, MODE_AX, st, cm);
     const cplx *xc = vcycle(h, bt, l + 1, h->lb[l + 1].p, cm);
     const int npost = h->vc_light ? 0 : h->nsweeps;
     const size_t npart = (size_t)(by_tile ? h->xfer[l].ft.dev.ntiles : PROLONG_NORM_BLOCKS) * bt.nb;
     const bool norms = cn && l == 0 && npost == 0 && npart <= h->partial.n && h->ops[l].n > 0 && !(cn->only && final_out);
-    cplx *const px = (norms && cn->only) ? nullptr : (final_out && npost == 0) ? final_out : x;
+    cplx *const x1 = x;
+    cplx *const px = (norms && cn->only) ? nullptr : (final_out && npost == 0) ? final_out : (implied && npost > 0) ? t : x;
     cplx *const part = norms ? h->partial.p : nullptr, *const nout = norms ? cn->out : nullptr;
     if (by_tile) launch_prolong_tiles(h->xfer[l].ft.dev, xc, x, px, bt.nb, st, cm, part, nout);
     else launch_prolong_add(h->xfer[l].p_ptr.p, h->xfer[l].p_col.p, h->xfer[l].p_val.p, h->xfer[l].nf, xc, x, px, bt.nb, st, cm, part, nout);
     if (norms) cn->done = true;
     if (px) x = px;
+    if (implied && npost > 0) {
+        cplx *dst = final_out ? final_out : x1;
+        launch_spmv(A, pc, bt.cps, x, dst, x1, h->jac_w_post, bt.nb, MODE_JAC_X1, st, cm, pre_weight(h));
+        return dst;
+    }
     for (int s = 0; s < npost; ++s) {
         cplx *dst = (final_out && s == npost - 1) ? final_out : t;
         launch_spmv(A, pc, bt.cps, x, dst, b, h->jac_w_post, bt.nb, MODE_JAC, st, cm);
@@ -222,8 +254,7 @@
         return zb;
     }
     cplx *residual(CycleNorms *cn = nullptr) {
-        launch_spmv(A, pc, bt.cps, X, h->W.p, B, 0.0, nb, MODE_RES, st);
-        return vcycle(h, bt, 0, h->W.p, nullptr, false, nullptr, cn);
+        return cycle_of_residual(h, bt, B, X, cn);
     }
     bool drop_bad_guess() {
         if (!x0_unchecked) return false;
@@ -336,13 +367,10 @@
             for (; j < m && total_it < maxit;) {
                 const cplx *vj = h->V.p + (size_t)j * vec;
                 const int nvj = j + 1;
-                const bool fuse0 = h->ops.size() > 1;
                 if (pair_on && j >= pair_min && j + 2 <= m && total_it + 2 <= maxit && status[0] > nb / 4) {
                     cplx *w1 = h->V.p + (size_t)nvj * vec, *w2 = w1 + vec;
-                    launch_spmv(A, pc, bt.cps, vj, h->W.p, h->lx[0].p, pre_weight(h), nb, MODE_AX_J0, st, mk);
-                    vcycle(h, bt, 0, h->W.p, mk, true, w1);
-                    launch_spmv(A, pc, bt.cps, w1, h->W.p, h->lx[0].p, pre_weight(h), nb, MODE_AX_J0, st, mk);
-                    vcycle(h, bt, 0, h->W.p, mk, true, w2);
+                    cycle_of_product(h, bt, vj, mk, w1);
+                    cycle_of_product(h, bt, w1, mk, w2);
                     launch_dots2_scaled(h->V.p, vec, nvj, w1, w2, n, nb, h->partial.p, pr_c1, pr_c2, pr_gram, h->vsq.p, st, mk);
                     launch_gmres_pair_coef(S, j, pr_c1, pr_c2, pr_gram, pr_alpha, pr_c2m, pr_hd2, st);
                     launch_axpy2_norm(h->V.p, vec, nvj, pr_c1, pr_c2m, pr_alpha, w1, w2, n, nb, h->partial.p, pr_norm, h->vsq.p + (size_t)nvj * nb, st, mk);
@@ -352,8 +380,7 @@
                     total_it += 2;
                     since_sync += 2;
                 } else {
-                    launch_spmv(A, pc, bt.cps, vj, h->W.p, fuse0 ? h->lx[0].p : nullptr, fuse0 ? pre_weight(h) : 0.0, nb, fuse0 ? MODE_AX_J0 : MODE_AX, st, mk);
-                    cplx *w = vcycle(h, bt, 0, h->W.p, mk, fuse0);
+                    cplx *w = cycle_of_product(h, bt, vj, mk);
                     launch_dots_scaled(h->V.p, vec, nvj, w, n, nb, h->partial.p, h->hdev.p, h->vsq.p, st, mk);
                     launch_axpy_neg_norm(h->V.p, vec, nvj, h->hdev.p, h->V.p + (size_t)nvj * vec, n, nb, h->partial.p, h->hdev.p + (size_t)nvj * nb, st, mk,
                                          w, h->vsq.p + (size_t)nvj * nb);
@@ -419,14 +446,12 @@
         cplx *c1a = pr_dev, *c2a = c1a + PK, *c1b = c2a + PK, *c2b = c1b + PK, *c2m = c2b + PK, *zero_al = c2m + PK,
              *gram = zero_al + nb, *alpha = gram + 3 * (size_t)nb, *nrm = alpha + nb, *inv = nrm + 2 * (size_t)nb,
              *tdef = inv + 2 * (size_t)nb;
-        launch_spmv(A, pc, bt.cps, vj, h->W.p, h->lx[0].p, pre_weight(h), nb, MODE_AX_J0, st, mk);
-        vcycle(h, bt, 0, h->W.p, mk, true, w1);
+        cycle_of_product(h, bt, vj, mk, w1);
         if (deflate) {
             launch_dots(h->V.p, vec, 1, w1, n, nb, h->partial.p, tdef, st, mk);
             launch_axpy_neg(h->V.p, vec, 1, tdef, w1, n, nb, st, mk);
         }
-        launch_spmv(A, pc, bt.cps, w1, h->W.p, h->lx[0].p, pre_weight(h), nb, MODE_AX_J0, st, mk);
-        vcycle(h, bt, 0, h->W.p, mk, true, w2);
+        cycle_of_product(h, bt, w1, mk, w2);
         launch_dots2_scaled(h->V.p, vec, nv, w1, w2, n, nb, h->partial.p, c1a, c2a, gram, h->vsq.p, st, mk);
         launch_fill_zero(zero_al, nb, st);
         launch_axpy2_norm(h->V.p, vec, nv, c1a, c2a, zero_al, w1, w2, n, nb, h->partial.p, nrm, inv, st, mk);
@@ -503,9 +528,7 @@
     void single_step(int j) {
         const cplx *vj = h->V.p + (size_t)(off + j) * vec;
         const int nvj = off + j + 1;
-        const bool fuse0 = h->ops.size() > 1;
-        launch_spmv(A, pc, bt.cps, vj, h->W.p, fuse0 ? h->lx[0].p : nullptr, fuse0 ? pre_weight(h) : 0.0, nb, fuse0 ? MODE_AX_J0 : MODE_AX, st, mk);
-        cplx *w = vcycle(h, bt, 0, h->W.p, mk, fuse0);
+        cplx *w = cycle_of_product(h, bt, vj, mk);
         if (lazy) {
             launch_dots_scaled(h->V.p, vec, nvj, w, n, nb, h->partial.p, h->hdev.p, h->vsq.p, st, mk);
             launch_axpy_neg_norm(h->V.p, vec, nvj, h->hdev.p, h->V.p + (size_t)nvj * vec, n, nb, h->partial.p, h->hdev.p + (size_t)nvj * nb, st, mk,
@@ -605,8 +628,7 @@
             }
         };
         if (deflate) {
-            launch_spmv(A, pc, bt.cps, guess_dir, h->W.p, nullptr, 0.0, nb, MODE_AX, st);
-            launch_copy(vcycle(h, bt, 0, h->W.p), h->V.p, vec, st);
+            launch_copy(cycle_of_product(h, bt, guess_dir, nullptr), h->V.p, vec, st);
             launch_norms(h->V.p, n, nb, h->partial.p, h->hdev.p, st);
             launch_norms(guess_dir, n, nb, h->partial.p, h->hdev.p + nb, st);
             HIP_CHECK(hipMemcpyAsync(hp, h->hdev.p, (size_t)2 * nb * sizeof(cplx), hipMemcpyDeviceToHost, st));
@@ -621,8 +643,7 @@
             HIP_CHECK(hipStreamSynchronize(st));
         }
         if (guess_dir && !deflate) {
-            launch_spmv(A, pc, bt.cps, guess_dir, h->W.p, nullptr, 0.0, nb, MODE_AX, st);
-            launch_copy(vcycle(h, bt, 0, h->W.p), h->U.p, vec, st);
+            launch_copy(cycle_of_product(h, bt, guess_dir, nullptr), h->U.p, vec, st);
             const cplx *zb = vcycle(h, bt, 0, B);
             launch_dots(h->U.p, 0, 1, zb, n, nb, h->partial.p, h->hdev.p, st);
             launch_dots(h->U.p, 0, 1, h->U.p, n, nb, h->partial.p, h->hdev.p + nb, st);
diff --git a/wavesandeigenvalues.jl_amd/csrc/kernel_helpers.h b/wavesandeigenvalues.jl_amd/csrc/kernel_helpers.h
--- a/wavesandeigenvalues.jl_amd/csrc/kernel_helpers.h
+++ b/wavesandeigenvalues.jl_amd/csrc/kernel_helpers.h
@@ -22,6 +22,10 @@
     double s = 1.0 / (b.x * b.x + b.y * b.y);
     return cplx{(a.x * b.x + a.y * b.y) * s, (a.y * b.x - a.x * b.y) * s};
 }
+__device__ __forceinline__ cplx implied_rhs(cplx dg, cplx x, double w) {
+    const cplx t = {fma(-dg.y, x.y, dg.x * x.x), fma(dg.y, x.x, dg.x * x.y)};
+    return cplx{t.x / w, t.y / w};
+}
 __device__ __forceinline__ int next_chunk(const unsigned char *cmask, int c, int nch) { while (c < nch && cmask && !cmask[c]) ++c; return c; }
 
 static inline unsigned grid_for(size_t total, unsigned cap = 4096) {
diff --git a/wavesandeigenvalues.jl_amd/csrc/kernels.hip b/wavesandeigenvalues.jl_amd/csrc/kernels.hip
--- a/wavesandeigenvalues.jl_amd/csrc/kernels.hip
+++ b/wavesandeigenvalues.jl_amd/csrc/kernels.hip
@@ -79,7 +79,7 @@
 __global__ __launch_bounds__(256) void spmv_kernel(OpDev op, const cplx *__restrict__ pc, int cps,
                                                    const cplx *__restrict__ X, cplx *Y,
                                                    const cplx *B, double jac_w, int nb, int mode,
-                                                   const unsigned char *__restrict__ cmask) {
+                                                   const unsigned char *__restrict__ cmask, double jac_w2) {
     if (C == 8 && cmask && !cmask[blockIdx.y]) return;
     constexpr int TEAM = C * S;
     constexpr int TPB = 256 / TEAM;
@@ -192,11 +192,15 @@
         for (int q = 0; q < npl; ++q) { cplx dq = op.diag[(size_t)row * npl + q]; dq.y *= dsg; cfma(dg, mypc[q], dq); }
         if (mode == MODE_AX_DS) {
             out = cdiv(acc, dg);
-        } else if (mode == MODE_RES_DS) {
+        } else if (mode == MODE_RES_DS || mode == MODE_RES_J0) {
             const cplx bv = B[e];
             out = cdiv(cplx{bv.x - acc.x, bv.y - acc.y}, dg);
+            if (mode == MODE_RES_J0) out = cplx{jac_w * out.x, jac_w * out.y};
+        } else if (mode == MODE_RES_X1) {
+            const cplx bi = implied_rhs(dg, X[e], jac_w);
+            out = cplx{bi.x - acc.x, bi.y - acc.y};
         } else {
-            const cplx bv = B[e], xv = X[e];
+            const cplx bv = mode == MODE_JAC_X1 ? implied_rhs(dg, B[e], jac_w2) : B[e], xv = X[e];
             cplx r = cdiv(cplx{bv.x - acc.x, bv.y - acc.y}, dg);
             out = cplx{xv.x + jac_w * r.x, xv.y + jac_w * r.y};
         }
@@ -210,7 +214,7 @@
 template <int NCH>
 __global__ __launch_bounds__(256, 4) void spmv_lds_kernel(OpDev op, const cplx *__restrict__ pc, int cps,
                                                        const cplx *__restrict__ X, cplx *Y, const cplx *B, double jac_w,
-                                                       int nb, int mode, const unsigned char *__restrict__ cmask) {
+                                                       int nb, int mode, const unsigned char *__restrict__ cmask, double jac_w2) {
     constexpr int C = 8;
     constexpr int TPB = 256 / C;
     constexpr int CW = C * NCH;
@@ -354,17 +358,22 @@
             cplx dg = {0.0, 0.0};
             const double dsg = op.conj_diag ? -1.0 : 1.0;
             for (int q = 0; q < npl; ++q) { cplx dq = op.diag[(size_t)row * npl + q]; dq.y *= dsg; cfma(dg, mypc[q], dq); }
-            if (mode == MODE_AX_J0) {
-                out = acc[k];
+            if (mode == MODE_AX_J0 || mode == MODE_J0) {
                 const cplx r = cdiv(acc[k], dg);
-                const_cast<cplx *>(B)[e] = cplx{jac_w * r.x, jac_w * r.y};
+                const cplx x1 = {jac_w * r.x, jac_w * r.y};
+                out = mode == MODE_J0 ? x1 : acc[k];
+                if (mode == MODE_AX_J0) const_cast<cplx *>(B)[e] = x1;
             } else if (mode == MODE_AX_DS) {
                 out = cdiv(acc[k], dg);
-            } else if (mode == MODE_RES_DS) {
+            } else if (mode == MODE_RES_DS || mode == MODE_RES_J0) {
                 const cplx bv = B[e];
                 out = cdiv(cplx{bv.x - acc[k].x, bv.y - acc[k].y}, dg);
+                if (mode == MODE_RES_J0) out = cplx{jac_w * out.x, jac_w * out.y};
+            } else if (mode == MODE_RES_X1) {
+                const cplx bi = implied_rhs(dg, X[e], jac_w);
+                out = cplx{bi.x - acc[k].x, bi.y - acc[k].y};
             } else {
-                const cplx bv = B[e], xv = X[e];
+                const cplx bv = mode == MODE_JAC_X1 ? implied_rhs(dg, B[e], jac_w2) : B[e], xv = X[e];
                 cplx r = cdiv(cplx{bv.x - acc[k].x, bv.y - acc[k].y}, dg);
                 out = cplx{xv.x + jac_w * r.x, xv.y + jac_w * r.y};
             }
@@ -433,7 +442,7 @@
 template <bool UNI, int LPR, int NBUF, int NWV = 8, int KRT = (LPR == 2 ? 8 : 12)>
 __global__ __launch_bounds__(64 * NWV, NWV == 8 ? 1 : 4) void spmv_tile_kernel(OpDev op, TileDev td, const cplx *__restrict__ pc, int cps,
                                                           const cplx *__restrict__ X, cplx *Y, const cplx *B, double jac_w,
-                                                          int nb, int mode, const unsigned char *__restrict__ cmask, int spc_all, int csplit) {
+                                                          int nb, int mode, const unsigned char *__restrict__ cmask, int spc_all, int csplit, double jac_w2) {
     extern __shared__ __attribute__((aligned(16))) unsigned char tile_smem[];
     const int tid = threadIdx.x;
 #ifdef WAE_TILE_STAMPS
@@ -699,8 +708,10 @@
         const int lrow = wv * RPW + lane / LPR;
         const bool live = lrow < nrows;
         const int64_t row = r0 + (live ? lrow : 0);
-        const bool need_b = mode == MODE_RES || mode == MODE_ADD || mode == MODE_RES_DS || mode == MODE_JAC;
+        const bool need_b = mode == MODE_RES || mode == MODE_ADD || mode == MODE_RES_DS || mode == MODE_JAC || mode == MODE_JAC_X1 ||
+                            mode == MODE_RES_J0;
         const bool need_d = !(mode == MODE_AX || mode == MODE_RES || mode == MODE_ADD);
+        const bool own_x = mode == MODE_JAC || mode == MODE_RES_X1 || mode == MODE_JAC_X1;
         const double dsg = op.conj_diag ? -1.0 : 1.0;
         cplx bv[NOUT], xv[NOUT];
         cplx dgu = {1.0, 0.0};
@@ -721,7 +732,7 @@
                 const int b = col0 + c < nb ? col0 + c : nb - 1;
                 const size_t e = (size_t)row * nb + b;
                 if constexpr (!COAL) bv[j] = need_b ? B[e] : cplx{0.0, 0.0};
-                xv[j] = (mode == MODE_JAC && dslot == 0xFFFFu) ? X[e] : cplx{0.0, 0.0};
+                xv[j] = (own_x && dslot == 0xFFFFu) ? X[e] : cplx{0.0, 0.0};
             }
             if (UNI && need_d) {
                 dgu = cplx{0.0, 0.0};
@@ -740,11 +751,15 @@
 #pragma unroll
             for (int j = 0; j < NOUT; ++j) {
                 if (!FOLD) continue;
+                const bool i8 = mode == MODE_RES_X1, i9 = mode == MODE_JAC_X1;
+                if (i8 && dslot != 0xFFFFu) xv[j] = win[dslot * 8 + ocol(j)];
+                cplx f = {i8 ? xv[j].x : bv[j].x, i8 ? xv[j].y : bv[j].y};
+                if (i8 || i9) f = implied_rhs(dgu, f, i8 ? jac_w : jac_w2);
                 if (LPR == 2) {
-                    acc[j] = cplx{sub == 0 ? sb * bv[j].x : 0.0, sub == 0 ? sb * bv[j].y : 0.0};
-                    acc[j + 4] = cplx{sub == 1 ? sb * bv[j].x : 0.0, sub == 1 ? sb * bv[j].y : 0.0};
+                    acc[j] = cplx{sub == 0 ? sb * f.x : 0.0, sub == 0 ? sb * f.y : 0.0};
+                    acc[j + 4] = cplx{sub == 1 ? sb * f.x : 0.0, sub == 1 ? sb * f.y : 0.0};
                 } else {
-                    acc[j] = cplx{sb * bv[j].x, sb * bv[j].y};
+                    acc[j] = cplx{sb * f.x, sb * f.y};
                 }
             }
         }
@@ -947,7 +962,7 @@
         TILE_STAMP(4);
         if (NBUF == 2) epilogue_loads();
         if constexpr (COAL) { if (need_b) transpose4(bv); }
-        if (mode == MODE_JAC && dslot != 0xFFFFu) {
+        if (own_x && dslot != 0xFFFFu) {
 #pragma unroll
             for (int j = 0; j < NOUT; ++j) xv[j] = win[dslot * 8 + ocol(j)];
         }
@@ -980,16 +995,21 @@
                     dg = cplx{0.0, 0.0};
                     for (int q = 0; q < npl; ++q) { cplx dq = op.diag[(size_t)row * npl + q]; dq.y *= dsg; cfma(dg, mypc[q], dq); }
                 }
-                if (mode == MODE_AX_J0) {
-                    out[j] = av;
+                if (mode == MODE_AX_J0 || mode == MODE_J0) {
                     const cplx r = cdiv(av, dg);
                     b2[j] = cplx{jac_w * r.x, jac_w * r.y};
+                    out[j] = mode == MODE_J0 ? b2[j] : av;
                 } else if (mode == MODE_AX_DS) {
                     out[j] = cdiv(av, dg);
-                } else if (mode == MODE_RES_DS) {
+                } else if (mode == MODE_RES_DS || mode == MODE_RES_J0) {
                     out[j] = cdiv(cplx{bz.x - av.x, bz.y - av.y}, dg);
+                    if (mode == MODE_RES_J0) out[j] = cplx{jac_w * out[j].x, jac_w * out[j].y};
+                } else if (mode == MODE_RES_X1) {
+                    const cplx bi = FOLD ? cplx{0.0, 0.0} : implied_rhs(dg, xv[j], jac_w);
+                    out[j] = cplx{bi.x - av.x, bi.y - av.y};
                 } else {
-                    const cplx r = cdiv(cplx{bz.x - av.x, bz.y - av.y}, dg);
+                    const cplx bi = (mode == MODE_JAC_X1 && !FOLD) ? implied_rhs(dg, bz, jac_w2) : bz;
+                    const cplx r = cdiv(cplx{bi.x - av.x, bi.y - av.y}, dg);
                     out[j] = cplx{xv[j].x + jac_w * r.x, xv[j].y + jac_w * r.y};
                 }
             }
@@ -1077,7 +1097,7 @@
 }
 #endif
 static void launch_spmv_tile(const OpDev &op, const TileDev &td, const cplx *pc, int cps, const cplx *X, cplx *Y, const cplx *B, double jac_w,
-                             int nb, int mode, hipStream_t st, const unsigned char *cmask) {
+                             int nb, int mode, hipStream_t st, const unsigned char *cmask, double jac_w2) {
     const int nbuf = td.nbuf == 3 && td.lpr == 2 ? 3 : 2;
     const size_t wslots = (size_t)((td.wmax + 7) & ~7);
     const int nch8 = ((nb + 7) / 8) * 8;
@@ -1121,10 +1141,10 @@
             HIP_CHECK(hipGetLastError());
         }
     }
-#define WAE_TILE_LAUNCH(U, L, N) hipLaunchKernelGGL((spmv_tile_kernel<U, L, N>), grid, dim3(512), shm, st, op, td, pc, cps, X, Y, B, jac_w, nb, mode, cmask, spc_all, csplit)
+#define WAE_TILE_LAUNCH(U, L, N) hipLaunchKernelGGL((spmv_tile_kernel<U, L, N>), grid, dim3(512), shm, st, op, td, pc, cps, X, Y, B, jac_w, nb, mode, cmask, spc_all, csplit, jac_w2)
     static const int waves16 = getenv("WAE_TILE_WAVES") ? atoi(getenv("WAE_TILE_WAVES")) == 16 : 0;
     if (waves16 && td.lpr == 2 && nbuf == 2 && cps % 8 == 0 && !td.unit)
-        hipLaunchKernelGGL((spmv_tile_kernel<true, 4, 2, 16, 8>), grid, dim3(1024), shm, st, op, td, pc, cps, X, Y, B, jac_w, nb, mode, cmask, spc_all, csplit);
+        hipLaunchKernelGGL((spmv_tile_kernel<true, 4, 2, 16, 8>), grid, dim3(1024), shm, st, op, td, pc, cps, X, Y, B, jac_w, nb, mode, cmask, spc_all, csplit, jac_w2);
     else
     if (td.lpr == 4) { if (cps % 8 == 0) WAE_TILE_LAUNCH(true, 4, 2); else WAE_TILE_LAUNCH(false, 4, 2); }
     else if (nbuf == 3) { if (cps % 8 == 0) WAE_TILE_LAUNCH(true, 2, 3); else WAE_TILE_LAUNCH(false, 2, 3); }
@@ -1133,7 +1153,7 @@
     HIP_CHECK(hipGetLastError());
 }
 
-typedef void (*spmv_fn)(OpDev, const cplx *, int, const cplx *, cplx *, const cplx *, double, int, int, const unsigned char *);
+typedef void (*spmv_fn)(OpDev, const cplx *, int, const cplx *, cplx *, const cplx *, double, int, int, const unsigned char *, double);
 template <int C, int S> static spmv_fn spmv_ptr() { return spmv_kernel<C, S>; }
 
 static spmv_fn pick_spmv(int C, int S) {
@@ -1152,8 +1172,12 @@
     return e ? atoi(e) : dflt;
 }
 
+bool launch_spmv_tiled(const OpDev &op, int nb) {
+    return op.n > 0 && op.tiles && nb >= 8 && env_int("WAE_SPMV_C", 0) == 0 && env_int("WAE_SPMV_S", 0) == 0 && env_int("WAE_SPMV_TILE", 1);
+}
+
 void launch_spmv(const OpDev &op, const cplx *pc, int cps, const cplx *X, cplx *Y, const cplx *B, double jac_w,
-                 int nb, int mode, hipStream_t st, const unsigned char *cmask) {
+                 int nb, int mode, hipStream_t st, const unsigned char *cmask, double jac_w2) {
     const int envC = env_int("WAE_SPMV_C", 0), envS = env_int("WAE_SPMV_S", 0);
     int C = nb >= 8 ? 8 : (nb >= 4 ? 4 : (nb >= 2 ? 2 : 1));
     int S = 64 / C >= 8 ? 8 : 64 / C;
@@ -1164,17 +1188,17 @@
     if (envC > 0 && envC <= nb) C = envC;
     if (envS > 0) S = envS;
     if (op.n <= 0) return;
-    if (op.tiles && nb >= 8 && envC == 0 && envS == 0 && env_int("WAE_SPMV_TILE", 1)) {
-        launch_spmv_tile(op, *op.tiles, pc, cps, X, Y, B, jac_w, nb, mode, st, cmask);
+    if (launch_spmv_tiled(op, nb)) {
+        launch_spmv_tile(op, *op.tiles, pc, cps, X, Y, B, jac_w, nb, mode, st, cmask, jac_w2);
         return;
     }
     if (op.nlong) {
         if (nb > 256) throw WaeError(WAE_ERR_INVALID, "launch_spmv: batch wider than 256 columns");
         launch_long_rows(op, pc, cps, X, nb, nb >= 8 ? cmask : (const unsigned char *)nullptr, st);
     }
-    if (mode == MODE_AX_J0 && !(C == 8 && S == 1 && env_int("WAE_SPMV_LDS", 1))) {
+    if ((mode == MODE_AX_J0 || mode == MODE_J0) && !(C == 8 && S == 1 && env_int("WAE_SPMV_LDS", 1))) {
         launch_spmv(op, pc, cps, X, Y, nullptr, 0.0, nb, MODE_AX, st, cmask);
-        launch_jacobi0(op, pc, cps, Y, const_cast<cplx *>(B), jac_w, nb, st, cmask);
+        launch_jacobi0(op, pc, cps, Y, mode == MODE_J0 ? Y : const_cast<cplx *>(B), jac_w, nb, st, cmask);
         return;
     }
     if (C == 8 && S == 1 && env_int("WAE_SPMV_LDS", 1)) {
@@ -1184,10 +1208,10 @@
         const unsigned nrb = (unsigned)((op.n + 31) / 32);
         dim3 grid((nrb + 7u) / 8u * 8u, (unsigned)((nb + 8 * NCH - 1) / (8 * NCH)));
         size_t shm = (size_t)8 * NCH * op.nplanes_total * sizeof(cplx);
-        if (NCH == 8) hipLaunchKernelGGL(spmv_lds_kernel<8>, grid, dim3(256), shm, st, op, pc, cps, X, Y, B, jac_w, nb, mode, cmask);
-        else if (NCH == 4) hipLaunchKernelGGL(spmv_lds_kernel<4>, grid, dim3(256), shm, st, op, pc, cps, X, Y, B, jac_w, nb, mode, cmask);
-        else if (NCH == 2) hipLaunchKernelGGL(spmv_lds_kernel<2>, grid, dim3(256), shm, st, op, pc, cps, X, Y, B, jac_w, nb, mode, cmask);
-        else hipLaunchKernelGGL(spmv_lds_kernel<1>, grid, dim3(256), shm, st, op, pc, cps, X, Y, B, jac_w, nb, mode, cmask);
+        if (NCH == 8) hipLaunchKernelGGL(spmv_lds_kernel<8>, grid, dim3(256), shm, st, op, pc, cps, X, Y, B, jac_w, nb, mode, cmask, jac_w2);
+        else if (NCH == 4) hipLaunchKernelGGL(spmv_lds_kernel<4>, grid, dim3(256), shm, st, op, pc, cps, X, Y, B, jac_w, nb, mode, cmask, jac_w2);
+        else if (NCH == 2) hipLaunchKernelGGL(spmv_lds_kernel<2>, grid, dim3(256), shm, st, op, pc, cps, X, Y, B, jac_w, nb, mode, cmask, jac_w2);
+        else hipLaunchKernelGGL(spmv_lds_kernel<1>, grid, dim3(256), shm, st, op, pc, cps, X, Y, B, jac_w, nb, mode, cmask, jac_w2);
         HIP_CHECK(hipGetLastError());
         return;
     }
@@ -1197,12 +1221,12 @@
     const unsigned nrb = (unsigned)((op.n + tpb - 1) / tpb);
     dim3 grid((nrb + 7u) / 8u * 8u, (unsigned)((nb + C - 1) / C));
     size_t shm = (size_t)C * op.nplanes_total * sizeof(cplx);
-    hipLaunchKernelGGL(fn, grid, dim3(256), shm, st, op, pc, cps, X, Y, B, jac_w, nb, mode, C == 8 ? cmask : (const unsigned char *)nullptr);
+    hipLaunchKernelGGL(fn, grid, dim3(256), shm, st, op, pc, cps, X, Y, B, jac_w, nb, mode, C == 8 ? cmask : (const unsigned char *)nullptr, jac_w2);
     HIP_CHECK(hipGetLastError());
 }
 
 __global__ __launch_bounds__(256) void jacobi0_kernel(OpDev op, const cplx *__restrict__ pc, int cps,
-                                                      const cplx *__restrict__ B, cplx *__restrict__ X, double w, int nb,
+                                                      const cplx *B, cplx *X, double w, int nb,
                                                       const unsigned char *__restrict__ cmask) {
     const size_t total = (size_t)op.n * nb;
     const int npl = op.nplanes_total;
diff --git a/wavesandeigenvalues.jl_amd/csrc/solver.h b/wavesandeigenvalues.jl_amd/csrc/solver.h
--- a/wavesandeigenvalues.jl_amd/csrc/solver.h
+++ b/wavesandeigenvalues.jl_amd/csrc/solver.h
@@ -8,6 +8,9 @@
 struct CycleNorms { cplx *out; bool only; bool done = false; };
 cplx *vcycle(wae_family *h, const Batch &bt, int l, const cplx *b, const unsigned char *cm = nullptr, bool have_x0 = false,
              cplx *final_out = nullptr, CycleNorms *cn = nullptr);
+bool implied_rhs_cycle(const wae_family *h, const Batch &bt, int l);
+cplx *cycle_of_product(wae_family *h, const Batch &bt, const cplx *v, const unsigned char *cm, cplx *final_out = nullptr);
+cplx *cycle_of_residual(wae_family *h, const Batch &bt, const cplx *B, const cplx *X, CycleNorms *cn = nullptr);
 void penalty_polish(wae_family *h, const Batch &bt, const cplx *B, cplx *X);
 int gmres(wae_family *h, const Batch &bt, const cplx *B, cplx *X, double tol, int maxit, wae_solve_info *info, const cplx *guess_dir = nullptr,
           bool have_x0 = false, double *relres_out = nullptr);
diff --git a/wavesandeigenvalues.jl_amd/csrc/wae_internal.h b/wavesandeigenvalues.jl_amd/csrc/wae_internal.h
--- a/wavesandeigenvalues.jl_amd/csrc/wae_internal.h
+++ b/wavesandeigenvalues.jl_amd/csrc/wae_internal.h
@@ -261,9 +261,11 @@
         if (!std::isfinite(c_point[i])) throw WaeError(WAE_ERR_INVALID, "c_point holds a value that is not finite");
 }
 
-enum { MODE_AX = 0, MODE_RES = 1, MODE_JAC = 2, MODE_ADD = 3, MODE_AX_DS = 4, MODE_RES_DS = 5, MODE_AX_J0 = 6 };
+enum { MODE_AX = 0, MODE_RES = 1, MODE_JAC = 2, MODE_ADD = 3, MODE_AX_DS = 4, MODE_RES_DS = 5, MODE_AX_J0 = 6,
+       MODE_J0 = 7, MODE_RES_X1 = 8, MODE_JAC_X1 = 9, MODE_RES_J0 = 10 };
 void launch_spmv(const OpDev &op, const cplx *pc, int cps, const cplx *X, cplx *Y, const cplx *B, double jac_w,
-                 int nb, int mode, hipStream_t s, const unsigned char *cmask = nullptr);
+                 int nb, int mode, hipStream_t s, const unsigned char *cmask = nullptr, double jac_w2 = 0.0);
+bool launch_spmv_tiled(const OpDev &op, int nb);
 void launch_jacobi0(const OpDev &op, const cplx *pc, int cps, const cplx *B, cplx *X, double jac_w, int nb, hipStream_t s,
                     const unsigned char *cmask = nullptr);
 void launch_spmv_multi(const OpDev &op, const cplx *pc, const int *plane_col, const cplx *X, cplx *Y, int nb, hipStream_t s);
diff --git a/wavesandeigenvalues.jl_amd/nlevp/linopfam.py b/wavesandeigenvalues.jl_amd/nlevp/linopfam.py
--- a/wavesandeigenvalues.jl_amd/nlevp/linopfam.py
+++ b/wavesandeigenvalues.jl_amd/nlevp/linopfam.py
@@ -444,7 +444,8 @@
         self._report(code, info, f"perturb_batch ({nsys} systems, order {N})", quiet=quiet)
         return lam, (None if V is None else V.transpose(0, 2, 1)), self.last_status
 
-    def debug_spmv(self, coeffs, X, mode=0, B=None, Y0=None, op=OP_N, jac_w=0.8, cmask=None, level=0, which=0, no_tiles=False):
+    def debug_spmv(self, coeffs, X, mode=0, B=None, Y0=None, op=OP_N, jac_w=0.8, cmask=None, level=0, which=0, no_tiles=False,
+                   jac_w_pre=None, inplace=False):
         lib = _lib.lib()
         nin, nout = C.c_int64(0), C.c_int64(0)
         check(lib.wae_debug_spmv(self.handle, which, level, 0, None, 0, None, None, None, None, 0, op, 0.0, None, 0, C.byref(nin), C.byref(nout)))
@@ -457,8 +458,13 @@
         if mode == 6 and Y0 is not None:
             B2[...] = Y0
         cm = None if cmask is None else (C.c_uint8 * ((r + 7) // 8))(*[1 if x else 0 for x in cmask])
+        if mode == 9 and inplace:
+            Y = np.asfortranarray(np.array(Bf, dtype=np.complex128))
+            Bf = Y
+        wpre = None if (mode != 9 or jac_w_pre is None) else np.array([float(jac_w_pre)])
+        b2p = wpre.ctypes.data_as(C.POINTER(C.c_double)) if wpre is not None else (None if B2 is None else zptr(B2))
         check(lib.wae_debug_spmv(self.handle, which, level, mode, zptr(c), c.shape[0], zptr(Xf), None if Bf is None else zptr(Bf), zptr(Y),
-                                 None if B2 is None else zptr(B2), r, op, float(jac_w), cm, 1 if no_tiles else 0, C.byref(nin), C.byref(nout)))
+                                 b2p, r, op, float(jac_w), cm, 1 if no_tiles else 0, C.byref(nin), C.byref(nout)))
         return (Y, B2) if mode == 6 else Y
 
     def debug_prolong(self, X, B, Y0=None, level=0, cmask=None, no_tiles=False, norms_only=False):
```

After: 4.384 (median of 3 runs). No clear change (-0.0%).
